# kan-bayashi/ParallelWaveGAN

Hardware: AMD Instinct MI355X
Metric: HiFi-GAN V1 22.05 kHz generator inference RTF^-1 (audio samples/s) (higher is better)
Workload: dtype f32; 1 GPU; HiFi-GAN V1 generator fwd, LJSpeech 22.05 kHz, B16 x 800 mel frames per GPU, fp32, random init; global_batch=16, parallelism=replicas x1

## Files before the change

include/pwg_kernels.h:

```cpp
#ifndef PWG_KERNELS_H_
#define PWG_KERNELS_H_

#include <stddef.h>
#include <stdint.h>

#ifdef __cplusplus
extern "C" {
#endif

typedef enum pwg_status {
  PWG_OK = 0,
  PWG_ERR_BAD_SHAPE = -1,
  PWG_ERR_UNSUPPORTED = -2,
  PWG_ERR_LAUNCH = -3,
  PWG_ERR_NULL = -4,
  PWG_ERR_WORKSPACE = -5
} pwg_status;

const char* pwg_last_error(void);
int pwg_abi_version(void);
int pwg_target_arch(void);

int pwg_prof_enable(int on);
int pwg_prof_reset(void);
int pwg_prof_num_kernels(void);
int pwg_prof_get(int32_t idx, char* name, size_t name_cap, double* total_ms, int64_t* launches,
                 double* flops, double* bytes);

float pwg_set_concurrency_hint(float fill_scale);

int pwg_debug_poison_lds(int on);

enum { PWG_ACT_NONE = 0, PWG_ACT_LEAKY_RELU = 1, PWG_ACT_TANH = 2, PWG_ACT_RELU = 3 };
enum { PWG_PAD_ZERO = 0, PWG_PAD_REFLECT = 1, PWG_PAD_REPLICATE = 2 };

typedef struct pwg_conv1d_desc {
  int32_t batch;
  int32_t c_in;
  int32_t c_out;
  int32_t t_in;
  int32_t t_out;
  int32_t width;
  int32_t kernel;
  int32_t stride;
  int32_t dilation;
  int32_t pad_left;
  int32_t groups;
  int32_t transposed;
  int32_t pad_mode;
  int32_t pre_act;
  float pre_slope;
  int32_t post_act;
  float post_slope;
  float out_mul;
  float out_div;
} pwg_conv1d_desc;

size_t pwg_conv1d_packed_weight_floats(const pwg_conv1d_desc* d);

int pwg_conv1d_pack_weight(const pwg_conv1d_desc* d, const float* w, const float* scale,
                           float* w_packed, void* stream);

size_t pwg_conv1d_forward_workspace_floats(const pwg_conv1d_desc* d);
int pwg_conv1d_forward(const pwg_conv1d_desc* d, const float* x, const float* w_packed,
                       const float* bias, const float* add1, const float* add2, float* y,
                       float* workspace, size_t workspace_floats, void* stream);

size_t pwg_conv1d_packed_weight_bwd_floats(const pwg_conv1d_desc* d);
int pwg_conv1d_pack_weight_bwd(const pwg_conv1d_desc* d, const float* w, const float* scale,
                               float* w_packed_bwd, void* stream);
typedef struct pwg_bank_item {
  const float* w;
  const float* g;
  float* scale;
  float* fwd;
  float* bwd;
  pwg_conv1d_desc desc;
} pwg_bank_item;
size_t pwg_weight_bank_table_bytes(int32_t n_items);
int pwg_weight_bank_build(const pwg_bank_item* items, int32_t n_items, void* table_host, size_t table_bytes,
                          int32_t* info);
int pwg_weight_bank_prepare(const void* table_dev, const int32_t* info, int32_t with_bwd, void* stream);

size_t pwg_conv1d_backward_data_workspace_floats(const pwg_conv1d_desc* d);
int pwg_conv1d_backward_data(const pwg_conv1d_desc* d, const float* dy, const float* w_packed_bwd,
                             const float* x, const float* accum, float* dx, float* workspace,
                             size_t workspace_floats, void* stream);
size_t pwg_conv1d_backward_weight_workspace_floats(const pwg_conv1d_desc* d);
int pwg_conv1d_backward_weight(const pwg_conv1d_desc* d, const float* x, const float* dy, float* dw,
                               float* db, float* workspace, size_t workspace_floats, void* stream);

size_t pwg_conv1d_backward_weight_wn_workspace_floats(const pwg_conv1d_desc* d);
int pwg_conv1d_backward_weight_wn(const pwg_conv1d_desc* d, const float* x, const float* dy, const float* v,
                                  const float* g, float* dv, float* dg, float* db, float* workspace,
                                  size_t workspace_floats, void* stream);

int pwg_conv1d_num_tile_configs(void);
int pwg_conv1d_forward_cfg(const pwg_conv1d_desc* d, const float* x, const float* w_packed,
                           const float* bias, const float* add1, const float* add2, float* y,
                           int32_t tile_config, int32_t use_dma, void* stream);

int pwg_conv1d_bf16_supported(const pwg_conv1d_desc* d);
size_t pwg_conv1d_bf16_packed_weight_bytes(const pwg_conv1d_desc* d);
int pwg_conv1d_bf16_pack_weight(const pwg_conv1d_desc* d, const float* w, const float* scale, void* w_packed,
                                void* stream);
int pwg_conv1d_bf16_forward(const pwg_conv1d_desc* d, const float* x, const void* w_packed, const float* bias,
                            const float* add1, const float* add2, float* y, float* workspace, size_t workspace_floats,
                            void* stream);
int pwg_conv1d_bf16_forward_cfg(const pwg_conv1d_desc* d, const float* x, const void* w_packed, const float* bias,
                                const float* add1, const float* add2, float* y, int32_t mfma_shape, void* stream);

int pwg_conv1d_split_supported(const pwg_conv1d_desc* d);
size_t pwg_conv1d_split_packed_weight_bytes(const pwg_conv1d_desc* d);
int pwg_conv1d_split_pack_weight(const pwg_conv1d_desc* d, const float* w, const float* scale, void* w_packed,
                                 void* stream);
int pwg_conv1d_split_forward(const pwg_conv1d_desc* d, const float* x, const void* w_packed, const float* bias,
                             const float* add1, const float* add2, float* y, float* workspace, size_t workspace_floats,
                             void* stream);
int pwg_conv1d_split_forward_cfg(const pwg_conv1d_desc* d, const float* x, const void* w_packed, const float* bias,
                                 const float* add1, const float* add2, float* y, int32_t mfma_shape, int32_t tile_mode,
                                 void* stream);
int pwg_conv1d_split_step_form(const pwg_conv1d_desc* d);
int pwg_conv1d_split_forward_step(const pwg_conv1d_desc* d, const float* x, const void* w_packed, const float* bias,
                                  const float* add1, const float* add2, float* y, int32_t mfma_shape, int32_t tile_mode,
                                  int32_t step_form, void* stream);
int pwg_conv1d_split_window_form(const pwg_conv1d_desc* d);
int pwg_conv1d_split_forward_window(const pwg_conv1d_desc* d, const float* x, const void* w_packed, const float* bias,
                                    const float* add1, const float* add2, float* y, int32_t mfma_shape,
                                    int32_t tile_mode, int32_t step_form, int32_t window_form, void* stream);

int pwg_convtr1d_split_supported(const pwg_conv1d_desc* d);
size_t pwg_convtr1d_split_packed_weight_bytes(const pwg_conv1d_desc* d);
int pwg_convtr1d_split_pack_weight(const pwg_conv1d_desc* d, const float* w, const float* scale, void* w_packed,
                                   void* stream);
int pwg_convtr1d_split_forward(const pwg_conv1d_desc* d, const float* x, const void* w_packed, const float* bias,
                               const float* add1, const float* add2, float* y, float* workspace,
                               size_t workspace_floats, void* stream);
int pwg_convtr1d_split_forward_cfg(const pwg_conv1d_desc* d, const float* x, const void* w_packed, const float* bias,
                                   const float* add1, const float* add2, float* y, int32_t mfma_shape,
                                   int32_t tile_mode, void* stream);

int pwg_conv1d_stream_supported(const pwg_conv1d_desc* d);
size_t pwg_conv1d_stream_hist_floats(const pwg_conv1d_desc* d);
int pwg_conv1d_stream_forward(const pwg_conv1d_desc* d, const float* x, const float* hist_in, float* hist_out,
                              const float* w_packed, const float* bias, const float* add1, const float* add2, float* y,
                              void* stream);

int pwg_conv1d_stream_bf16_supported(const pwg_conv1d_desc* d);
int pwg_conv1d_stream_bf16_forward(const pwg_conv1d_desc* d, const float* x, const float* hist_in, float* hist_out,
                                   const void* w_packed_bf16, const float* bias, const float* add1,
                                   const float* add2, float* y, void* stream);

int pwg_conv1d_stream_delayed_supported(const pwg_conv1d_desc* d, int32_t delay1, int32_t delay2);
int pwg_conv1d_stream_delayed_forward(const pwg_conv1d_desc* d, const float* x, const float* hist_in, float* hist_out,
                                      const float* w_packed, const float* bias, const float* add1,
                                      const float* add1_hist_in, float* add1_hist_out, int32_t delay1, const float* add2,
                                      const float* add2_hist_in, float* add2_hist_out, int32_t delay2, int32_t valid_lo,
                                      int32_t valid_hi, float* y, void* stream);

int pwg_conv1d_stream_bf16_delayed_supported(const pwg_conv1d_desc* d, int32_t delay1, int32_t delay2);
int pwg_conv1d_stream_bf16_delayed_forward(const pwg_conv1d_desc* d, const float* x, const float* hist_in,
                                           float* hist_out, const void* w_packed_bf16, const float* bias,
                                           const float* add1, const float* add1_hist_in, float* add1_hist_out,
                                           int32_t delay1, const float* add2, const float* add2_hist_in,
                                           float* add2_hist_out, int32_t delay2, int32_t valid_lo, int32_t valid_hi,
                                           float* y, void* stream);

int pwg_conv1d_stream_slots_forward(const pwg_conv1d_desc* d, const float* x, const float* hist_in, float* hist_out,
                                    const float* w_packed, const float* bias, const float* add1,
                                    const float* add1_hist_in, float* add1_hist_out, int32_t delay1, const float* add2,
                                    const float* add2_hist_in, float* add2_hist_out, int32_t delay2, const int32_t* slots,
                                    int32_t rate, int32_t delay, float* y, void* stream);
int pwg_conv1d_stream_slots_forward_bf16(const pwg_conv1d_desc* d, const float* x, const float* hist_in, float* hist_out,
                                         const void* w_packed_bf16, const float* bias, const float* add1,
                                         const float* add1_hist_in, float* add1_hist_out, int32_t delay1,
                                         const float* add2, const float* add2_hist_in, float* add2_hist_out,
                                         int32_t delay2, const int32_t* slots, int32_t rate, int32_t delay, float* y,
                                         void* stream);

int pwg_conv1d_stream_mirrored_supported(const pwg_conv1d_desc* d);
int pwg_conv1d_stream_mirrored_forward(const pwg_conv1d_desc* d, const float* x, const float* hist_in, float* hist_out,
                                       const float* w_packed, const float* bias, float* y, int32_t in_lo, int32_t in_hi,
                                       int32_t valid_lo, int32_t valid_hi, void* stream);

int pwg_conv1d_stream_plan(const pwg_conv1d_desc* d, int32_t* out);

int pwg_conv1d_plan(const pwg_conv1d_desc* d, int32_t has_addends, int32_t* out);
int pwg_debug_conv_tile_of_workgroup(int32_t grid_x, int32_t grid_y, int32_t grid_z, int32_t row_blocks,
                                     int32_t ksplit, int32_t item_major, int32_t workgroup, int32_t* out);

int pwg_conv1d_backward_weight_plan(const pwg_conv1d_desc* d, int32_t weight_norm, int32_t has_bias, int32_t* out);

typedef struct pwg_resunit_desc {
  int32_t batch;
  int32_t channels;
  int32_t t;
  int32_t kernel;
  int32_t dilation;
  int32_t has_conv2;
  float slope1;
  float slope2;
  float out_div;
} pwg_resunit_desc;
int pwg_resunit_supported(const pwg_resunit_desc* d);
int pwg_resunit_profitable(const pwg_resunit_desc* d);
size_t pwg_resunit_packed_weight_floats(int32_t channels, int32_t kernel);
int pwg_resunit_pack_weight(int32_t channels, int32_t kernel, const float* w, const float* scale,
                            float* w_packed, void* stream);
int pwg_resunit_forward(const pwg_resunit_desc* d, const float* x, const float* w1_packed, const float* b1,
                        const float* w2_packed, const float* b2, const float* add2, float* y, void* stream);

int pwg_resunit_split_supported(const pwg_resunit_desc* d);
int pwg_resunit_split_forward(const pwg_resunit_desc* d, const float* x, const void* w1_split, const float* b1,
                              const void* w2_split, const float* b2, const float* add2, float* y, void* stream);
int pwg_resunit_split_forward_cfg(const pwg_resunit_desc* d, const float* x, const void* w1_split, const float* b1,
                                  const void* w2_split, const float* b2, const float* add2, float* y, int32_t mfma_shape,
                                  void* stream);
int pwg_resunit_split_ragged_supported(const pwg_resunit_desc* d, int32_t rate);
int pwg_resunit_split_forward_ragged(const pwg_resunit_desc* d, const float* x, const void* w1_split, const float* b1,
                                     const void* w2_split, const float* b2, const float* add2, float* y,
                                     int32_t mfma_shape, const int32_t* frames, int32_t rate, void* stream);
int pwg_resblock_split_supported(const pwg_resunit_desc* d, int32_t n_units, const int32_t* dilations);
int pwg_resblock_split_frame(const pwg_resunit_desc* d, int32_t n_units, const int32_t* dilations, int32_t* out);
int pwg_resblock_split_forward_cfg(const pwg_resunit_desc* d, int32_t n_units, const int32_t* dilations,
                                   const float* slopes1, const float* slopes2, const float* x,
                                   const void* const* w1_split, const float* const* b1, const void* const* w2_split,
                                   const float* const* b2, const float* add2, float* y, int32_t mfma_shape, void* stream);

int pwg_resstack_supported(int32_t channels, int32_t t, int32_t dilation);
size_t pwg_resstack_packed_weight_floats(int32_t channels);
int pwg_resstack_pack_weight(int32_t channels, const float* w1, const float* scale1, const float* w2,
                             const float* scale2, const float* ws, const float* scale_s, float* w_packed, void* stream);
int pwg_resstack_forward(int32_t batch, int32_t channels, int32_t t, int32_t dilation, float slope, const float* x,
                         const float* w_packed, const float* b1, const float* b2, const float* bs, float* y, float* h,
                         void* stream);
int pwg_resstack_ragged_supported(int32_t channels, int32_t t, int32_t dilation, int32_t rate);
int pwg_resstack_forward_ragged(int32_t batch, int32_t channels, int32_t t, int32_t dilation, float slope, const float* x,
                                const float* w_packed, const float* b1, const float* b2, const float* bs, float* y,
                                const int32_t* frames, int32_t rate, void* stream);
int pwg_resstack_pack_weight_bwd(int32_t channels, const float* w1, const float* scale1, const float* w2,
                                 const float* scale2, const float* ws, const float* scale_s, float* w_packed,
                                 void* stream);
int pwg_resstack_backward_data(int32_t batch, int32_t channels, int32_t t, int32_t dilation, float slope,
                               const float* dy, const float* h, const float* x, const float* w_packed_bwd, float* dh,
                               float* dxp, void* stream);

typedef struct pwg_wavenet_desc {
  int32_t batch;
  int32_t t;
  int32_t residual_channels;
  int32_t gate_channels;
  int32_t skip_channels;
  int32_t aux_channels;
  int32_t kernel;
  int32_t dilation;
  int32_t causal;
  float out_mul;
  float skip_mul;
} pwg_wavenet_desc;
int pwg_wavenet_layer_supported(const pwg_wavenet_desc* d);
size_t pwg_wavenet_packed_weight_floats(const pwg_wavenet_desc* d);
int pwg_wavenet_pack_weights(const pwg_wavenet_desc* d, const float* w_dil, const float* scale_dil, const float* w_aux,
                             const float* scale_aux, const float* w_skip, const float* scale_skip, const float* w_out,
                             const float* scale_out, float* packed, void* stream);
int pwg_wavenet_layer_forward(const pwg_wavenet_desc* d, const float* x, const float* c, const float* skips,
                              const float* packed, const float* b_dil, const float* b_skip, const float* b_out,
                              float* x_out, float* skips_out, float* z_out, float* g_out, void* stream);
int pwg_wavenet_stream_supported(const pwg_wavenet_desc* d);
size_t pwg_wavenet_stream_hist_floats(const pwg_wavenet_desc* d);
int pwg_wavenet_stream_forward(const pwg_wavenet_desc* d, const float* x, const float* c, const float* skips,
                               const float* hist_in, float* hist_out, const float* packed, const float* b_dil,
                               const float* b_skip, const float* b_out, float* x_out, float* skips_out, void* stream);
int pwg_wavenet_stream_delayed_supported(const pwg_wavenet_desc* d, int32_t c_delay);
size_t pwg_wavenet_stream_delayed_hist_floats(const pwg_wavenet_desc* d);
int pwg_wavenet_stream_delayed_forward(const pwg_wavenet_desc* d, const float* x, const float* c, const float* c_line,
                                       int32_t c_cols, int32_t c_delay, const float* skips, const float* skip_line_in,
                                       float* skip_line_out, const float* hist_in, float* hist_out, const float* packed,
                                       const float* b_dil, const float* b_skip, const float* b_out, int32_t valid_lo,
                                       int32_t valid_hi, float* x_out, float* skips_out, void* stream);
int pwg_wavenet_stream_slots_forward(const pwg_wavenet_desc* d, const float* x, const float* c, const float* c_line,
                                     int32_t c_cols, int32_t c_delay, const float* skips, const float* skip_line_in,
                                     float* skip_line_out, const float* hist_in, float* hist_out, const float* packed,
                                     const float* b_dil, const float* b_skip, const float* b_out, const int32_t* slots,
                                     int32_t rate, int32_t delay, float* x_out, float* skips_out, void* stream);
int pwg_wavenet_stream_slots_forward_bf16(const pwg_wavenet_desc* d, const float* x, const float* c, const float* c_line,
                                          int32_t c_cols, int32_t c_delay, const float* skips, const float* skip_line_in,
                                          float* skip_line_out, const float* hist_in, float* hist_out, const void* packed,
                                          const float* b_dil, const float* b_skip, const float* b_out,
                                          const int32_t* slots, int32_t rate, int32_t delay, float* x_out,
                                          float* skips_out, void* stream);
int pwg_wavenet_bf16_supported(const pwg_wavenet_desc* d);
size_t pwg_wavenet_bf16_packed_weight_bytes(const pwg_wavenet_desc* d);
int pwg_wavenet_bf16_pack_weights(const pwg_wavenet_desc* d, const float* w_dil, const float* scale_dil,
                                  const float* w_aux, const float* scale_aux, const float* w_skip, const float* scale_skip,
                                  const float* w_out, const float* scale_out, void* packed, void* stream);
int pwg_wavenet_bf16_layer_forward(const pwg_wavenet_desc* d, const float* x, const float* c, const float* skips,
                                   const void* packed, const float* b_dil, const float* b_skip, const float* b_out,
                                   float* x_out, float* skips_out, float* z_out, float* g_out, void* stream);
int pwg_wavenet_bf16_layer_forward_cfg(const pwg_wavenet_desc* d, const float* x, const float* c, const float* skips,
                                       const void* packed, const float* b_dil, const float* b_skip, const float* b_out,
                                       float* x_out, float* skips_out, float* z_out, float* g_out, int32_t mfma_shape,
                                       void* stream);
int pwg_wavenet_layer_ragged_supported(const pwg_wavenet_desc* d, int32_t rate);
int pwg_wavenet_layer_forward_ragged(const pwg_wavenet_desc* d, const float* x, const float* c, const float* skips,
                                     const float* packed, const float* b_dil, const float* b_skip, const float* b_out,
                                     float* x_out, float* skips_out, const int32_t* frames, int32_t rate, void* stream);
int pwg_wavenet_bf16_layer_forward_ragged(const pwg_wavenet_desc* d, const float* x, const float* c, const float* skips,
                                          const void* packed, const float* b_dil, const float* b_skip,
                                          const float* b_out, float* x_out, float* skips_out, int32_t mfma_shape,
                                          const int32_t* frames, int32_t rate, void* stream);
int pwg_wavenet_stream_bf16_supported(const pwg_wavenet_desc* d);
int pwg_wavenet_stream_bf16_forward(const pwg_wavenet_desc* d, const float* x, const float* c, const float* skips,
                                    const float* hist_in, float* hist_out, const void* packed, const float* b_dil,
                                    const float* b_skip, const float* b_out, float* x_out, float* skips_out, float* z_out,
                                    float* g_out, void* stream);
int pwg_wavenet_stream_bf16_delayed_supported(const pwg_wavenet_desc* d, int32_t c_delay);
int pwg_wavenet_stream_bf16_delayed_forward(const pwg_wavenet_desc* d, const float* x, const float* c, const float* c_line,
                                            int32_t c_cols, int32_t c_delay, const float* skips, const float* skip_line_in,
                                            float* skip_line_out, const float* hist_in, float* hist_out, const void* packed,
                                            const float* b_dil, const float* b_skip, const float* b_out, int32_t valid_lo,
                                            int32_t valid_hi, float* x_out, float* skips_out, float* z_out, float* g_out,
                                            void* stream);
size_t pwg_wavenet_packed_weight_bwd_floats(const pwg_wavenet_desc* d);
int pwg_wavenet_pack_weights_bwd(const pwg_wavenet_desc* d, const float* w_dil, const float* scale_dil, const float* w_aux,
                                 const float* scale_aux, const float* w_skip, const float* scale_skip, const float* w_out,
                                 const float* scale_out, float* packed, void* stream);
int pwg_wavenet_gate_backward(const pwg_wavenet_desc* d, const float* z, const float* dx_out, const float* ds_out,
                              const float* packed_bwd, float* dz, float* go, void* stream);
int pwg_wavenet_data_backward(const pwg_wavenet_desc* d, const float* dz, const float* go, const float* packed_bwd,
                              const float* dc_accum, float* dx, float* dc, void* stream);
typedef struct pwg_wavenet_param_grad {
  const float* v;
  const float* g;
  float* dw;
  float* dg;
  float* db;
} pwg_wavenet_param_grad;
size_t pwg_wavenet_weight_backward_workspace_floats(const pwg_wavenet_desc* d);
int pwg_wavenet_weight_backward(const pwg_wavenet_desc* d, const float* dz, const float* x, const float* c, const float* gs,
                                const float* go, const float* g, const pwg_wavenet_param_grad* grads, float* workspace,
                                size_t workspace_floats, void* stream);
int pwg_wavenet_weight_backward_plan(const pwg_wavenet_desc* d, int32_t out[4]);

int pwg_weight_norm_scale(const float* v, const float* g, float* scale, int32_t n0,
                          int32_t inner, void* stream);
int pwg_scale_rows(const float* v, const float* scale, float* w, int32_t n0, int32_t inner,
                   void* stream);

int pwg_act_backward(const float* dy, const float* y, float* dx, int64_t n, int32_t act, float slope,
                     float scale, void* stream);
int pwg_add3_div(const float* a, const float* b, const float* c, float* y, int64_t n, float div, void* stream);
int pwg_weight_norm_backward(const float* dw, const float* v, const float* g, float* dv, float* dg,
                             int32_t n0, int32_t inner, void* stream);
int pwg_spectral_norm_forward(const float* w_orig, float* u, float* v, float* sigma, float* w, float* tmp,
                              int32_t rows, int32_t cols, int32_t do_iter, float eps, void* stream);
int pwg_spectral_norm_forward_saved(const float* w_orig, float* u, float* v, float* sigma, float* w, float* tmp,
                                    float* u_saved, float* v_saved, int32_t rows, int32_t cols, int32_t do_iter,
                                    float eps, void* stream);
#define PWG_SPECTRAL_NORM_SCRATCH_FLOATS 257
int pwg_spectral_norm_backward(const float* dw, const float* w_orig, const float* u, const float* v,
                               const float* sigma, float* dw_orig, float* scratch, int32_t rows,
                               int32_t cols, void* stream);

int pwg_gate_forward(const float* z, float* out, int32_t batch, int32_t channels, int64_t t, void* stream);
int pwg_gate_backward(const float* z, const float* dout, float* dz, int32_t batch, int32_t channels,
                      int64_t t, void* stream);
#define PWG_STRETCH_CONV_WGRAD_BLOCKS 512
int pwg_stretch_conv_forward(const float* x, const float* w, float* y, int64_t rows, int32_t t_in,
                             int32_t scale, int32_t kernel, int32_t pad_left, int32_t channels,
                             int32_t freq_kernel, int32_t act, float slope, void* stream);
int pwg_stretch_conv_stream(const float* x, const float* hist_in, float* hist_out, const float* w, float* y,
                            int64_t rows, int32_t n, int32_t scale, int32_t freq_kernel, int32_t act, float slope,
                            void* stream);
int pwg_stretch_conv_stream_delayed(const float* x, const float* hist_in, float* hist_out, const float* w, float* y,
                                    int64_t rows, int32_t n, int32_t scale, int32_t freq_kernel, int32_t act, float slope,
                                    int32_t valid_lo, int32_t valid_hi, void* stream);
int pwg_delay_line_forward(const float* x, const float* line_in, float* line_out, float* delayed_out, int64_t rows,
                           int32_t n, int32_t columns, void* stream);
int pwg_stretch_conv_stream_slots(const float* x, const float* hist_in, float* hist_out, const float* w, float* y,
                                  int64_t items, int32_t channels, int32_t n, int32_t scale, int32_t freq_kernel,
                                  int32_t act, float slope, const int32_t* slots, int32_t rate, int32_t delay, void* stream);
int pwg_delay_line_slots_forward(const float* x, const float* line_in, float* line_out, float* delayed_out, int64_t items,
                                 int32_t channels, int32_t n, int32_t columns, const int32_t* slots, void* stream);
int pwg_slot_seed_history(const float* x, float* hist, int64_t items, int32_t channels, int32_t n, int32_t columns,
                          const int32_t* slots, void* stream);
size_t pwg_stretch_conv_backward_workspace_floats(int32_t kernel, int32_t freq_kernel);
int pwg_stretch_conv_backward(const float* dy, const float* x, const float* w, float* dx, float* dw,
                              int64_t rows, int32_t t_in, int32_t scale, int32_t kernel, int32_t pad_left,
                              int32_t channels, int32_t freq_kernel, float* workspace, size_t workspace_floats,
                              void* stream);
int pwg_pqmf_down(const float* x, const float* h, float* y, int32_t batch, int64_t t_in, int64_t n_out,
                  int32_t subbands, int32_t len, int32_t pad, void* stream);
int pwg_pqmf_up(const float* y, const float* g, float* x, int32_t batch, int64_t n_in, int64_t t_out,
                int32_t subbands, int32_t len, int32_t pad, void* stream);

int pwg_pqmf_up_stream_geometry(int32_t subbands, int32_t len, int32_t pad, int32_t* hist_columns,
                                int32_t* delay_columns);
int pwg_pqmf_up_stream(const float* y, const float* hist_in, float* hist_out, const float* g, float* x, int32_t batch,
                       int64_t n, int64_t n_emit, int32_t subbands, int32_t len, int32_t pad, void* stream);

int pwg_instance_norm_forward(const float* x, float* y, float* mean, float* rstd, int64_t rows, int32_t t,
                              float eps, void* stream);
int pwg_instance_norm_backward(const float* dy, const float* y, const float* rstd, float* dx, int64_t rows,
                               int32_t t, void* stream);
int pwg_upsample_nearest_forward(const float* x, const float* add, float* y, int64_t rows, int32_t t_in,
                                 int32_t scale, void* stream);
int pwg_upsample_nearest_backward(const float* dy, float* dx, int64_t rows, int32_t t_in, int32_t scale,
                                  void* stream);
int pwg_tade_modulate_forward(const float* xn, const float* cg, float* y, int32_t batch, int32_t channels,
                              int32_t t_in, int32_t scale, void* stream);
int pwg_tade_modulate_backward(const float* dy, const float* xn, const float* cg, float* dxn, float* dcg,
                               int32_t batch, int32_t channels, int32_t t_in, int32_t scale, void* stream);
int pwg_softmax_gate_forward(const float* z, float* y, int32_t batch, int32_t channels, int64_t t,
                             int32_t use_softmax, void* stream);
int pwg_softmax_gate_backward(const float* z, const float* dy, float* dz, int32_t batch, int32_t channels,
                              int64_t t, int32_t use_softmax, void* stream);

int pwg_copy_channels(float* x, float* y, int32_t batch, int32_t c_src, int32_t c_dst, int32_t c_off,
                      int64_t t, int32_t reverse, void* stream);
int pwg_dropout(const float* x, float* y, int64_t n, float p, uint64_t seed, const uint64_t* seed_dev,
                void* stream);

int pwg_gather_crop(const float* audio, const int64_t* audio_off, const int64_t* audio_len, const float* mel,
                    const int64_t* mel_off, const int32_t* utt, const int32_t* start, float* y, float* c,
                    int32_t batch, int32_t steps, int32_t hop, int32_t frames_ctx, int32_t acw,
                    int32_t channels, void* stream);

int pwg_wave_to_pcm16(const float* x, int16_t* pcm, int64_t n, void* stream);
int pwg_normalize_transpose(const float* x, const float* mean, const float* scale, float* y,
                            int32_t batch, int32_t frames, int32_t channels, void* stream);
int pwg_zero_tail(float* y, const int32_t* frames, int32_t batch, int32_t channels, int64_t t, int32_t rate,
                  void* stream);
int pwg_mirror_tail(float* y, const int32_t* frames, int32_t batch, int32_t channels, int64_t t, int32_t rate,
                    int32_t pad, void* stream);

int pwg_avg_pool1d_forward(const float* x, float* y, int64_t rows, int32_t t_in, int32_t t_out,
                           int32_t kernel, int32_t stride, int32_t pad, int32_t count_include_pad,
                           void* stream);
int pwg_avg_pool1d_backward(const float* dy, float* dx, int64_t rows, int32_t t_in, int32_t t_out,
                            int32_t kernel, int32_t stride, int32_t pad, int32_t count_include_pad,
                            void* stream);
int pwg_pad1d_forward(const float* x, float* y, int64_t rows, int32_t t_in, int32_t pad_left,
                      int32_t pad_right, int32_t mode, void* stream);
int pwg_pad1d_backward(const float* dy, float* dx, int64_t rows, int32_t t_in, int32_t pad_left,
                       int32_t pad_right, int32_t mode, void* stream);

int pwg_frame_fold_forward(const float* x, float* y, int32_t batch, int32_t t, int32_t pad, int32_t hop,
                           int32_t n_cols, void* stream);
int pwg_frame_fold_backward(const float* dy, float* dx, int32_t batch, int32_t t, int32_t pad,
                            int32_t hop, int32_t n_cols, void* stream);
int pwg_stft_mag_forward(const float* spec, float* mag, int32_t batch, int32_t bins, int32_t frames,
                         float eps, void* stream);
int pwg_stft_mag_backward(const float* spec, const float* mag, const float* dmag, float* dspec,
                          int32_t batch, int32_t bins, int32_t frames, float eps, void* stream);
int pwg_log_clamp_forward(const float* x, float* y, int64_t n, float eps, float log_div, void* stream);
int pwg_log_clamp_backward(const float* x, const float* dy, float* dx, int64_t n, float eps, float log_div,
                           void* stream);

size_t pwg_stft_loss_workspace_floats(int32_t batch, int32_t bins, int32_t frames);
int pwg_stft_loss_forward(const float* fx, const float* fy, const float* basis, int32_t batch, int32_t hop,
                          int32_t n_cols, int32_t taps, int32_t bins, int32_t frames, float eps,
                          float* workspace, float* sums, void* stream);
int pwg_stft_loss_backward(const float* fx, const float* fy, const float* basis, int32_t batch, int32_t hop,
                           int32_t n_cols, int32_t taps, int32_t bins, int32_t frames, float eps,
                           const float* sums, const float* g2, float* dspec, void* stream);

int pwg_stft_fft_supported(int32_t n_fft, int32_t win, int32_t hop);
size_t pwg_stft_fft_workspace_floats(int32_t batch, int32_t frames, int32_t n_fft);
int pwg_stft_fft_loss_forward(const float* x, const float* y, const float* window, const float* twiddle, int32_t batch,
                              int32_t t, int32_t n_fft, int32_t hop, int32_t win, float eps, float* workspace,
                              float* sums, void* stream);
int pwg_stft_fft_loss_backward(const float* x, const float* y, const float* window, const float* twiddle, int32_t batch,
                               int32_t t, int32_t n_fft, int32_t hop, int32_t win, float eps, const float* sums,
                               const float* g2, float* dframes, float* dx, void* stream);

int pwg_mel_fft_loss_forward(const float* x, const float* y, const float* window, const float* twiddle, const float* fb,
                             const int32_t* mel_range, const int32_t* bin_range, int32_t batch, int32_t t, int32_t n_fft,
                             int32_t hop, int32_t win, int32_t n_mels, int32_t bins_pad, float eps, float log_div,
                             float* workspace, float* total, void* stream);
int pwg_mel_fft_loss_backward(const float* x, const float* y, const float* window, const float* twiddle, const float* fb,
                              const int32_t* mel_range, const int32_t* bin_range, int32_t batch, int32_t t, int32_t n_fft,
                              int32_t hop, int32_t win, int32_t n_mels, int32_t bins_pad, float eps, float log_div,
                              const float* gout, float* dframes, float* dx, void* stream);

size_t pwg_mel_loss_workspace_floats(int32_t batch, int32_t bins, int32_t frames, int32_t n_mels);
int pwg_mel_loss_forward(const float* fx, const float* fy, const float* basis, const float* mel_t, int32_t batch,
                         int32_t hop, int32_t n_cols, int32_t taps, int32_t bins, int32_t frames, int32_t n_mels,
                         float eps, float log_div, float* workspace, float* mel_x, float* mel_y, float* sum,
                         void* stream);
int pwg_mel_loss_backward(const float* fx, const float* basis, const float* mel_b, const float* mel_x,
                          const float* mel_y, int32_t batch, int32_t hop, int32_t n_cols, int32_t taps,
                          int32_t bins, int32_t frames, int32_t n_mels, float eps, float log_div,
                          const float* gout, float* dspec, void* stream);

enum { PWG_RED_ABS_DIFF = 0, PWG_RED_SQ_DIFF = 1, PWG_RED_SQ = 2, PWG_RED_SQ_DIFF_CONST = 3, PWG_RED_SUM = 4,
       PWG_RED_HINGE_REAL = 5, PWG_RED_HINGE_FAKE = 6 };
int pwg_reduce_forward(const float* a, const float* b, float c, int64_t n, int32_t mode, float scale,
                       float* out, float* workspace, void* stream);
int pwg_reduce_backward(const float* a, const float* b, float c, int64_t n, int32_t mode, float scale,
                        const float* gout, float* da, float* db, void* stream);

#define PWG_RED_MAX_ITEMS 64
typedef struct pwg_red_item {
  const float* a;
  const float* b;
  float* da;
  float* db;
  int64_t n;
  int32_t mode;
  int32_t slot;
  float scale;
  float c;
} pwg_red_item;
size_t pwg_multi_reduce_workspace_floats(const pwg_red_item* items, int32_t n_items);
int pwg_multi_reduce_forward(const pwg_red_item* items, int32_t n_items, int32_t n_slots, float* out,
                             int32_t accumulate, float* workspace, void* stream);
int pwg_multi_reduce_backward(const pwg_red_item* items, int32_t n_items, int32_t n_slots, const float* gout,
                              void* stream);

typedef struct pwg_opt_chunk {
  float* p;
  const float* g;
  float* m;
  float* v;
  float* vmax;
  int32_t n;
  int32_t pad_;
} pwg_opt_chunk;
int pwg_adam_step(const void* chunks, int32_t n_chunks, float lr, float beta1, float beta2, float eps,
                  float weight_decay, int32_t step, float grad_scale, void* stream);
// ... 12 lines not shown
```

parallelwavegan_amd/_lib.py:

```python
import ctypes
import os

_HERE = os.path.dirname(os.path.abspath(__file__))
LIB_PATH = os.environ.get("PWG_KERNEL_LIB") or os.path.join(_HERE, "libpwgkernels.so")

PWG_ACT_NONE, PWG_ACT_LEAKY_RELU, PWG_ACT_TANH, PWG_ACT_RELU = 0, 1, 2, 3
PWG_PAD_ZERO, PWG_PAD_REFLECT, PWG_PAD_REPLICATE = 0, 1, 2
ABI_VERSION = 15
SPECTRAL_NORM_SCRATCH_FLOATS = 257


class ConvDesc(ctypes.Structure):

    _fields_ = [
        ("batch", ctypes.c_int32),
        ("c_in", ctypes.c_int32),
        ("c_out", ctypes.c_int32),
        ("t_in", ctypes.c_int32),
        ("t_out", ctypes.c_int32),
        ("width", ctypes.c_int32),
        ("kernel", ctypes.c_int32),
        ("stride", ctypes.c_int32),
        ("dilation", ctypes.c_int32),
        ("pad_left", ctypes.c_int32),
        ("groups", ctypes.c_int32),
        ("transposed", ctypes.c_int32),
        ("pad_mode", ctypes.c_int32),
        ("pre_act", ctypes.c_int32),
        ("pre_slope", ctypes.c_float),
        ("post_act", ctypes.c_int32),
        ("post_slope", ctypes.c_float),
        ("out_mul", ctypes.c_float),
        ("out_div", ctypes.c_float),
    ]


class BankItem(ctypes.Structure):

    _fields_ = [("w", ctypes.c_void_p), ("g", ctypes.c_void_p), ("scale", ctypes.c_void_p), ("fwd", ctypes.c_void_p),
                ("bwd", ctypes.c_void_p), ("desc", ConvDesc)]


class WaveNetDesc(ctypes.Structure):

    _fields_ = [
        ("batch", ctypes.c_int32),
        ("t", ctypes.c_int32),
        ("residual_channels", ctypes.c_int32),
        ("gate_channels", ctypes.c_int32),
        ("skip_channels", ctypes.c_int32),
        ("aux_channels", ctypes.c_int32),
        ("kernel", ctypes.c_int32),
        ("dilation", ctypes.c_int32),
        ("causal", ctypes.c_int32),
        ("out_mul", ctypes.c_float),
        ("skip_mul", ctypes.c_float),
    ]


class WaveNetParamGrad(ctypes.Structure):

    _fields_ = [("v", ctypes.c_void_p), ("g", ctypes.c_void_p), ("dw", ctypes.c_void_p), ("dg", ctypes.c_void_p),
                ("db", ctypes.c_void_p)]


class ResUnitDesc(ctypes.Structure):

    _fields_ = [
        ("batch", ctypes.c_int32),
        ("channels", ctypes.c_int32),
        ("t", ctypes.c_int32),
        ("kernel", ctypes.c_int32),
        ("dilation", ctypes.c_int32),
        ("has_conv2", ctypes.c_int32),
        ("slope1", ctypes.c_float),
        ("slope2", ctypes.c_float),
        ("out_div", ctypes.c_float),
    ]


class RedItem(ctypes.Structure):

    _fields_ = [
        ("a", ctypes.c_void_p),
        ("b", ctypes.c_void_p),
        ("da", ctypes.c_void_p),
        ("db", ctypes.c_void_p),
        ("n", ctypes.c_int64),
        ("mode", ctypes.c_int32),
        ("slot", ctypes.c_int32),
        ("scale", ctypes.c_float),
        ("c", ctypes.c_float),
    ]


RED_MAX_ITEMS = 64

_lib = None
_vp = ctypes.c_void_p
_i32 = ctypes.c_int32
_i64 = ctypes.c_int64
_f32 = ctypes.c_float

SIGNATURES = {
    "pwg_last_error": (ctypes.c_char_p, []),
    "pwg_abi_version": (ctypes.c_int, []),
    "pwg_target_arch": (ctypes.c_int, []),
    "pwg_debug_poison_lds": (ctypes.c_int, [ctypes.c_int]),
    "pwg_set_concurrency_hint": (ctypes.c_float, [ctypes.c_float]),
    "pwg_prof_enable": (ctypes.c_int, [ctypes.c_int]),
    "pwg_prof_reset": (ctypes.c_int, []),
    "pwg_prof_num_kernels": (ctypes.c_int, []),
    "pwg_prof_get": (ctypes.c_int, [_i32, ctypes.c_char_p, ctypes.c_size_t, ctypes.POINTER(ctypes.c_double),
                                    ctypes.POINTER(ctypes.c_int64), ctypes.POINTER(ctypes.c_double),
                                    ctypes.POINTER(ctypes.c_double)]),
    "pwg_conv1d_packed_weight_floats": (ctypes.c_size_t, [ctypes.POINTER(ConvDesc)]),
    "pwg_conv1d_pack_weight": (ctypes.c_int, [ctypes.POINTER(ConvDesc), _vp, _vp, _vp, _vp]),
    "pwg_conv1d_forward_workspace_floats": (ctypes.c_size_t, [ctypes.POINTER(ConvDesc)]),
    "pwg_conv1d_forward": (ctypes.c_int, [ctypes.POINTER(ConvDesc), _vp, _vp, _vp, _vp, _vp, _vp, _vp, ctypes.c_size_t,
                                          _vp]),
    "pwg_conv1d_bf16_supported": (ctypes.c_int, [ctypes.POINTER(ConvDesc)]),
    "pwg_conv1d_bf16_packed_weight_bytes": (ctypes.c_size_t, [ctypes.POINTER(ConvDesc)]),
    "pwg_conv1d_bf16_pack_weight": (ctypes.c_int, [ctypes.POINTER(ConvDesc), _vp, _vp, _vp, _vp]),
    "pwg_conv1d_bf16_forward": (ctypes.c_int, [ctypes.POINTER(ConvDesc), _vp, _vp, _vp, _vp, _vp, _vp, _vp, ctypes.c_size_t,
                                               _vp]),
    "pwg_conv1d_bf16_forward_cfg": (ctypes.c_int, [ctypes.POINTER(ConvDesc), _vp, _vp, _vp, _vp, _vp, _vp, _i32, _vp]),
    "pwg_conv1d_split_supported": (ctypes.c_int, [ctypes.POINTER(ConvDesc)]),
    "pwg_conv1d_split_packed_weight_bytes": (ctypes.c_size_t, [ctypes.POINTER(ConvDesc)]),
    "pwg_conv1d_split_pack_weight": (ctypes.c_int, [ctypes.POINTER(ConvDesc), _vp, _vp, _vp, _vp]),
    "pwg_conv1d_split_forward": (ctypes.c_int, [ctypes.POINTER(ConvDesc), _vp, _vp, _vp, _vp, _vp, _vp, _vp,
                                                ctypes.c_size_t, _vp]),
    "pwg_conv1d_split_forward_cfg": (ctypes.c_int, [ctypes.POINTER(ConvDesc), _vp, _vp, _vp, _vp, _vp, _vp, _i32, _i32,
                                                    _vp]),
    "pwg_conv1d_split_step_form": (ctypes.c_int, [ctypes.POINTER(ConvDesc)]),
    "pwg_conv1d_split_forward_step": (ctypes.c_int, [ctypes.POINTER(ConvDesc), _vp, _vp, _vp, _vp, _vp, _vp, _i32, _i32,
                                                     _i32, _vp]),
    "pwg_conv1d_split_window_form": (ctypes.c_int, [ctypes.POINTER(ConvDesc)]),
    "pwg_conv1d_split_forward_window": (ctypes.c_int, [ctypes.POINTER(ConvDesc), _vp, _vp, _vp, _vp, _vp, _vp, _i32,
                                                       _i32, _i32, _i32, _vp]),
    "pwg_convtr1d_split_supported": (ctypes.c_int, [ctypes.POINTER(ConvDesc)]),
    "pwg_convtr1d_split_packed_weight_bytes": (ctypes.c_size_t, [ctypes.POINTER(ConvDesc)]),
    "pwg_convtr1d_split_pack_weight": (ctypes.c_int, [ctypes.POINTER(ConvDesc), _vp, _vp, _vp, _vp]),
    "pwg_convtr1d_split_forward": (ctypes.c_int, [ctypes.POINTER(ConvDesc), _vp, _vp, _vp, _vp, _vp, _vp, _vp,
                                                  ctypes.c_size_t, _vp]),
    "pwg_convtr1d_split_forward_cfg": (ctypes.c_int, [ctypes.POINTER(ConvDesc), _vp, _vp, _vp, _vp, _vp, _vp, _i32, _i32,
                                                      _vp]),
    "pwg_conv1d_stream_supported": (ctypes.c_int, [ctypes.POINTER(ConvDesc)]),
    "pwg_conv1d_stream_hist_floats": (ctypes.c_size_t, [ctypes.POINTER(ConvDesc)]),
    "pwg_conv1d_stream_forward": (ctypes.c_int, [ctypes.POINTER(ConvDesc), _vp, _vp, _vp, _vp, _vp, _vp, _vp, _vp, _vp]),
    "pwg_conv1d_stream_plan": (ctypes.c_int, [ctypes.POINTER(ConvDesc), ctypes.POINTER(_i32)]),
    "pwg_conv1d_stream_bf16_supported": (ctypes.c_int, [ctypes.POINTER(ConvDesc)]),
    "pwg_conv1d_stream_bf16_forward": (ctypes.c_int, [ctypes.POINTER(ConvDesc), _vp, _vp, _vp, _vp, _vp, _vp, _vp, _vp,
                                                      _vp]),
    "pwg_conv1d_stream_delayed_supported": (ctypes.c_int, [ctypes.POINTER(ConvDesc), _i32, _i32]),
    "pwg_conv1d_stream_delayed_forward": (ctypes.c_int, [ctypes.POINTER(ConvDesc), _vp, _vp, _vp, _vp, _vp, _vp, _vp, _vp,
                                                         _i32, _vp, _vp, _vp, _i32, _i32, _i32, _vp, _vp]),
    "pwg_conv1d_stream_bf16_delayed_supported": (ctypes.c_int, [ctypes.POINTER(ConvDesc), _i32, _i32]),
    "pwg_conv1d_stream_bf16_delayed_forward": (ctypes.c_int, [ctypes.POINTER(ConvDesc), _vp, _vp, _vp, _vp, _vp, _vp, _vp,
                                                              _vp, _i32, _vp, _vp, _vp, _i32, _i32, _i32, _vp, _vp]),
    "pwg_conv1d_stream_slots_forward": (ctypes.c_int, [ctypes.POINTER(ConvDesc), _vp, _vp, _vp, _vp, _vp, _vp, _vp, _vp,
                                                       _i32, _vp, _vp, _vp, _i32, _vp, _i32, _i32, _vp, _vp]),
    "pwg_conv1d_stream_slots_forward_bf16": (ctypes.c_int, [ctypes.POINTER(ConvDesc), _vp, _vp, _vp, _vp, _vp, _vp, _vp,
                                                            _vp, _i32, _vp, _vp, _vp, _i32, _vp, _i32, _i32, _vp, _vp]),
    "pwg_conv1d_stream_mirrored_supported": (ctypes.c_int, [ctypes.POINTER(ConvDesc)]),
    "pwg_conv1d_stream_mirrored_forward": (ctypes.c_int, [ctypes.POINTER(ConvDesc), _vp, _vp, _vp, _vp, _vp, _vp, _i32,
                                                          _i32, _i32, _i32, _vp]),
    "pwg_conv1d_packed_weight_bwd_floats": (ctypes.c_size_t, [ctypes.POINTER(ConvDesc)]),
    "pwg_conv1d_pack_weight_bwd": (ctypes.c_int, [ctypes.POINTER(ConvDesc), _vp, _vp, _vp, _vp]),
    "pwg_weight_bank_table_bytes": (ctypes.c_size_t, [_i32]),
    "pwg_weight_bank_build": (ctypes.c_int, [ctypes.POINTER(BankItem), _i32, _vp, ctypes.c_size_t,
                                             ctypes.POINTER(ctypes.c_int32)]),
    "pwg_weight_bank_prepare": (ctypes.c_int, [_vp, ctypes.POINTER(ctypes.c_int32), _i32, _vp]),
    "pwg_conv1d_backward_data_workspace_floats": (ctypes.c_size_t, [ctypes.POINTER(ConvDesc)]),
    "pwg_conv1d_backward_data": (ctypes.c_int, [ctypes.POINTER(ConvDesc), _vp, _vp, _vp, _vp, _vp, _vp, ctypes.c_size_t,
                                                _vp]),
    "pwg_conv1d_backward_weight_workspace_floats": (ctypes.c_size_t, [ctypes.POINTER(ConvDesc)]),
    "pwg_conv1d_backward_weight": (ctypes.c_int, [ctypes.POINTER(ConvDesc), _vp, _vp, _vp, _vp, _vp, ctypes.c_size_t, _vp]),
    "pwg_conv1d_backward_weight_wn_workspace_floats": (ctypes.c_size_t, [ctypes.POINTER(ConvDesc)]),
    "pwg_conv1d_backward_weight_wn": (ctypes.c_int, [ctypes.POINTER(ConvDesc), _vp, _vp, _vp, _vp, _vp, _vp, _vp, _vp,
                                                     ctypes.c_size_t, _vp]),
    "pwg_conv1d_num_tile_configs": (ctypes.c_int, []),
    "pwg_conv1d_forward_cfg": (ctypes.c_int, [ctypes.POINTER(ConvDesc), _vp, _vp, _vp, _vp, _vp, _vp, _i32, _i32, _vp]),
    "pwg_conv1d_plan": (ctypes.c_int, [ctypes.POINTER(ConvDesc), _i32, ctypes.POINTER(_i32)]),
    "pwg_conv1d_backward_weight_plan": (ctypes.c_int, [ctypes.POINTER(ConvDesc), _i32, _i32, ctypes.POINTER(_i32)]),
    "pwg_debug_conv_tile_of_workgroup": (ctypes.c_int, [_i32, _i32, _i32, _i32, _i32, _i32, _i32, ctypes.POINTER(_i32)]),
    "pwg_resunit_supported": (ctypes.c_int, [ctypes.POINTER(ResUnitDesc)]),
    "pwg_resunit_profitable": (ctypes.c_int, [ctypes.POINTER(ResUnitDesc)]),
    "pwg_resunit_packed_weight_floats": (ctypes.c_size_t, [_i32, _i32]),
    "pwg_resunit_pack_weight": (ctypes.c_int, [_i32, _i32, _vp, _vp, _vp, _vp]),
    "pwg_resunit_forward": (ctypes.c_int, [ctypes.POINTER(ResUnitDesc), _vp, _vp, _vp, _vp, _vp, _vp, _vp, _vp]),
    "pwg_resunit_split_supported": (ctypes.c_int, [ctypes.POINTER(ResUnitDesc)]),
    "pwg_resunit_split_forward": (ctypes.c_int, [ctypes.POINTER(ResUnitDesc), _vp, _vp, _vp, _vp, _vp, _vp, _vp, _vp]),
    "pwg_resunit_split_forward_cfg": (ctypes.c_int, [ctypes.POINTER(ResUnitDesc), _vp, _vp, _vp, _vp, _vp, _vp, _vp, _i32,
                                                     _vp]),
    "pwg_resunit_split_ragged_supported": (ctypes.c_int, [ctypes.POINTER(ResUnitDesc), _i32]),
    "pwg_resunit_split_forward_ragged": (ctypes.c_int, [ctypes.POINTER(ResUnitDesc), _vp, _vp, _vp, _vp, _vp, _vp, _vp,
                                                        _i32, _vp, _i32, _vp]),
    "pwg_resblock_split_supported": (ctypes.c_int, [ctypes.POINTER(ResUnitDesc), _i32, ctypes.POINTER(_i32)]),
    "pwg_resblock_split_frame": (ctypes.c_int, [ctypes.POINTER(ResUnitDesc), _i32, ctypes.POINTER(_i32),
                                                ctypes.POINTER(_i32)]),
    "pwg_resblock_split_forward_cfg": (ctypes.c_int, [ctypes.POINTER(ResUnitDesc), _i32, ctypes.POINTER(_i32),
                                                      ctypes.POINTER(ctypes.c_float), ctypes.POINTER(ctypes.c_float), _vp,
                                                      ctypes.POINTER(_vp), ctypes.POINTER(_vp), ctypes.POINTER(_vp),
                                                      ctypes.POINTER(_vp), _vp, _vp, _i32, _vp]),
    "pwg_resstack_supported": (ctypes.c_int, [_i32, _i32, _i32]),
    "pwg_resstack_packed_weight_floats": (ctypes.c_size_t, [_i32]),
    "pwg_resstack_pack_weight": (ctypes.c_int, [_i32, _vp, _vp, _vp, _vp, _vp, _vp, _vp, _vp]),
    "pwg_resstack_forward": (ctypes.c_int, [_i32, _i32, _i32, _i32, ctypes.c_float, _vp, _vp, _vp, _vp, _vp, _vp, _vp, _vp]),
    "pwg_resstack_ragged_supported": (ctypes.c_int, [_i32, _i32, _i32, _i32]),
    "pwg_resstack_forward_ragged": (ctypes.c_int, [_i32, _i32, _i32, _i32, ctypes.c_float, _vp, _vp, _vp, _vp, _vp, _vp, _vp,
                                                   _i32, _vp]),
    "pwg_resstack_pack_weight_bwd": (ctypes.c_int, [_i32, _vp, _vp, _vp, _vp, _vp, _vp, _vp, _vp]),
    "pwg_resstack_backward_data": (ctypes.c_int, [_i32, _i32, _i32, _i32, ctypes.c_float, _vp, _vp, _vp, _vp, _vp, _vp, _vp]),
    "pwg_wavenet_layer_supported": (ctypes.c_int, [ctypes.POINTER(WaveNetDesc)]),
    "pwg_wavenet_packed_weight_floats": (ctypes.c_size_t, [ctypes.POINTER(WaveNetDesc)]),
    "pwg_wavenet_pack_weights": (ctypes.c_int, [ctypes.POINTER(WaveNetDesc)] + [_vp] * 10),
    "pwg_wavenet_layer_forward": (ctypes.c_int, [ctypes.POINTER(WaveNetDesc)] + [_vp] * 12),
    "pwg_wavenet_stream_supported": (ctypes.c_int, [ctypes.POINTER(WaveNetDesc)]),
    "pwg_wavenet_stream_hist_floats": (ctypes.c_size_t, [ctypes.POINTER(WaveNetDesc)]),
    "pwg_wavenet_stream_forward": (ctypes.c_int, [ctypes.POINTER(WaveNetDesc)] + [_vp] * 12),
    "pwg_wavenet_stream_delayed_supported": (ctypes.c_int, [ctypes.POINTER(WaveNetDesc), _i32]),
    "pwg_wavenet_stream_delayed_hist_floats": (ctypes.c_size_t, [ctypes.POINTER(WaveNetDesc)]),
    "pwg_wavenet_stream_delayed_forward": (ctypes.c_int, [ctypes.POINTER(WaveNetDesc), _vp, _vp, _vp, _i32, _i32] + [_vp] * 9
                                           + [_i32, _i32, _vp, _vp, _vp]),
    "pwg_wavenet_stream_slots_forward": (ctypes.c_int, [ctypes.POINTER(WaveNetDesc), _vp, _vp, _vp, _i32, _i32] + [_vp] * 9
                                         + [_vp, _i32, _i32, _vp, _vp, _vp]),
    "pwg_wavenet_stream_slots_forward_bf16": (ctypes.c_int, [ctypes.POINTER(WaveNetDesc), _vp, _vp, _vp, _i32, _i32]
                                              + [_vp] * 9 + [_vp, _i32, _i32, _vp, _vp, _vp]),
    "pwg_wavenet_bf16_supported": (ctypes.c_int, [ctypes.POINTER(WaveNetDesc)]),
    "pwg_wavenet_bf16_packed_weight_bytes": (ctypes.c_size_t, [ctypes.POINTER(WaveNetDesc)]),
    "pwg_wavenet_bf16_pack_weights": (ctypes.c_int, [ctypes.POINTER(WaveNetDesc)] + [_vp] * 10),
    "pwg_wavenet_bf16_layer_forward": (ctypes.c_int, [ctypes.POINTER(WaveNetDesc)] + [_vp] * 12),
    "pwg_wavenet_bf16_layer_forward_cfg": (ctypes.c_int, [ctypes.POINTER(WaveNetDesc)] + [_vp] * 11 + [_i32, _vp]),
    "pwg_wavenet_layer_ragged_supported": (ctypes.c_int, [ctypes.POINTER(WaveNetDesc), _i32]),
    "pwg_wavenet_layer_forward_ragged": (ctypes.c_int, [ctypes.POINTER(WaveNetDesc)] + [_vp] * 10 + [_i32, _vp]),
    "pwg_wavenet_bf16_layer_forward_ragged": (ctypes.c_int, [ctypes.POINTER(WaveNetDesc)] + [_vp] * 9
                                              + [_i32, _vp, _i32, _vp]),
    "pwg_wavenet_stream_bf16_supported": (ctypes.c_int, [ctypes.POINTER(WaveNetDesc)]),
    "pwg_wavenet_stream_bf16_forward": (ctypes.c_int, [ctypes.POINTER(WaveNetDesc)] + [_vp] * 14),
    "pwg_wavenet_stream_bf16_delayed_supported": (ctypes.c_int, [ctypes.POINTER(WaveNetDesc), _i32]),
    "pwg_wavenet_stream_bf16_delayed_forward": (ctypes.c_int, [ctypes.POINTER(WaveNetDesc), _vp, _vp, _vp, _i32, _i32]
                                                + [_vp] * 9 + [_i32, _i32, _vp, _vp, _vp, _vp, _vp]),
    "pwg_wavenet_packed_weight_bwd_floats": (ctypes.c_size_t, [ctypes.POINTER(WaveNetDesc)]),
    "pwg_wavenet_pack_weights_bwd": (ctypes.c_int, [ctypes.POINTER(WaveNetDesc)] + [_vp] * 10),
    "pwg_wavenet_gate_backward": (ctypes.c_int, [ctypes.POINTER(WaveNetDesc)] + [_vp] * 7),
    "pwg_wavenet_data_backward": (ctypes.c_int, [ctypes.POINTER(WaveNetDesc)] + [_vp] * 7),
    "pwg_wavenet_weight_backward_workspace_floats": (ctypes.c_size_t, [ctypes.POINTER(WaveNetDesc)]),
    "pwg_wavenet_weight_backward_plan": (ctypes.c_int, [ctypes.POINTER(WaveNetDesc), ctypes.POINTER(_i32)]),
    "pwg_wavenet_weight_backward": (ctypes.c_int, [ctypes.POINTER(WaveNetDesc)] + [_vp] * 6
                                    + [ctypes.POINTER(WaveNetParamGrad), _vp, ctypes.c_size_t, _vp]),
    "pwg_act_backward": (ctypes.c_int, [_vp, _vp, _vp, _i64, _i32, _f32, _f32, _vp]),
    "pwg_add3_div": (ctypes.c_int, [_vp, _vp, _vp, _vp, _i64, _f32, _vp]),
    "pwg_wave_to_pcm16": (ctypes.c_int, [_vp, _vp, _i64, _vp]),
    "pwg_copy_channels": (ctypes.c_int, [_vp, _vp, _i32, _i32, _i32, _i32, _i64, _i32, _vp]),
    "pwg_dropout": (ctypes.c_int, [_vp, _vp, _i64, _f32, ctypes.c_uint64, _vp, _vp]),
    "pwg_instance_norm_forward": (ctypes.c_int, [_vp, _vp, _vp, _vp, _i64, _i32, _f32, _vp]),
    "pwg_instance_norm_backward": (ctypes.c_int, [_vp, _vp, _vp, _vp, _i64, _i32, _vp]),
    "pwg_upsample_nearest_forward": (ctypes.c_int, [_vp, _vp, _vp, _i64, _i32, _i32, _vp]),
    "pwg_upsample_nearest_backward": (ctypes.c_int, [_vp, _vp, _i64, _i32, _i32, _vp]),
    "pwg_tade_modulate_forward": (ctypes.c_int, [_vp, _vp, _vp, _i32, _i32, _i32, _i32, _vp]),
    "pwg_tade_modulate_backward": (ctypes.c_int, [_vp, _vp, _vp, _vp, _vp, _i32, _i32, _i32, _i32, _vp]),
    "pwg_softmax_gate_forward": (ctypes.c_int, [_vp, _vp, _i32, _i32, _i64, _i32, _vp]),
    "pwg_softmax_gate_backward": (ctypes.c_int, [_vp, _vp, _vp, _i32, _i32, _i64, _i32, _vp]),
    "pwg_gather_crop": (ctypes.c_int, [_vp, _vp, _vp, _vp, _vp, _vp, _vp, _vp, _vp, _i32, _i32, _i32, _i32, _i32, _i32,
                                       _vp]),
    "pwg_normalize_transpose": (ctypes.c_int, [_vp, _vp, _vp, _vp, _i32, _i32, _i32, _vp]),
    "pwg_zero_tail": (ctypes.c_int, [_vp, _vp, _i32, _i32, _i64, _i32, _vp]),
    "pwg_mirror_tail": (ctypes.c_int, [_vp, _vp, _i32, _i32, _i64, _i32, _i32, _vp]),
    "pwg_weight_norm_backward": (ctypes.c_int, [_vp, _vp, _vp, _vp, _vp, _i32, _i32, _vp]),
    "pwg_spectral_norm_forward": (ctypes.c_int, [_vp, _vp, _vp, _vp, _vp, _vp, _i32, _i32, _i32, _f32, _vp]),
    "pwg_spectral_norm_forward_saved": (ctypes.c_int, [_vp, _vp, _vp, _vp, _vp, _vp, _vp, _vp, _i32, _i32, _i32, _f32, _vp]),
    "pwg_spectral_norm_backward": (ctypes.c_int, [_vp, _vp, _vp, _vp, _vp, _vp, _vp, _i32, _i32, _vp]),
    "pwg_gate_forward": (ctypes.c_int, [_vp, _vp, _i32, _i32, _i64, _vp]),
    "pwg_gate_backward": (ctypes.c_int, [_vp, _vp, _vp, _i32, _i32, _i64, _vp]),
    "pwg_stretch_conv_forward": (ctypes.c_int, [_vp, _vp, _vp, _i64, _i32, _i32, _i32, _i32, _i32, _i32, _i32, _f32, _vp]),
    "pwg_stretch_conv_stream": (ctypes.c_int, [_vp, _vp, _vp, _vp, _vp, _i64, _i32, _i32, _i32, _i32, _f32, _vp]),
    "pwg_stretch_conv_stream_delayed": (ctypes.c_int, [_vp, _vp, _vp, _vp, _vp, _i64, _i32, _i32, _i32, _i32, _f32, _i32, _i32,
                                                       _vp]),
    "pwg_delay_line_forward": (ctypes.c_int, [_vp, _vp, _vp, _vp, _i64, _i32, _i32, _vp]),
    "pwg_stretch_conv_stream_slots": (ctypes.c_int, [_vp, _vp, _vp, _vp, _vp, _i64, _i32, _i32, _i32, _i32, _i32, _f32, _vp,
                                                     _i32, _i32, _vp]),
    "pwg_delay_line_slots_forward": (ctypes.c_int, [_vp, _vp, _vp, _vp, _i64, _i32, _i32, _i32, _vp, _vp]),
    "pwg_slot_seed_history": (ctypes.c_int, [_vp, _vp, _i64, _i32, _i32, _i32, _vp, _vp]),
    "pwg_stretch_conv_backward_workspace_floats": (ctypes.c_size_t, [_i32, _i32]),
    "pwg_stretch_conv_backward": (ctypes.c_int, [_vp, _vp, _vp, _vp, _vp, _i64, _i32, _i32, _i32, _i32, _i32, _i32, _vp,
                                                 ctypes.c_size_t, _vp]),
    "pwg_pqmf_down": (ctypes.c_int, [_vp, _vp, _vp, _i32, _i64, _i64, _i32, _i32, _i32, _vp]),
    "pwg_pqmf_up": (ctypes.c_int, [_vp, _vp, _vp, _i32, _i64, _i64, _i32, _i32, _i32, _vp]),
    "pwg_pqmf_up_stream_geometry": (ctypes.c_int, [_i32, _i32, _i32, ctypes.POINTER(_i32), ctypes.POINTER(_i32)]),
    "pwg_pqmf_up_stream": (ctypes.c_int, [_vp, _vp, _vp, _vp, _vp, _i32, _i64, _i64, _i32, _i32, _i32, _vp]),
    "pwg_avg_pool1d_forward": (ctypes.c_int, [_vp, _vp, _i64, _i32, _i32, _i32, _i32, _i32, _i32, _vp]),
    "pwg_avg_pool1d_backward": (ctypes.c_int, [_vp, _vp, _i64, _i32, _i32, _i32, _i32, _i32, _i32, _vp]),
    "pwg_pad1d_forward": (ctypes.c_int, [_vp, _vp, _i64, _i32, _i32, _i32, _i32, _vp]),
    "pwg_pad1d_backward": (ctypes.c_int, [_vp, _vp, _i64, _i32, _i32, _i32, _i32, _vp]),
    "pwg_frame_fold_forward": (ctypes.c_int, [_vp, _vp, _i32, _i32, _i32, _i32, _i32, _vp]),
    "pwg_frame_fold_backward": (ctypes.c_int, [_vp, _vp, _i32, _i32, _i32, _i32, _i32, _vp]),
    "pwg_stft_mag_forward": (ctypes.c_int, [_vp, _vp, _i32, _i32, _i32, _f32, _vp]),
    "pwg_stft_mag_backward": (ctypes.c_int, [_vp, _vp, _vp, _vp, _i32, _i32, _i32, _f32, _vp]),
    "pwg_stft_loss_workspace_floats": (ctypes.c_size_t, [_i32, _i32, _i32]),
    "pwg_stft_loss_forward": (ctypes.c_int, [_vp, _vp, _vp, _i32, _i32, _i32, _i32, _i32, _i32, _f32, _vp, _vp, _vp]),
    "pwg_stft_loss_backward": (ctypes.c_int, [_vp, _vp, _vp, _i32, _i32, _i32, _i32, _i32, _i32, _f32, _vp, _vp, _vp,
                                              _vp]),
    "pwg_stft_fft_supported": (ctypes.c_int, [_i32, _i32, _i32]),
    "pwg_stft_fft_workspace_floats": (ctypes.c_size_t, [_i32, _i32, _i32]),
    "pwg_stft_fft_loss_forward": (ctypes.c_int, [_vp, _vp, _vp, _vp, _i32, _i32, _i32, _i32, _i32, _f32, _vp, _vp, _vp]),
    "pwg_stft_fft_loss_backward": (ctypes.c_int, [_vp, _vp, _vp, _vp, _i32, _i32, _i32, _i32, _i32, _f32, _vp, _vp, _vp,
                                                  _vp, _vp]),
    "pwg_mel_fft_loss_forward": (ctypes.c_int, [_vp] * 7 + [_i32] * 7 + [_f32, _f32, _vp, _vp, _vp]),
    "pwg_mel_fft_loss_backward": (ctypes.c_int, [_vp] * 7 + [_i32] * 7 + [_f32, _f32, _vp, _vp, _vp, _vp]),
    "pwg_mel_loss_workspace_floats": (ctypes.c_size_t, [_i32, _i32, _i32, _i32]),
    "pwg_mel_loss_forward": (ctypes.c_int, [_vp, _vp, _vp, _vp, _i32, _i32, _i32, _i32, _i32, _i32, _i32, _f32, _f32, _vp,
                                            _vp, _vp, _vp, _vp]),
    "pwg_mel_loss_backward": (ctypes.c_int, [_vp, _vp, _vp, _vp, _vp, _i32, _i32, _i32, _i32, _i32, _i32, _i32, _f32, _f32,
                                             _vp, _vp, _vp]),
    "pwg_log_clamp_forward": (ctypes.c_int, [_vp, _vp, _i64, _f32, _f32, _vp]),
    "pwg_log_clamp_backward": (ctypes.c_int, [_vp, _vp, _vp, _i64, _f32, _f32, _vp]),
    "pwg_reduce_forward": (ctypes.c_int, [_vp, _vp, _f32, _i64, _i32, _f32, _vp, _vp, _vp]),
    "pwg_reduce_backward": (ctypes.c_int, [_vp, _vp, _f32, _i64, _i32, _f32, _vp, _vp, _vp, _vp]),
    "pwg_multi_reduce_workspace_floats": (ctypes.c_size_t, [ctypes.POINTER(RedItem), _i32]),
    "pwg_multi_reduce_forward": (ctypes.c_int, [ctypes.POINTER(RedItem), _i32, _i32, _vp, _i32, _vp, _vp]),
    "pwg_multi_reduce_backward": (ctypes.c_int, [ctypes.POINTER(RedItem), _i32, _i32, _vp, _vp]),
    "pwg_adam_step": (ctypes.c_int, [_vp, _i32, _f32, _f32, _f32, _f32, _f32, _i32, _f32, _vp]),
    "pwg_radam_step": (ctypes.c_int, [_vp, _i32, _f32, _f32, _f32, _f32, _f32, _i32, _f32, _vp]),
    "pwg_adam_step_dev": (ctypes.c_int, [_vp, _i32, _vp, _vp]),
    "pwg_radam_step_dev": (ctypes.c_int, [_vp, _i32, _vp, _vp]),
    "pwg_clip_grad_norm": (ctypes.c_int, [_vp, _i32, _f32, _vp, _vp, _vp]),
    "pwg_weight_norm_scale": (ctypes.c_int, [_vp, _vp, _vp, _i32, _i32, _vp]),
    "pwg_scale_rows": (ctypes.c_int, [_vp, _vp, _vp, _i32, _i32, _vp]),
}


def lib():
    global _lib
    if _lib is None:
        if not os.path.exists(LIB_PATH):
            raise RuntimeError(
                f"{LIB_PATH} not found: build it with `python -m parallelwavegan_amd.csrc.build` "
                "(hipcc --offload-arch=gfx950). This package has no fallback compute path."
            )
        import torch

        l = ctypes.CDLL(LIB_PATH)
        for name, (res, args) in SIGNATURES.items():
            fn = getattr(l, name)
            fn.restype = res
            fn.argtypes = args
        if l.pwg_abi_version() != ABI_VERSION:
            raise RuntimeError(
                f"libpwgkernels.so ABI {l.pwg_abi_version()} != expected {ABI_VERSION}; rebuild it"
            )
        _lib = l
    return _lib


def check(rc, what=""):
    if rc != 0:
        msg = lib().pwg_last_error().decode(errors="replace")
        raise RuntimeError(f"pwg kernel call failed ({what}, status {rc}): {msg}")
```

parallelwavegan_amd/csrc/mfma_conv.h:

```cpp
#pragma once
#include "common.h"

#include "bf16_mfma.h"

#include <stdint.h>

namespace pwg {

constexpr int KC = 32;
constexpr int kConvRow = KC + 8;
constexpr size_t kConvMaxLds = 64 * 1024;
constexpr int kConvFillWorkgroups = 256;

static inline int plane_rows(int nt, int halo) { return round_up(nt + halo + 3, 4); }
static inline size_t conv_lds_bytes(int parts, int nt, int halo) {
  return (size_t)parts * plane_rows(nt, halo) * kConvRow * sizeof(__bf16);
}

constexpr int conv_row_tile(int m) { return m <= 32 ? 32 : (m <= 64 ? 64 : 128); }
constexpr int image_m_pad(int m) { return (m + conv_row_tile(m) - 1) / conv_row_tile(m) * conv_row_tile(m); }
constexpr int image_chunks(int c_in) { return (c_in + KC - 1) / KC; }

struct MfmaConvGeom {
  int taps, dil, x_off;
  int m, m_pad, mt;
  int phases, out_off;
  int nq;
  int cin_chunks;
  int nt;
  bool half_only;
};

static inline int mfma_conv_geometry(const char* name, int parts, bool allow_transposed, const pwg_conv1d_desc* d,
                                     MfmaConvGeom* g) {
  PWG_REQUIRE(d != nullptr, PWG_ERR_NULL, "%s: NULL descriptor", name);
  PWG_REQUIRE(d->batch > 0 && d->c_in > 0 && d->c_out > 0 && d->t_in > 0 && d->t_out > 0 && d->kernel > 0 &&
                  d->stride > 0 && d->dilation > 0 && d->groups > 0 && d->width > 0 && d->pad_left >= 0,
              PWG_ERR_BAD_SHAPE, "%s: non-positive size in descriptor", name);
  PWG_REQUIRE(d->groups == 1, PWG_ERR_UNSUPPORTED, "%s: groups = %d (only groups == 1)", name, d->groups);
  PWG_REQUIRE(d->width == 1, PWG_ERR_UNSUPPORTED, "%s: width = %d (only width == 1)", name, d->width);
  PWG_REQUIRE(d->pad_mode == PWG_PAD_ZERO, PWG_ERR_UNSUPPORTED, "%s: only zero padding (pad_mode = %d)", name, d->pad_mode);
  if (!allow_transposed) {
    PWG_REQUIRE(!d->transposed, PWG_ERR_UNSUPPORTED, "%s: transposed convolutions are not covered", name);
    PWG_REQUIRE(d->stride == 1, PWG_ERR_UNSUPPORTED, "%s: stride = %d (only stride 1)", name, d->stride);
  }
  PWG_REQUIRE(d->pre_act == PWG_ACT_NONE || d->pre_act == PWG_ACT_LEAKY_RELU || d->pre_act == PWG_ACT_RELU,
              PWG_ERR_UNSUPPORTED, "%s: pre_act = %d", name, d->pre_act);
  PWG_REQUIRE(d->batch <= 65535, PWG_ERR_UNSUPPORTED, "%s: batch = %d (> 65535)", name, d->batch);
  if (d->transposed) {
    PWG_REQUIRE(d->kernel == 2 * d->stride && d->dilation == 1, PWG_ERR_UNSUPPORTED,
                "%s: transposed convolution with kernel = %d, stride = %d (only kernel == 2 * stride)", name, d->kernel,
                d->stride);
    *g = MfmaConvGeom{2, 1, -1, d->c_out * d->stride, 0, 0, d->stride, d->pad_left,
                      ceil_div(d->t_out + d->pad_left, d->stride)};
  } else {
    PWG_REQUIRE(d->stride == 1, PWG_ERR_UNSUPPORTED, "%s: stride = %d (only stride 1)", name, d->stride);
    *g = MfmaConvGeom{d->kernel, d->dilation, -d->pad_left, d->c_out, 0, 0, 1, 0, d->t_out};
  }
  g->mt = conv_row_tile(g->m);
  g->nt = g->m <= 32 ? 256 : 128;
  g->m_pad = image_m_pad(g->m);
  g->cin_chunks = image_chunks(d->c_in);
  PWG_REQUIRE(parts == 1 || (long)(g->taps - 1) * g->dil < (1 << 20), PWG_ERR_UNSUPPORTED, "%s: receptive field too long",
              name);
  const int halo = (g->taps - 1) * g->dil;
  g->half_only = parts > 1 && conv_lds_bytes(parts, g->nt, halo) > kConvMaxLds;
  const size_t lds = conv_lds_bytes(parts, g->half_only ? g->nt / 2 : g->nt, halo);
  PWG_REQUIRE(lds <= kConvMaxLds, PWG_ERR_UNSUPPORTED, "%s: receptive field (%d taps, dilation %d) needs %zu B of LDS", name,
              g->taps, g->dil, lds);
  PWG_REQUIRE(ceil_div(g->m_pad, g->mt) <= 65535, PWG_ERR_UNSUPPORTED, "%s: too many row blocks", name);
  return PWG_OK;
}

constexpr long image_elems(int taps, int cin_chunks, int m_pad) { return (long)taps * cin_chunks * KC * m_pad; }
static inline long image_elems(const MfmaConvGeom& g) { return image_elems(g.taps, g.cin_chunks, g.m_pad); }

struct ImageIndex {
  int tap, ci, row;
};
__device__ __forceinline__ ImageIndex image_decode(long i, int cin_pad, int m_pad) {
  const int j = (int)(i & 7);
  long rest = i >> 3;
  const int row = (int)(rest % m_pad);
  rest /= m_pad;
  const int oct = (int)(rest % (cin_pad / 8));
  return ImageIndex{(int)(rest / (cin_pad / 8)), oct * 8 + j, row};
}

__device__ __forceinline__ const bf16x8* image_rows(const bf16x8* w, int cin_chunks, int m_pad, int tap, int chunk, int oct) {
  return w + ((size_t)(tap * cin_chunks + chunk) * (KC / 8) + oct) * m_pad;
}

__device__ __forceinline__ void split3(float v, __bf16& hi, __bf16& mid, __bf16& lo) {
  hi = (__bf16)v;
  const float r = v - (float)hi;
  mid = (__bf16)r;
  lo = (__bf16)(r - (float)mid);
}

template <int N>
__device__ __forceinline__ void split3_store(const float (&v)[N], __bf16* dst, int plane) {
  typedef __bf16 vec_t __attribute__((ext_vector_type(N)));
  vec_t vh, vm, vl;
#pragma unroll
  for (int j = 0; j < N; ++j) {
    __bf16 hi, mid, lo;
    split3(v[j], hi, mid, lo);
    vh[j] = hi;
    vm[j] = mid;
    vl[j] = lo;
  }
  *reinterpret_cast<vec_t*>(dst) = vh;
  *reinterpret_cast<vec_t*>(dst + plane) = vm;
  *reinterpret_cast<vec_t*>(dst + 2 * plane) = vl;
}

constexpr int kSplitWeightPart[6] = {2, 0, 1, 1, 0, 0};
constexpr int kSplitInputPart[6] = {0, 2, 1, 0, 1, 0};
template <int TILE, int TN, bool XFIRST>
__device__ __forceinline__ void split_product(int p, const bf16x8 (&wf)[3], const bf16x8 (&bfr)[3][TN],
                                              typename Mfma<TILE>::acc_t (&acc)[TN]) {
#pragma unroll
  for (int ni = 0; ni < TN; ++ni)
    acc[ni] = XFIRST ? Mfma<TILE>::run(bfr[kSplitInputPart[p]][ni], wf[kSplitWeightPart[p]], acc[ni])
                     : Mfma<TILE>::run(wf[kSplitWeightPart[p]], bfr[kSplitInputPart[p]][ni], acc[ni]);
}

template <int TILE, int TN, int ROW>
__device__ __forceinline__ void split_plane_fragments(bf16x8 (&bfr)[3][TN], const __bf16* xs, int col, int off, int plane) {
#pragma unroll
  for (int ni = 0; ni < TN; ++ni) {
    const __bf16* src = xs + (col + ni * TILE) * ROW + off;
#pragma unroll
    for (int p = 0; p < 3; ++p) bfr[p][ni] = *reinterpret_cast<const bf16x8*>(src + p * plane);
  }
}

template <int TILE, int TM, int TN, int ROW, bool XFIRST>
__device__ __forceinline__ void split_step(const bf16x8* __restrict__ wp, long part_stride, const __bf16* xs, int col,
                                           int off, int plane, typename Mfma<TILE>::acc_t (&acc)[TM][TN]) {
  bf16x8 af[TM][3], bfr[3][TN];
#pragma unroll
  for (int p = 0; p < 3; ++p)
#pragma unroll
    for (int mi = 0; mi < TM; ++mi) af[mi][p] = wp[p * part_stride + mi * TILE];
  split_plane_fragments<TILE, TN, ROW>(bfr, xs, col, off, plane);
#pragma unroll
  for (int p = 0; p < 6; ++p)
#pragma unroll
    for (int mi = 0; mi < TM; ++mi) split_product<TILE, TN, XFIRST>(p, af[mi], bfr, acc[mi]);
}

struct SplitStepId {
  int chunk, tap, ks;
};
__host__ __device__ __forceinline__ constexpr SplitStepId split_step_successor(SplitStepId s, int chunks, int taps,
                                                                               int ksteps) {
  if (s.ks + 1 < ksteps) return SplitStepId{s.chunk, s.tap, s.ks + 1};
  if (s.tap + 1 < taps) return SplitStepId{s.chunk, s.tap + 1, 0};
  if (s.chunk + 1 < chunks) return SplitStepId{s.chunk + 1, 0, 0};
  return s;
}
constexpr bool split_step_is(SplitStepId s, int chunk, int tap, int ks) {
  return s.chunk == chunk && s.tap == tap && s.ks == ks;
}
static_assert(split_step_is(split_step_successor({0, 0, 0}, 2, 3, 2), 0, 0, 1), "k-step advances first");
static_assert(split_step_is(split_step_successor({0, 0, 1}, 2, 3, 2), 0, 1, 0), "then the tap");
static_assert(split_step_is(split_step_successor({0, 2, 1}, 2, 3, 2), 1, 0, 0), "last step of an inner chunk");
static_assert(split_step_is(split_step_successor({1, 2, 1}, 2, 3, 2), 1, 2, 1), "last step of the last chunk: clamped");
static_assert(split_step_is(split_step_successor({0, 0, 0}, 2, 3, 1), 0, 1, 0), "KSTEPS = 1: every step is a tap");
static_assert(split_step_is(split_step_successor({0, 2, 0}, 2, 3, 1), 1, 0, 0), "KSTEPS = 1: chunk crossing");
static_assert(split_step_is(split_step_successor({1, 2, 0}, 2, 3, 1), 1, 2, 0), "KSTEPS = 1: clamped");
static_assert(split_step_is(split_step_successor({0, 0, 0}, 1, 1, 1), 0, 0, 0), "one step in total: clamped at once");
static_assert(split_step_is(split_step_successor({0, 0, 0}, 3, 1, 1), 1, 0, 0), "k = 1: a chunk crossing every step");

constexpr bool split_image_addressable(long elems_per_part) { return elems_per_part * (long)sizeof(__bf16) < (1L << 32); }
template <int TILE>
__device__ __forceinline__ unsigned split_step_rows(int cin_chunks, int m_pad, SplitStepId s, int h) {
  return (unsigned)(((s.tap * cin_chunks + s.chunk) * (KC / 8) + s.ks * (64 / TILE) + h) * m_pad);
}
template <int TILE>
__device__ __forceinline__ int split_step_off(SplitStepId s, int h) {
  return (s.ks * (64 / TILE) + h) * 8;
}

__device__ __forceinline__ bf16x8 split_part_request(const bf16x8* __restrict__ w, long part_stride, unsigned row, int part) {
  return *reinterpret_cast<const bf16x8*>(reinterpret_cast<const char*>(w + part * part_stride) +
                                          (size_t)(row * (unsigned)sizeof(bf16x8)));
}
__device__ __forceinline__ void split_step_request(bf16x8 (&wf)[3], const bf16x8* __restrict__ w, long part_stride,
                                                   unsigned row) {
#pragma unroll
  for (int p = 0; p < 3; ++p) wf[p] = split_part_request(w, part_stride, row, p);
}

template <int TILE, int TM, int TN, int ROW, bool XFIRST>
__device__ __forceinline__ void split_step_streamed(bf16x8 (&wf)[3], const bf16x8* __restrict__ w, long part_stride,
                                                    unsigned row, unsigned row_next, const __bf16* xs, int col, int off,
                                                    int plane, typename Mfma<TILE>::acc_t (&acc)[TM][TN]) {
  bf16x8 bfr[3][TN];
  split_plane_fragments<TILE, TN, ROW>(bfr, xs, col, off, plane);
  static_assert(kSplitWeightPart[0] == 2 && kSplitWeightPart[1] != 2 && kSplitWeightPart[2] != 2 &&
                    kSplitWeightPart[3] != 2 && kSplitWeightPart[4] != 2 && kSplitWeightPart[5] != 2,
                "lo is read by the first product only");
#pragma unroll
  for (int mi = 0; mi < TM; ++mi) {
    const unsigned rn = mi + 1 < TM ? row + (mi + 1) * TILE : row_next;
    bf16x8 nx[3];
    nx[0] = split_part_request(w, part_stride, rn, 0);
    nx[1] = split_part_request(w, part_stride, rn, 1);
    __builtin_amdgcn_sched_barrier(0);
#pragma unroll
    for (int p = 0; p < 6; ++p) {
      split_product<TILE, TN, XFIRST>(p, wf, bfr, acc[mi]);
      if (p == 0) {
        __builtin_amdgcn_sched_barrier(0);
        nx[2] = split_part_request(w, part_stride, rn, 2);
        __builtin_amdgcn_sched_barrier(0);
      }
    }
#pragma unroll
    for (int p = 0; p < 3; ++p) wf[p] = nx[p];
    __builtin_amdgcn_sched_barrier(0);
  }
}

template <int PARTS>
static __global__ __launch_bounds__(256) void mfma_conv_pack_kernel(const float* __restrict__ w,
                                                                    const float* __restrict__ scale,
                                                                    __bf16* __restrict__ wp, int c_in, int c_out, int kernel,
                                                                    int taps, int cin_pad, int m, int m_pad, int phases,
                                                                    int transposed) {
  const long total = (long)taps * cin_pad * m_pad;
  for (long i = blockIdx.x * 256L + threadIdx.x; i < total; i += (long)gridDim.x * 256L) {
    const ImageIndex e = image_decode(i, cin_pad, m_pad);
    float v = 0.f;
    if (e.ci < c_in && e.row < m) {
      if (transposed) {
        const int co = e.row / phases, ph = e.row - co * phases;
        const int kk = e.tap == 0 ? ph + phases : ph;
        v = w[((long)e.ci * c_out + co) * kernel + kk];
        if (scale) v *= scale[e.ci];
      } else {
        v = w[((long)e.row * c_in + e.ci) * kernel + e.tap];
        if (scale) v *= scale[e.row];
      }
    }
    if (PARTS == 1) {
      wp[i] = (__bf16)v;
    } else {
      __bf16 hi, mid, lo;
      split3(v, hi, mid, lo);
      wp[i] = hi;
      wp[total + i] = mid;
      wp[2 * total + i] = lo;
    }
  }
}

template <int PARTS>
static inline void mfma_conv_pack(const pwg_conv1d_desc* d, const MfmaConvGeom& g, const float* w, const float* scale,
                                  void* w_packed, hipStream_t stream) {
  int blocks = (int)((image_elems(g) + 255) / 256);
  if (blocks > 4096) blocks = 4096;
  hipLaunchKernelGGL(mfma_conv_pack_kernel<PARTS>, dim3(blocks), dim3(256), 0, stream, w, scale,
                     static_cast<__bf16*>(w_packed), d->c_in, d->c_out, d->kernel, g.taps, g.cin_chunks * KC, g.m, g.m_pad,
                     g.phases, d->transposed);
}

constexpr int window_items(int nt) { return nt >= 128 ? nt / 128 : 1; }

struct MfmaConvPlan {
  bool small, vec;
  int mt, nt;
  int plane;
  dim3 grid;
  size_t lds;
  double flops, bytes;
};

static inline MfmaConvPlan mfma_conv_plan(const pwg_conv1d_desc* d, const MfmaConvGeom& g, int parts, int tile_mode,
                                          const float* x, const float* add1, const float* add2) {
  MfmaConvPlan p;
  const int halo = (g.taps - 1) * g.dil;
  const bool few = (long)ceil_div(g.nq, g.nt) * (g.m_pad / g.mt) * d->batch < kConvFillWorkgroups;
  p.small = g.half_only || (tile_mode == 0 ? few : tile_mode == 2);
  p.mt = p.small ? (g.mt > 32 ? 64 : 32) : g.mt;
  p.nt = p.small ? g.nt / 2 : g.nt;
  p.plane = plane_rows(p.nt, halo) * kConvRow;
  p.grid = dim3(ceil_div(g.nq, p.nt), g.m_pad / p.mt, d->batch);
  p.lds = conv_lds_bytes(parts, p.nt, halo);
  p.vec = d->t_in % 4 == 0 && (reinterpret_cast<uintptr_t>(x) & 15u) == 0 &&
          p.nt + halo + 3 <= window_items(p.nt) * 256;
  const double out_elems = (double)d->batch * d->c_out * d->t_out;
  const double in_elems = (double)d->batch * d->c_in * d->t_in;
  p.flops = 2.0 * (double)d->batch * g.m * g.nq * g.taps * d->c_in;
  p.bytes = 4.0 * (in_elems + out_elems * (1 + (add1 ? 1 : 0) + (add2 ? 1 : 0))) + 2.0 * parts * (double)image_elems(g);
  return p;
}

template <template <int, int, int, int> class K, int TILE, class Args>
static inline auto mfma_conv_tile_kernel(const MfmaConvPlan& p) -> void (*)(Args) {
  if (p.small && p.mt == 32) return K<TILE, 1, 1, 1>::fn;
  if (p.small) return K<TILE, 1, 1, 2>::fn;
  if (p.mt == 32) return K<TILE, 1, 2, 1>::fn;
  if (p.mt == 64) return K<TILE, 1, 2, 2>::fn;
  return K<TILE, 2, 2, 2>::fn;
}
template <template <int, int, int, int> class K, class Args>
static inline void mfma_conv_launch(const MfmaConvPlan& p, int mfma_shape, const Args& a, hipStream_t stream) {
  void (*kern)(Args) = mfma_shape == 32 ? mfma_conv_tile_kernel<K, 32, Args>(p) : mfma_conv_tile_kernel<K, 16, Args>(p);
  hipLaunchKernelGGL(kern, p.grid, dim3(256), p.lds, stream, a);
}

struct MfmaConvArgs {
  const float* x;
  const bf16x8* w;
  const float* bias;
  const float* add1;
  const float* add2;
  float* y;
  int c_in, c_out, t_in, t_out;
  int m, m_pad, cin_chunks, taps, dil, x_off, nq;
  int post_act;
  float post_slope, out_mul, out_div;
};

static inline void mfma_conv_fill_args(MfmaConvArgs* a, const pwg_conv1d_desc* d, const MfmaConvGeom& g, const float* x,
                                       const void* w_packed, const float* bias, const float* add1, const float* add2,
                                       float* y) {
  *a = MfmaConvArgs{x, static_cast<const bf16x8*>(w_packed), bias, add1, add2, y, d->c_in, d->c_out, d->t_in, d->t_out,
                    g.m, g.m_pad, g.cin_chunks, g.taps, g.dil, g.x_off, g.nq, d->post_act, d->post_slope, d->out_mul,
                    d->out_div};
}

static inline int mfma_conv_check_forward(const char* name, const pwg_conv1d_desc* d, const void* x, const void* w_packed,
                                          const void* y, int mfma_shape, int tile_mode) {
  PWG_REQUIRE(x && w_packed && y, PWG_ERR_NULL, "%s: NULL pointer", name);
  PWG_REQUIRE((reinterpret_cast<uintptr_t>(w_packed) & 15u) == 0, PWG_ERR_BAD_SHAPE,
              "%s: the weight image must be 16-B aligned", name);
  PWG_REQUIRE(mfma_shape == 16 || mfma_shape == 32, PWG_ERR_BAD_SHAPE, "%s: mfma_shape = %d (16 or 32)", name, mfma_shape);
  PWG_REQUIRE(tile_mode >= 0 && tile_mode <= 2, PWG_ERR_BAD_SHAPE, "%s: tile_mode = %d (0, 1 or 2)", name, tile_mode);
  PWG_REQUIRE(d->post_act >= PWG_ACT_NONE && d->post_act <= PWG_ACT_RELU, PWG_ERR_BAD_SHAPE, "%s: post_act = %d", name,
              d->post_act);
  return PWG_OK;
}

struct MfmaConvTile {
  int tid, lane, wave, wave_m, wave_n;
  int r, h;
  int q0, m0, b;
  int base;
  int sh;
  int wcols;
  const float* xb;
};
template <int TILE, int MT, int NT, int WAVES_M, bool VEC>
__device__ __forceinline__ MfmaConvTile mfma_conv_tile(const MfmaConvArgs& a) {
  MfmaConvTile c;
  c.tid = threadIdx.x, c.lane = c.tid & 63, c.wave = c.tid >> 6;
  c.wave_m = c.wave % WAVES_M, c.wave_n = c.wave / WAVES_M;
  c.r = c.lane & (TILE - 1), c.h = c.lane / TILE;
  c.q0 = blockIdx.x * NT, c.m0 = blockIdx.y * MT, c.b = blockIdx.z;
  const int start = c.q0 + a.x_off;
  c.base = VEC ? (start & ~3) : start;
  c.sh = start - c.base;
  c.wcols = NT + (a.taps - 1) * a.dil + c.sh;
  c.xb = a.x + (size_t)c.b * a.c_in * a.t_in;
  return c;
}

}
```

parallelwavegan_amd/csrc/resunit_split.hip:

```cpp
#include "mfma_conv.h"

#include <stdlib.h>

#include <type_traits>

namespace pwg {
namespace {

constexpr size_t kRuSplitMaxLds = 80 * 1024;

struct RuSplitArgs {
  const float* x;
  const bf16x8* w1;
  const float* b1;
  const bf16x8* w2;
  const float* b2;
  const float* add2;
  float* y;
  int T, k, d1;
  int bn_out;
  int hla;
  int sh;
  int p2;
  int rows;
  int plane;
  long part_stride;
  float slope1, slope2, out_div;
};

struct RuSplitRaggedArgs : RuSplitArgs {
  const int* frames;
  int rate;
};
template <bool RAGGED>
using RuSplitArgsOf = typename std::conditional<RAGGED, RuSplitRaggedArgs, RuSplitArgs>::type;

template <int C>
struct RuSplitCfg {
  static constexpr int MB = C / KC;
  static constexpr int WAVES_N = 4 / MB;
  static constexpr int H = WAVES_N * 64;
  static constexpr int ROW = C + 8;
  static constexpr int OCTS = C / 8;
  static constexpr int CHUNKS = image_chunks(C), M_PAD = image_m_pad(C);
};

template <int C, bool CHECKED, typename Behind>
__device__ __forceinline__ void ru_stage_window(const RuSplitArgs& a, const float* __restrict__ xb, int base, __bf16* xs,
                                                int tid, Behind&& behind) {
  constexpr int OCTS = RuSplitCfg<C>::OCTS, ROW = RuSplitCfg<C>::ROW;
  const int nitems = (a.rows >> 2) * OCTS;
  f32x4 st[2][8];
#pragma unroll
  for (int it = 0; it < 2; ++it) {
    const int idx = tid + it * 256, oct = idx % OCTS, grp = idx / OCTS;
    const int t = base + grp * 4;
    const float* __restrict__ src = xb + (size_t)(oct * 8) * a.T + t;
    const bool in = idx < nitems && (!CHECKED || (t >= 0 && t < a.T));
#pragma unroll
    for (int j = 0; j < 8; ++j) {
      f32x4 v = {0.f, 0.f, 0.f, 0.f};
      if (in) v = *reinterpret_cast<const f32x4*>(src + (size_t)j * a.T);
      st[it][j] = v;
    }
  }
  behind();
#pragma unroll
  for (int it = 0; it < 2; ++it) {
    const int idx = tid + it * 256, oct = idx % OCTS, grp = idx / OCTS;
    if (idx < nitems) {
#pragma unroll
      for (int e = 0; e < 4; ++e) {
        float v[8];
#pragma unroll
        for (int j = 0; j < 8; ++j) {
          const float s = st[it][j][e];
          v[j] = s > 0.f ? s : s * a.slope1;
        }
        split3_store<8>(v, xs + (grp * 4 + e) * ROW + oct * 8, a.plane);
        __builtin_amdgcn_sched_barrier(0);
      }
    }
  }
}

template <int C, int TILE>
__device__ __forceinline__ void ru_request(bf16x8 (&wf)[3], const bf16x8* __restrict__ w, long part_stride, unsigned wrow,
                                           int h) {
  using Cfg = RuSplitCfg<C>;
  split_step_request(wf, w, part_stride, wrow + split_step_rows<TILE>(Cfg::CHUNKS, Cfg::M_PAD, SplitStepId{0, 0, 0}, h));
}
template <int C, int TILE, bool XFIRST>
__device__ __forceinline__ void ru_contract(bf16x8 (&wf)[3], const bf16x8* __restrict__ w, long part_stride, unsigned wrow,
                                            const __bf16* bl, int plane, int tap_step, int taps, int h,
                                            typename Mfma<TILE>::acc_t (&acc)[32 / TILE][64 / TILE]) {
  using Cfg = RuSplitCfg<C>;
  constexpr int HL = 64 / TILE, KSTEPS = KC / (8 * HL), TM = 32 / TILE, TN = 64 / TILE;
  SplitStepId step{0, 0, 0};
#pragma unroll 1
  for (int s = 0; s < Cfg::CHUNKS * taps * KSTEPS; ++s) {
    const SplitStepId next = split_step_successor(step, Cfg::CHUNKS, taps, KSTEPS);
    split_step_streamed<TILE, TM, TN, Cfg::ROW, XFIRST>(
        wf, w, part_stride, wrow + split_step_rows<TILE>(Cfg::CHUNKS, Cfg::M_PAD, step, h),
        wrow + split_step_rows<TILE>(Cfg::CHUNKS, Cfg::M_PAD, next, h), bl, step.tap * tap_step,
        step.chunk * KC + split_step_off<TILE>(step, h), plane, acc);
    step = next;
  }
}

template <int TILE>
__device__ __forceinline__ int ru_out_slot(int wave_n, int h, int n) {
  constexpr int HL = 64 / TILE, NG = TILE * TILE / 256;
  return wave_n * 64 + (n / NG) * TILE + 4 * h + 4 * HL * (n % NG);
}

template <int C, int TILE, bool RAGGED>
__global__ __launch_bounds__(256, 2) void resunit_split_kernel(RuSplitArgsOf<RAGGED> a) {
  using Cfg = RuSplitCfg<C>;
  constexpr int WAVES_N = Cfg::WAVES_N, ROW = Cfg::ROW, H = Cfg::H;
  constexpr int HL = 64 / TILE, TM = 32 / TILE, TN = 64 / TILE, NREG = TILE * TILE / 64, NG = NREG / 4;
  typedef typename Mfma<TILE>::acc_t acc_t;
  extern __shared__ __attribute__((aligned(16))) unsigned char smem[];
  __bf16* xs = reinterpret_cast<__bf16*>(smem);

  const int tid = threadIdx.x, lane = tid & 63;
  const int wave = __builtin_amdgcn_readfirstlane(tid >> 6);
  const int wave_m = wave / WAVES_N, wave_n = wave % WAVES_N;
  const int r = lane & (TILE - 1), h = lane / TILE;
  const int b = blockIdx.y;
  const int t0 = blockIdx.x * a.bn_out;
  const int base = t0 - a.hla;
  const int T = a.T;
  const bool pair = a.w2 != nullptr;
  const float* __restrict__ xb = a.x + (size_t)b * C * T;
  int Tv = T;
  if constexpr (RAGGED) {
    const long end = (long)a.frames[b] * a.rate;
    Tv = end < 0 ? 0 : end < T ? (int)end : T;
    if (t0 >= Tv) {
      const int quads = (T - t0 < a.bn_out ? T - t0 : a.bn_out) >> 2;
      for (int i = tid; i < C * quads; i += 256)
        *reinterpret_cast<f32x4*>(a.y + ((size_t)b * C + i / quads) * T + t0 + 4 * (i % quads)) = f32x4{0.f, 0.f, 0.f, 0.f};
      return;
    }
  }

  const unsigned wrow = wave_m * 32 + r;
  bf16x8 wf[3];
  ru_request<C, TILE>(wf, a.w1, a.part_stride, wrow, h);

  constexpr int NV = TN * NG;
  const bool has2 = a.add2 != nullptr;
  f32x4 res[TM][NV], ad2[TM][NV];
  auto request_values = [&](const float* __restrict__ src, f32x4 (&dst)[TM][NV]) {
    __builtin_amdgcn_sched_barrier(0);
#pragma unroll
    for (int mi = 0; mi < TM; ++mi) {
      const float* __restrict__ rowp = src + ((size_t)b * C + wave_m * 32 + mi * TILE + r) * T;
#pragma unroll
      for (int n = 0; n < NV; ++n) {
        const int slot = ru_out_slot<TILE>(wave_n, h, n);
        const bool ok = slot < a.bn_out && t0 + slot < T;
        dst[mi][n] = *reinterpret_cast<const f32x4*>(rowp + (ok ? t0 + slot : t0));
      }
    }
    __builtin_amdgcn_sched_barrier(0);
  };
#pragma unroll
  for (int mi = 0; mi < TM; ++mi)
#pragma unroll
    for (int n = 0; n < NV; ++n) ad2[mi][n] = f32x4{0.f, 0.f, 0.f, 0.f};
  const float* __restrict__ bias_p = pair ? a.b2 : a.b1;
  const bool has_b1 = a.b1 != nullptr, has_bias = bias_p != nullptr;
  f32x4 bias_h[TM][NG];
  float bias_y[TM];
#pragma unroll
  for (int mi = 0; mi < TM; ++mi) {
    bias_y[mi] = 0.f;
#pragma unroll
    for (int g = 0; g < NG; ++g) bias_h[mi][g] = f32x4{0.f, 0.f, 0.f, 0.f};
  }
  auto behind_window = [&] {
    request_values(a.x, res);
    if (!pair && has2) request_values(a.add2, ad2);
#pragma unroll
    for (int mi = 0; mi < TM; ++mi) {
      if (has_bias) bias_y[mi] = bias_p[wave_m * 32 + mi * TILE + r];
      if (pair && has_b1) {
#pragma unroll
        for (int g = 0; g < NG; ++g)
#pragma unroll
          for (int e = 0; e < 4; ++e) bias_h[mi][g][e] = a.b1[wave_m * 32 + mi * TILE + 4 * h + 4 * HL * g + e];
      }
    }
    __builtin_amdgcn_sched_barrier(0);
  };
  if (base >= 0 && base + a.rows <= T)
    ru_stage_window<C, false>(a, xb, base, xs, tid, behind_window);
  else
    ru_stage_window<C, true>(a, xb, base, xs, tid, behind_window);

  acc_t acc[TM][TN];
#pragma unroll
  for (int mi = 0; mi < TM; ++mi)
#pragma unroll
    for (int ni = 0; ni < TN; ++ni)
#pragma unroll
      for (int i = 0; i < NREG; ++i) acc[mi][ni][i] = 0.f;
  __syncthreads();

  if (pair) {
    ru_contract<C, TILE, false>(wf, a.w1, a.part_stride, wrow, xs + (wave_n * 64 + r + a.sh) * ROW, a.plane, a.d1, a.k,
                                h, acc);
    ru_request<C, TILE>(wf, a.w2, a.part_stride, wrow, h);
    if (has2) request_values(a.add2, ad2);
    __syncthreads();
#pragma unroll
    for (int mi = 0; mi < TM; ++mi)
#pragma unroll
      for (int g = 0; g < NG; ++g) {
        const int c = wave_m * 32 + mi * TILE + 4 * h + 4 * HL * g;
        const f32x4 bias = bias_h[mi][g];
#pragma unroll
        for (int ni = 0; ni < TN; ++ni) {
          const int m = wave_n * 64 + ni * TILE + r;
          const int th = t0 - a.p2 + m;
          const bool inside = th >= 0 && th < Tv;
          float v[4];
#pragma unroll
          for (int e = 0; e < 4; ++e) {
            v[e] = acc[mi][ni][4 * g + e];
            if (has_b1) v[e] += bias[e];
            v[e] = v[e] > 0.f ? v[e] : v[e] * a.slope2;
            v[e] = inside ? v[e] : 0.f;
            acc[mi][ni][4 * g + e] = 0.f;
          }
          split3_store<4>(v, xs + m * ROW + c, a.plane);
        }
      }
    for (int i = tid; i < (a.k - 1) * Cfg::OCTS; i += 256) {
      bf16x8 z;
#pragma unroll
      for (int j = 0; j < 8; ++j) z[j] = (__bf16)0.f;
      __bf16* dst = xs + (H + i / Cfg::OCTS) * ROW + (i % Cfg::OCTS) * 8;
      *reinterpret_cast<bf16x8*>(dst) = z;
      *reinterpret_cast<bf16x8*>(dst + a.plane) = z;
      *reinterpret_cast<bf16x8*>(dst + 2 * a.plane) = z;
    }
    __syncthreads();
    ru_contract<C, TILE, true>(wf, a.w2, a.part_stride, wrow, xs + (wave_n * 64 + r) * ROW, a.plane, 1, a.k, h,
                               acc);
  } else {
    ru_contract<C, TILE, true>(wf, a.w1, a.part_stride, wrow, xs + (wave_n * 64 + r + a.sh) * ROW, a.plane, a.d1, a.k,
                               h, acc);
  }

#pragma unroll
  for (int mi = 0; mi < TM; ++mi) {
    const int c = wave_m * 32 + mi * TILE + r;
    const size_t row = ((size_t)b * C + c) * T;
    int t[NV];
    bool ok[NV];
#pragma unroll
    for (int n = 0; n < NV; ++n) {
      const int slot = ru_out_slot<TILE>(wave_n, h, n);
      ok[n] = slot < a.bn_out && t0 + slot < T;
      t[n] = ok[n] ? t0 + slot : t0;
    }
    const f32x4(&t1)[NV] = res[mi];
    const f32x4(&t2)[NV] = ad2[mi];
    f32x4 v[NV];
    const float bias = bias_y[mi];
#pragma unroll
    for (int n = 0; n < NV; ++n)
#pragma unroll
      for (int e = 0; e < 4; ++e) v[n][e] = acc[mi][n / NG][(n % NG) * 4 + e];
    if (has_bias) {
#pragma unroll
      for (int n = 0; n < NV; ++n) v[n] += bias;
    }
#pragma unroll
    for (int n = 0; n < NV; ++n) v[n] += t1[n];
    if (has2) {
#pragma unroll
      for (int n = 0; n < NV; ++n) v[n] += t2[n];
    }
    if (a.out_div != 1.0f) {
#pragma unroll
      for (int n = 0; n < NV; ++n) v[n] = v[n] / a.out_div;
    }
    if constexpr (RAGGED) {
#pragma unroll
      for (int n = 0; n < NV; ++n)
        if (t[n] >= Tv) v[n] = f32x4{0.f, 0.f, 0.f, 0.f};
    }
#pragma unroll
    for (int n = 0; n < NV; ++n)
      if (ok[n]) *reinterpret_cast<f32x4*>(a.y + row + t[n]) = v[n];
  }
}

struct RuSplitGeom {
  int hla, sh, p2, bn_out, rows, tiles;
  size_t lds;
};

static int ru_split_geometry(const pwg_resunit_desc* d, RuSplitGeom* g) {
  PWG_REQUIRE(d != nullptr, PWG_ERR_NULL, "resunit_split: NULL descriptor");
  const int C = d->channels;
  PWG_REQUIRE(C == 32 || C == 64, PWG_ERR_UNSUPPORTED, "resunit_split: channels = %d (only 32 and 64)", C);
  PWG_REQUIRE(d->kernel >= 1 && (d->kernel & 1) == 1, PWG_ERR_UNSUPPORTED, "resunit_split: kernel = %d (only odd sizes)",
              d->kernel);
  PWG_REQUIRE(d->dilation >= 1, PWG_ERR_UNSUPPORTED, "resunit_split: dilation = %d", d->dilation);
  PWG_REQUIRE(d->batch >= 1 && d->batch <= 65535, PWG_ERR_UNSUPPORTED, "resunit_split: batch = %d (1 .. 65535)", d->batch);
  PWG_REQUIRE(d->t >= 4 && (d->t & 3) == 0, PWG_ERR_UNSUPPORTED, "resunit_split: t = %d (a positive multiple of 4)", d->t);
  PWG_REQUIRE(d->slope1 > 0.f && d->slope1 < 1.f, PWG_ERR_UNSUPPORTED, "resunit_split: slope1 = %g (0 < slope < 1)",
              (double)d->slope1);
  PWG_REQUIRE(!d->has_conv2 || (d->slope2 > 0.f && d->slope2 < 1.f), PWG_ERR_UNSUPPORTED,
              "resunit_split: slope2 = %g (0 < slope < 1)", (double)d->slope2);
  const int k = d->kernel, H = C == 32 ? RuSplitCfg<32>::H : RuSplitCfg<64>::H;
  PWG_REQUIRE((long)(k - 1) * d->dilation < (1 << 20), PWG_ERR_UNSUPPORTED, "resunit_split: receptive field too long");
  g->p2 = d->has_conv2 ? (k - 1) / 2 : 0;
  const int hl = (k - 1) / 2 * d->dilation + g->p2;
  g->hla = round_up(hl, 4);
  g->sh = g->hla - hl;
  g->bn_out = d->has_conv2 ? ((H - (k - 1)) & ~3) : H;
  PWG_REQUIRE(g->bn_out >= 64, PWG_ERR_UNSUPPORTED, "resunit_split: kernel = %d leaves %d outputs per tile", k, g->bn_out);
  g->rows = round_up(H + (k - 1) * d->dilation + g->sh, 4);
  g->lds = (size_t)3 * g->rows * (C + 8) * sizeof(__bf16);
  PWG_REQUIRE(g->lds <= kRuSplitMaxLds && (g->rows / 4) * (C / 8) <= 512, PWG_ERR_UNSUPPORTED,
              "resunit_split: the window (kernel %d, dilation %d) needs %zu B of LDS", k, d->dilation, g->lds);
  g->tiles = ceil_div(d->t, g->bn_out);
  return PWG_OK;
}

template <bool RAGGED>
static int ru_split_forward(const pwg_resunit_desc* d, const float* x, const void* w1, const float* b1, const void* w2,
                            const float* b2, const float* add2, float* y, int mfma_shape, hipStream_t stream,
                            const int32_t* frames = nullptr, int rate = 0) {
  RuSplitGeom g;
  const int rc = ru_split_geometry(d, &g);
  if (rc != PWG_OK) return rc;
  PWG_REQUIRE(x && w1 && y, PWG_ERR_NULL, "resunit_split_forward: NULL pointer");
  PWG_REQUIRE(x != y, PWG_ERR_BAD_SHAPE, "resunit_split_forward: y must not alias x (tiles read their neighbours' halo)");
  PWG_REQUIRE((d->has_conv2 != 0) == (w2 != nullptr), PWG_ERR_BAD_SHAPE,
              "resunit_split_forward: has_conv2 = %d but w2_packed is %s", d->has_conv2, w2 ? "given" : "NULL");
  auto al16 = [](const void* p) { return (reinterpret_cast<uintptr_t>(p) & 15u) == 0; };
  PWG_REQUIRE(al16(x) && al16(y) && al16(add2), PWG_ERR_BAD_SHAPE,
              "resunit_split_forward: x / y / add2 must be 16-B aligned");
  PWG_REQUIRE(al16(w1) && al16(w2), PWG_ERR_BAD_SHAPE, "resunit_split_forward: the weight images must be 16-B aligned");
  PWG_REQUIRE(mfma_shape == 16 || mfma_shape == 32, PWG_ERR_BAD_SHAPE, "resunit_split_forward: mfma_shape = %d (16 or 32)",
              mfma_shape);
  const int C = d->channels;
  RuSplitArgsOf<RAGGED> a;
  a.x = x;
  a.w1 = static_cast<const bf16x8*>(w1);
  a.b1 = b1;
  a.w2 = static_cast<const bf16x8*>(w2);
  a.b2 = b2;
  a.add2 = add2;
  a.y = y;
  a.T = d->t, a.k = d->kernel, a.d1 = d->dilation;
  a.bn_out = g.bn_out, a.hla = g.hla, a.sh = g.sh, a.p2 = g.p2, a.rows = g.rows;
  a.plane = g.rows * (C + 8);
  a.part_stride = image_elems(d->kernel, image_chunks(C), image_m_pad(C)) / 8;
  PWG_REQUIRE(split_image_addressable(a.part_stride * 8), PWG_ERR_UNSUPPORTED, "resunit_split_forward: weight image too large");
  a.slope1 = d->slope1, a.slope2 = d->slope2, a.out_div = d->out_div;
  if constexpr (RAGGED) a.frames = frames, a.rate = rate;
  void (*kern)(RuSplitArgsOf<RAGGED>) =
      C == 32 ? (mfma_shape == 32 ? resunit_split_kernel<32, 32, RAGGED> : resunit_split_kernel<32, 16, RAGGED>)
              : (mfma_shape == 32 ? resunit_split_kernel<64, 32, RAGGED> : resunit_split_kernel<64, 16, RAGGED>);
  if (g.lds > kConvMaxLds && !lds_limit_is_set(reinterpret_cast<const void*>(kern), g.lds)) {
    hipError_t e = hipFuncSetAttribute(reinterpret_cast<const void*>(kern), hipFuncAttributeMaxDynamicSharedMemorySize,
                                       (int)g.lds);
    PWG_REQUIRE(e == hipSuccess, PWG_ERR_LAUNCH, "resunit_split_forward: cannot raise LDS limit to %zu: %s", g.lds,
                hipGetErrorString(e));
  }
  const double elems = (double)d->batch * C * d->t;
  const double flops = 2.0 * elems * C * d->kernel * (d->has_conv2 ? 2 : 1);
  const double bytes = 4.0 * (elems * (2 + (add2 != nullptr)) + (d->has_conv2 ? 2 : 1) * (double)C * C * d->kernel);
  maybe_poison_lds(stream);
  {
    ProfScope prof(stream,
                   RAGGED ? prof_shape_name("resunit_split_ragged_kernel",
                                            "resunit_split_ragged_kernel B%d C%d T%d k%d d%d pair%d", d->batch, C, d->t,
                                            d->kernel, d->dilation, d->has_conv2)
                          : prof_shape_name("resunit_split_kernel", "resunit_split_kernel B%d C%d T%d k%d d%d pair%d",
                                            d->batch, C, d->t, d->kernel, d->dilation, d->has_conv2),
                   flops, bytes);
    hipLaunchKernelGGL(kern, dim3(g.tiles, d->batch), dim3(256), g.lds, stream, a);
  }
  PWG_CHECK_LAUNCH("resunit_split_forward");
  return PWG_OK;
}

constexpr int kDefaultMfmaShape = 16;

static int ru_split_ragged_rate(int rate) {
  PWG_REQUIRE(rate > 0 && (rate & 3) == 0, PWG_ERR_UNSUPPORTED,
              "resunit_split_ragged: rate = %d (a positive multiple of 4: an item ends between two values of four samples)",
              rate);
  return PWG_OK;
}

constexpr int kRbMaxUnits = 3;

struct RbSplitArgs {
  RuSplitArgs u;
  const bf16x8* w1[kRbMaxUnits];
  const bf16x8* w2[kRbMaxUnits];
  const float* b1[kRbMaxUnits];
  const float* b2[kRbMaxUnits];
  int d[kRbMaxUnits];
  float slope1[kRbMaxUnits], slope2[kRbMaxUnits];
  int n_units;
  int margin;
  int edge;
};

template <int C, int TILE>
__global__ __launch_bounds__(256, 2) void resblock_split_kernel(RbSplitArgs a) {
  using Cfg = RuSplitCfg<C>;
  constexpr int WAVES_N = Cfg::WAVES_N, ROW = Cfg::ROW, H = Cfg::H;
  constexpr int HL = 64 / TILE, TM = 32 / TILE, TN = 64 / TILE, NREG = TILE * TILE / 64, NG = NREG / 4;
  typedef typename Mfma<TILE>::acc_t acc_t;
  extern __shared__ __attribute__((aligned(16))) unsigned char smem[];
  __bf16* xs = reinterpret_cast<__bf16*>(smem);

  const int tid = threadIdx.x, lane = tid & 63;
  const int wave = __builtin_amdgcn_readfirstlane(tid >> 6);
  const int wave_m = wave / WAVES_N, wave_n = wave % WAVES_N;
  const int r = lane & (TILE - 1), h = lane / TILE;
  const int b = blockIdx.y;
  const int t0 = blockIdx.x * a.u.bn_out;
  const int f0 = t0 - a.edge;
  const int T = a.u.T, k = a.u.k, p = (k - 1) / 2, plane = a.u.plane, margin = a.margin;
  const long part_stride = a.u.part_stride;
  const float* __restrict__ xb = a.u.x + (size_t)b * C * T;
  __bf16* fr = xs + margin * ROW;

  const unsigned wrow = wave_m * 32 + r;
  bf16x8 wf[3];
  ru_request<C, TILE>(wf, a.w1[0], part_stride, wrow, h);

  for (int i = tid; i < 2 * margin * Cfg::OCTS; i += 256) {
    bf16x8 z;
#pragma unroll
    for (int j = 0; j < 8; ++j) z[j] = (__bf16)0.f;
    const int row = i / Cfg::OCTS;
    __bf16* dst = xs + (row < margin ? row : H + row) * ROW + (i % Cfg::OCTS) * 8;
    *reinterpret_cast<bf16x8*>(dst) = z;
    *reinterpret_cast<bf16x8*>(dst + plane) = z;
    *reinterpret_cast<bf16x8*>(dst + 2 * plane) = z;
  }

  constexpr int NV = TN * NG;
  const bool has2 = a.u.add2 != nullptr;
  f32x4 res[TM][NV], ad2[TM][NV];
  auto request_values = [&](const float* __restrict__ src, f32x4 (&dst)[TM][NV], bool stored_only) {
    __builtin_amdgcn_sched_barrier(0);
#pragma unroll
    for (int mi = 0; mi < TM; ++mi) {
      const float* __restrict__ rowp = src + ((size_t)b * C + wave_m * 32 + mi * TILE + r) * T;
#pragma unroll
      for (int n = 0; n < NV; ++n) {
        const int slot = ru_out_slot<TILE>(wave_n, h, n), t = f0 + slot;
        const bool ok = t >= 0 && t < T && (!stored_only || (slot >= a.edge && slot < a.edge + a.u.bn_out));
        dst[mi][n] = *reinterpret_cast<const f32x4*>(rowp + (ok ? t : t0));
      }
    }
    __builtin_amdgcn_sched_barrier(0);
  };
#pragma unroll
  for (int mi = 0; mi < TM; ++mi)
#pragma unroll
    for (int n = 0; n < NV; ++n) ad2[mi][n] = f32x4{0.f, 0.f, 0.f, 0.f};
  auto behind_window = [&] { request_values(a.u.x, res, false); };
  if (f0 >= 0 && f0 + H <= T)
    ru_stage_window<C, false>(a.u, xb, f0, fr, tid, behind_window);
  else
    ru_stage_window<C, true>(a.u, xb, f0, fr, tid, behind_window);

  acc_t acc[TM][TN];
#pragma unroll
  for (int mi = 0; mi < TM; ++mi)
#pragma unroll
    for (int ni = 0; ni < TN; ++ni)
#pragma unroll
      for (int i = 0; i < NREG; ++i) acc[mi][ni][i] = 0.f;

#pragma unroll 1
  for (int u = 0; u < a.n_units; ++u) {
    const bool last = u + 1 == a.n_units;
    const int d1 = a.d[u];
    const float* __restrict__ b1p = a.b1[u];
    const float* __restrict__ b2p = a.b2[u];
    const bool has_b1 = b1p != nullptr, has_b2 = b2p != nullptr;
    f32x4 bias_h[TM][NG];
    float bias_y[TM];
#pragma unroll
    for (int mi = 0; mi < TM; ++mi) {
      bias_y[mi] = has_b2 ? b2p[wave_m * 32 + mi * TILE + r] : 0.f;
#pragma unroll
      for (int g = 0; g < NG; ++g)
#pragma unroll
        for (int e = 0; e < 4; ++e)
          bias_h[mi][g][e] = has_b1 ? b1p[wave_m * 32 + mi * TILE + 4 * h + 4 * HL * g + e] : 0.f;
    }
    __syncthreads();

    ru_contract<C, TILE, false>(wf, a.w1[u], part_stride, wrow, fr + (wave_n * 64 + r - p * d1) * ROW, plane, d1, k, h,
                                acc);
    ru_request<C, TILE>(wf, a.w2[u], part_stride, wrow, h);
    if (last && has2) request_values(a.u.add2, ad2, true);
    __syncthreads();
#pragma unroll
    for (int mi = 0; mi < TM; ++mi)
#pragma unroll
      for (int g = 0; g < NG; ++g) {
        const int c = wave_m * 32 + mi * TILE + 4 * h + 4 * HL * g;
        const f32x4 bias = bias_h[mi][g];
#pragma unroll
        for (int ni = 0; ni < TN; ++ni) {
          const int m = wave_n * 64 + ni * TILE + r;
          const int th = f0 + m;
          const bool inside = th >= 0 && th < T;
          float v[4];
#pragma unroll
          for (int e = 0; e < 4; ++e) {
            v[e] = acc[mi][ni][4 * g + e];
            if (has_b1) v[e] += bias[e];
            v[e] = v[e] > 0.f ? v[e] : v[e] * a.slope2[u];
            v[e] = inside ? v[e] : 0.f;
            acc[mi][ni][4 * g + e] = 0.f;
          }
          split3_store<4>(v, fr + m * ROW + c, plane);
        }
      }
    __syncthreads();
    ru_contract<C, TILE, true>(wf, a.w2[u], part_stride, wrow, fr + (wave_n * 64 + r - p) * ROW, plane, 1, k, h, acc);
    if (last) break;

    ru_request<C, TILE>(wf, a.w1[u + 1], part_stride, wrow, h);
    const float slope = a.slope1[u + 1];
    __syncthreads();
#pragma unroll
    for (int mi = 0; mi < TM; ++mi) {
      const int c = wave_m * 32 + mi * TILE + r;
      const float bias = bias_y[mi];
#pragma unroll
      for (int n = 0; n < NV; ++n) {
        const int slot = ru_out_slot<TILE>(wave_n, h, n), t = f0 + slot;
        const bool inside = t >= 0 && t < T;
        f32x4 v;
#pragma unroll
        for (int e = 0; e < 4; ++e) {
          v[e] = acc[mi][n / NG][(n % NG) * 4 + e];
          acc[mi][n / NG][(n % NG) * 4 + e] = 0.f;
        }
        if (has_b2) v += bias;
        v += res[mi][n];
        if (!inside) v = f32x4{0.f, 0.f, 0.f, 0.f};
        res[mi][n] = v;
#pragma unroll
        for (int e = 0; e < 4; ++e) {
          const float s = v[e] > 0.f ? v[e] : v[e] * slope;
          __bf16 hi, mid, lo;
          split3(s, hi, mid, lo);
          __bf16* dst = fr + (slot + e) * ROW + c;
          dst[0] = hi;
          dst[plane] = mid;
          dst[2 * plane] = lo;
        }
      }
    }
  }

  const float* __restrict__ b2l = a.b2[a.n_units - 1];
#pragma unroll
  for (int mi = 0; mi < TM; ++mi) {
    const int c = wave_m * 32 + mi * TILE + r;
    const size_t row = ((size_t)b * C + c) * T;
    f32x4 v[NV];
#pragma unroll
    for (int n = 0; n < NV; ++n)
#pragma unroll
      for (int e = 0; e < 4; ++e) v[n][e] = acc[mi][n / NG][(n % NG) * 4 + e];
    if (b2l != nullptr) {
      const float bias = b2l[c];
#pragma unroll
      for (int n = 0; n < NV; ++n) v[n] += bias;
    }
#pragma unroll
    for (int n = 0; n < NV; ++n) v[n] += res[mi][n];
    if (has2) {
#pragma unroll
      for (int n = 0; n < NV; ++n) v[n] += ad2[mi][n];
    }
    if (a.u.out_div != 1.0f) {
#pragma unroll
      for (int n = 0; n < NV; ++n) v[n] = v[n] / a.u.out_div;
    }
#pragma unroll
    for (int n = 0; n < NV; ++n) {
      const int slot = ru_out_slot<TILE>(wave_n, h, n), t = f0 + slot;
      if (slot >= a.edge && slot < a.edge + a.u.bn_out && t < T) *reinterpret_cast<f32x4*>(a.u.y + row + t) = v[n];
    }
  }
}

struct RbSplitGeom {
  int H, edge, margin, bn_out, rows, tiles;
  size_t lds;
};

static int rb_split_geometry(const pwg_resunit_desc* d, int n_units, const int32_t* dilations, RbSplitGeom* g) {
  PWG_REQUIRE(d != nullptr && dilations != nullptr, PWG_ERR_NULL, "resblock_split: NULL descriptor or dilations");
  PWG_REQUIRE(n_units >= 1 && n_units <= kRbMaxUnits, PWG_ERR_UNSUPPORTED, "resblock_split: n_units = %d (1 .. %d)",
              n_units, kRbMaxUnits);
  PWG_REQUIRE(d->has_conv2, PWG_ERR_UNSUPPORTED, "resblock_split: single-convolution units are not chained");
  int dmax = 1, sum = 0;
  for (int u = 0; u < n_units; ++u) {
    pwg_resunit_desc du = *d;
    du.dilation = dilations[u];
    RuSplitGeom gu;
    const int rc = ru_split_geometry(&du, &gu);
    if (rc != PWG_OK) return rc;
    dmax = dilations[u] > dmax ? dilations[u] : dmax;
    sum += (d->kernel - 1) / 2 * (dilations[u] + 1);
  }
  const int C = d->channels;
  g->H = C == 32 ? RuSplitCfg<32>::H : RuSplitCfg<64>::H;
  g->edge = round_up(sum, 4);
  g->margin = (d->kernel - 1) / 2 * dmax;
  g->bn_out = g->H - 2 * g->edge;
  PWG_REQUIRE(g->bn_out >= g->H / 2, PWG_ERR_UNSUPPORTED,
              "resblock_split: kernel = %d over %d units leaves %d outputs per frame of %d columns", d->kernel, n_units,
              g->bn_out, g->H);
  g->rows = g->H + 2 * g->margin;
  g->lds = (size_t)3 * g->rows * (C + 8) * sizeof(__bf16);
  PWG_REQUIRE(g->lds <= kRuSplitMaxLds, PWG_ERR_UNSUPPORTED, "resblock_split: the planes (kernel %d) need %zu B of LDS",
              d->kernel, g->lds);
  g->tiles = ceil_div(d->t, g->bn_out);
  return PWG_OK;
}

}
}

using namespace pwg;

extern "C" int pwg_resblock_split_supported(const pwg_resunit_desc* d, int32_t n_units, const int32_t* dilations) {
  RbSplitGeom g;
  return rb_split_geometry(d, n_units, dilations, &g) == PWG_OK ? 1 : 0;
}

extern "C" int pwg_resblock_split_frame(const pwg_resunit_desc* d, int32_t n_units, const int32_t* dilations,
                                        int32_t* out) {
  RbSplitGeom g;
  const int rc = rb_split_geometry(d, n_units, dilations, &g);
  if (rc != PWG_OK) return rc;
  PWG_REQUIRE(out != nullptr, PWG_ERR_NULL, "resblock_split_frame: NULL out");
  out[0] = g.H, out[1] = g.bn_out, out[2] = g.edge, out[3] = g.margin, out[4] = (int32_t)g.lds, out[5] = g.tiles;
  return PWG_OK;
}

extern "C" int pwg_resblock_split_forward_cfg(const pwg_resunit_desc* d, int32_t n_units, const int32_t* dilations,
                                              const float* slopes1, const float* slopes2, const float* x,
                                              const void* const* w1_split, const float* const* b1,
                                              const void* const* w2_split, const float* const* b2, const float* add2,
                                              float* y, int32_t mfma_shape, void* stream_) {
  hipStream_t stream = (hipStream_t)stream_;
  RbSplitGeom g;
  const int rc = rb_split_geometry(d, n_units, dilations, &g);
  if (rc != PWG_OK) return rc;
  PWG_REQUIRE(x && y && w1_split && w2_split && b1 && b2 && slopes1 && slopes2, PWG_ERR_NULL,
              "resblock_split_forward: NULL pointer");
  PWG_REQUIRE(x != y, PWG_ERR_BAD_SHAPE, "resblock_split_forward: y must not alias x (frames read their neighbours' columns)");
  auto al16 = [](const void* p) { return (reinterpret_cast<uintptr_t>(p) & 15u) == 0; };
  PWG_REQUIRE(al16(x) && al16(y) && al16(add2), PWG_ERR_BAD_SHAPE,
              "resblock_split_forward: x / y / add2 must be 16-B aligned");
  PWG_REQUIRE(mfma_shape == 16 || mfma_shape == 32, PWG_ERR_BAD_SHAPE, "resblock_split_forward: mfma_shape = %d (16 or 32)",
              mfma_shape);
  const int C = d->channels;
  RbSplitArgs a = {};
  for (int u = 0; u < n_units; ++u) {
    PWG_REQUIRE(w1_split[u] && w2_split[u], PWG_ERR_NULL, "resblock_split_forward: NULL weight image of unit %d", u);
    PWG_REQUIRE(al16(w1_split[u]) && al16(w2_split[u]), PWG_ERR_BAD_SHAPE,
                "resblock_split_forward: the weight images must be 16-B aligned");
    PWG_REQUIRE(slopes1[u] > 0.f && slopes1[u] < 1.f && slopes2[u] > 0.f && slopes2[u] < 1.f, PWG_ERR_UNSUPPORTED,
                "resblock_split_forward: slopes of unit %d = %g, %g (0 < slope < 1)", u, (double)slopes1[u],
                (double)slopes2[u]);
    a.w1[u] = static_cast<const bf16x8*>(w1_split[u]);
    a.w2[u] = static_cast<const bf16x8*>(w2_split[u]);
    a.b1[u] = b1[u], a.b2[u] = b2[u];
    a.d[u] = dilations[u];
    a.slope1[u] = slopes1[u], a.slope2[u] = slopes2[u];
  }
  a.n_units = n_units, a.margin = g.margin, a.edge = g.edge;
  a.u.x = x, a.u.add2 = add2, a.u.y = y;
  a.u.T = d->t, a.u.k = d->kernel, a.u.d1 = dilations[0];
  a.u.bn_out = g.bn_out, a.u.rows = g.H;
  a.u.plane = g.rows * (C + 8);
  a.u.part_stride = image_elems(d->kernel, image_chunks(C), image_m_pad(C)) / 8;
  PWG_REQUIRE(split_image_addressable(a.u.part_stride * 8), PWG_ERR_UNSUPPORTED,
              "resblock_split_forward: weight image too large");
  a.u.slope1 = slopes1[0], a.u.slope2 = slopes2[0], a.u.out_div = d->out_div;
  void (*kern)(RbSplitArgs) = C == 32 ? (mfma_shape == 32 ? resblock_split_kernel<32, 32> : resblock_split_kernel<32, 16>)
                                      : (mfma_shape == 32 ? resblock_split_kernel<64, 32> : resblock_split_kernel<64, 16>);
  if (g.lds > kConvMaxLds && !lds_limit_is_set(reinterpret_cast<const void*>(kern), g.lds)) {
    hipError_t e = hipFuncSetAttribute(reinterpret_cast<const void*>(kern), hipFuncAttributeMaxDynamicSharedMemorySize,
                                       (int)g.lds);
    PWG_REQUIRE(e == hipSuccess, PWG_ERR_LAUNCH, "resblock_split_forward: cannot raise LDS limit to %zu: %s", g.lds,
                hipGetErrorString(e));
  }
  const double elems = (double)d->batch * C * d->t;
  const double flops = 2.0 * elems * C * d->kernel * 2 * n_units;
  const double bytes = 4.0 * (elems * (2 * n_units + (add2 != nullptr)) + 2.0 * n_units * C * C * d->kernel);
  maybe_poison_lds(stream);
  {
    ProfScope prof(stream,
                   prof_shape_name("resblock_split_kernel", "resblock_split_kernel B%d C%d T%d k%d n%d", d->batch, C, d->t,
                                   d->kernel, n_units),
                   flops, bytes);
    hipLaunchKernelGGL(kern, dim3(g.tiles, d->batch), dim3(256), g.lds, stream, a);
  }
  PWG_CHECK_LAUNCH("resblock_split_forward");
  return PWG_OK;
}

extern "C" int pwg_resunit_split_supported(const pwg_resunit_desc* d) {
  RuSplitGeom g;
  return ru_split_geometry(d, &g) == PWG_OK ? 1 : 0;
}

extern "C" int pwg_resunit_split_forward(const pwg_resunit_desc* d, const float* x, const void* w1_split, const float* b1,
                                         const void* w2_split, const float* b2, const float* add2, float* y,
                                         void* stream) {
  return ru_split_forward<false>(d, x, w1_split, b1, w2_split, b2, add2, y, kDefaultMfmaShape, (hipStream_t)stream);
}

extern "C" int pwg_resunit_split_forward_cfg(const pwg_resunit_desc* d, const float* x, const void* w1_split,
                                             const float* b1, const void* w2_split, const float* b2, const float* add2,
                                             float* y, int32_t mfma_shape, void* stream) {
  return ru_split_forward<false>(d, x, w1_split, b1, w2_split, b2, add2, y, mfma_shape, (hipStream_t)stream);
}

extern "C" int pwg_resunit_split_ragged_supported(const pwg_resunit_desc* d, int32_t rate) {
  RuSplitGeom g;
  return ru_split_geometry(d, &g) == PWG_OK && ru_split_ragged_rate(rate) == PWG_OK ? 1 : 0;
}

extern "C" int pwg_resunit_split_forward_ragged(const pwg_resunit_desc* d, const float* x, const void* w1_split,
                                                const float* b1, const void* w2_split, const float* b2,
                                                const float* add2, float* y, int32_t mfma_shape, const int32_t* frames,
                                                int32_t rate, void* stream) {
  PWG_REQUIRE(frames != nullptr, PWG_ERR_NULL, "resunit_split_forward_ragged: NULL frames table");
  PWG_REQUIRE((reinterpret_cast<uintptr_t>(frames) & 3u) == 0, PWG_ERR_BAD_SHAPE,
              "resunit_split_forward_ragged: the frames table must be 4-B aligned");
  const int rc = ru_split_ragged_rate(rate);
  if (rc != PWG_OK) return rc;
  return ru_split_forward<true>(d, x, w1_split, b1, w2_split, b2, add2, y, mfma_shape, (hipStream_t)stream, frames, rate);
}
```

parallelwavegan_amd/ops.py:

```python
import ctypes

import torch

from . import _lib
from ._lib import ConvDesc, ResUnitDesc, WaveNetDesc

ACT = {None: _lib.PWG_ACT_NONE, "none": _lib.PWG_ACT_NONE, "leaky_relu": _lib.PWG_ACT_LEAKY_RELU,
       "tanh": _lib.PWG_ACT_TANH, "relu": _lib.PWG_ACT_RELU}
PAD = {"zero": _lib.PWG_PAD_ZERO, "reflect": _lib.PWG_PAD_REFLECT, "replicate": _lib.PWG_PAD_REPLICATE}


PARAM_EPOCH = [0]


def bump_param_epoch():
    PARAM_EPOCH[0] += 1


def cache_epoch():
    return PARAM_EPOCH[0]


def param_epoch(p):
    return getattr(p, "_pwg_epoch", 0)
# ... 134 lines not shown
    assert x.numel() == desc.batch * desc.c_in * desc.t_in * desc.width, (tuple(x.shape), desc.batch, desc.c_in, desc.t_in)
    assert out.numel() == desc.batch * desc.c_out * desc.t_out * desc.width
    ws, ws_n = _workspace(_lib.lib().pwg_conv1d_forward_workspace_floats(ctypes.byref(desc)), x.device)
    _lib.check(_lib.lib().pwg_conv1d_forward(ctypes.byref(desc), _ptr(x), _ptr(w_packed), _ptr(bias), _ptr(add1),
                                             _ptr(add2), _ptr(out), _ptr(ws), ws_n, _stream()), "conv1d_forward")
    return out


def conv1d_bf16_supported(desc):
    return bool(_lib.lib().pwg_conv1d_bf16_supported(ctypes.byref(desc)))


def _zero_padded(desc):
    if desc.pad_mode == PAD["zero"]:
        return desc
    desc = ConvDesc.from_buffer_copy(desc)
    desc.pad_mode = PAD["zero"]
    return desc


def _pack_weight_mfma(kind, desc, w, scale, op="conv1d"):
    _require_device(w, scale)
    n = getattr(_lib.lib(), f"pwg_{op}_{kind}_packed_weight_bytes")(ctypes.byref(desc))
    if n == 0:
        _lib.check(-1, f"{op}_{kind}_packed_weight_bytes")
    out = torch.empty(n, device=w.device, dtype=torch.uint8)
    pack = getattr(_lib.lib(), f"pwg_{op}_{kind}_pack_weight")
    _lib.check(pack(ctypes.byref(desc), _ptr(w), _ptr(scale), _ptr(out), _stream()), f"{op}_{kind}_pack_weight")
    return out


def _conv1d_forward_mfma(kind, desc, image_desc, x, w_packed, bias, add1, add2, out, cfg, op="conv1d", entry="cfg"):
    name = f"{op}_forward_{kind}"
    _require_device(x, bias, add1, add2, out)
    if not w_packed.is_cuda or w_packed.dtype != torch.uint8:
        raise RuntimeError(f"{name}: w_packed must be the device image of pack_weight_{kind}")
    if out is None:
        out = torch.empty((desc.batch, desc.c_out, desc.t_out), device=x.device, dtype=torch.float32)
    assert x.numel() == desc.batch * desc.c_in * desc.t_in, (tuple(x.shape), desc.batch, desc.c_in, desc.t_in)
    assert out.numel() == desc.batch * desc.c_out * desc.t_out
    image_bytes = getattr(_lib.lib(), f"pwg_{op}_{kind}_packed_weight_bytes")(ctypes.byref(image_desc))
    if image_bytes == 0:
        _lib.check(-1, f"{op}_{kind}_packed_weight_bytes")
    assert w_packed.numel() == image_bytes, f"{name}: w_packed is not this layer's {kind} image"
    for t in (add1, add2):
        assert t is None or t.numel() == out.numel()
    args = (ctypes.byref(desc), _ptr(x), _ptr(w_packed), _ptr(bias), _ptr(add1), _ptr(add2), _ptr(out))
    if cfg is None:
        rc = getattr(_lib.lib(), f"pwg_{op}_{kind}_forward")(*args, None, 0, _stream())
    else:
        rc = getattr(_lib.lib(), f"pwg_{op}_{kind}_forward_{entry}")(*args, *cfg, _stream())
    _lib.check(rc, name)
    return out


def pack_weight_bf16(desc, w, scale=None):
    return _pack_weight_mfma("bf16", _zero_padded(desc), w, scale)


def conv1d_forward_bf16(desc, x, w_packed, bias=None, add1=None, add2=None, out=None, mfma_shape=None):
    return _conv1d_forward_mfma("bf16", desc, _zero_padded(desc), x, w_packed, bias, add1, add2, out,
                                None if mfma_shape is None else (int(mfma_shape),))


def conv1d_split_supported(desc):
    return bool(_lib.lib().pwg_conv1d_split_supported(ctypes.byref(desc)))


def pack_weight_split(desc, w, scale=None):
    return _pack_weight_mfma("split", desc, w, scale)


STEP_FORMS = {1: "resident", 2: "streamed"}


def conv1d_split_step_form(desc):
    form = _lib.lib().pwg_conv1d_split_step_form(ctypes.byref(desc))
    if form == 0:
        _lib.check(-1, "conv1d_split_step_form")
    return STEP_FORMS[form]


WINDOW_FORMS = {1: "staged", 2: "prefetched"}


def conv1d_split_window_form(desc):
    form = _lib.lib().pwg_conv1d_split_window_form(ctypes.byref(desc))
    if form == 0:
        _lib.check(-1, "conv1d_split_window_form")
    return WINDOW_FORMS[form]


def conv1d_forward_split(desc, x, w_packed, bias=None, add1=None, add2=None, out=None, mfma_shape=None, tile_mode=0,
                         step_form=0, window_form=0):
    if window_form:
        cfg = (int(mfma_shape or 16), int(tile_mode), int(step_form), int(window_form))
        return _conv1d_forward_mfma("split", desc, desc, x, w_packed, bias, add1, add2, out, cfg, entry="window")
    if step_form:
        cfg = (int(mfma_shape or 16), int(tile_mode), int(step_form))
        return _conv1d_forward_mfma("split", desc, desc, x, w_packed, bias, add1, add2, out, cfg, entry="step")
    cfg = None if mfma_shape is None and not tile_mode else (int(mfma_shape or 16), int(tile_mode))
    return _conv1d_forward_mfma("split", desc, desc, x, w_packed, bias, add1, add2, out, cfg)


def convtr1d_split_supported(desc):
    return bool(_lib.lib().pwg_convtr1d_split_supported(ctypes.byref(desc)))


def pack_weight_split_transposed(desc, w, scale=None):
    return _pack_weight_mfma("split", desc, w, scale, op="convtr1d")


def conv1d_forward_split_transposed(desc, x, w_packed, bias=None, add1=None, add2=None, out=None, mfma_shape=None,
                                    tile_mode=0):
    cfg = None if mfma_shape is None and not tile_mode else (int(mfma_shape or 16), int(tile_mode))
    return _conv1d_forward_mfma("split", desc, desc, x, w_packed, bias, add1, add2, out, cfg, op="convtr1d")


def conv1d_stream_supported(desc):
    return bool(_lib.lib().pwg_conv1d_stream_supported(ctypes.byref(desc)))


def conv1d_stream_hist_floats(desc):
    return _lib.lib().pwg_conv1d_stream_hist_floats(ctypes.byref(desc))


def conv1d_stream_plan(desc):
    out = (ctypes.c_int32 * 5)()
    _lib.check(_lib.lib().pwg_conv1d_stream_plan(ctypes.byref(desc), out), "conv1d_stream_plan")
    return dict(tile=(out[0], out[1]), grid=(out[2], out[3], out[4]))


def _conv1d_stream_out(desc, x, hist_in, hist_out, add1, add2, out):
    if out is None:
        out = torch.empty((desc.batch, desc.c_out, desc.t_out), device=x.device, dtype=torch.float32)
    assert x.numel() == desc.batch * desc.c_in * desc.t_in, (tuple(x.shape), desc.batch, desc.c_in, desc.t_in)
    assert out.numel() == desc.batch * desc.c_out * desc.t_out
    n_hist = conv1d_stream_hist_floats(desc)
    for t in (hist_in, hist_out):
        assert t is None or t.numel() == n_hist, (tuple(t.shape), n_hist)
    for t in (add1, add2):
        assert t is None or t.numel() == out.numel()
    return out


def conv1d_stream_forward(desc, x, hist_in, hist_out, w_packed, bias=None, add1=None, add2=None, out=None):
    _require_device(x, hist_in, hist_out, w_packed, bias, add1, add2, out)
    out = _conv1d_stream_out(desc, x, hist_in, hist_out, add1, add2, out)
    _lib.check(_lib.lib().pwg_conv1d_stream_forward(ctypes.byref(desc), _ptr(x), _ptr(hist_in), _ptr(hist_out),
                                                    _ptr(w_packed), _ptr(bias), _ptr(add1), _ptr(add2), _ptr(out),
                                                    _stream()), "conv1d_stream_forward")
    return out


def conv1d_stream_delayed_supported(desc, delay1=0, delay2=0):
    return bool(_lib.lib().pwg_conv1d_stream_delayed_supported(ctypes.byref(desc), int(delay1), int(delay2)))


def conv1d_stream_delayed_forward(desc, x, hist_in, hist_out, w_packed, bias=None, add1=None, add1_hist=(None, None),
                                  delay1=0, add2=None, add2_hist=(None, None), delay2=0, valid=None, out=None):
    _require_device(w_packed)
    return _conv1d_stream_delayed(_lib.lib().pwg_conv1d_stream_delayed_forward, "conv1d_stream_delayed_forward", desc, x, hist_in, hist_out, w_packed, bias, add1,
                                  add1_hist, delay1, add2, add2_hist, delay2, valid, out)


def _conv1d_stream_delayed(entry, name, desc, x, hist_in, hist_out, image, bias, add1, add1_hist, delay1, add2, add2_hist,
                           delay2, valid, out, slots=None):
    flat = (add1_hist[0], add1_hist[1], add2_hist[0], add2_hist[1])
    _require_device(x, hist_in, hist_out, bias, add1, add2, out, *flat)
    out = _conv1d_stream_out(desc, x, hist_in, hist_out, add1, add2, out)
    for delay, (h_in, h_out) in ((delay1, add1_hist), (delay2, add2_hist)):
        for t in (h_in, h_out):
            assert t is None or t.numel() == desc.batch * desc.c_out * delay, (tuple(t.shape), delay)
    if slots is None:
        lo, hi = (0, desc.t_out) if valid is None else valid
        position = (int(lo), int(hi))
    else:
        table, rate, delay = slots
        if table is None or not table.is_cuda or table.dtype != torch.int32 or not table.is_contiguous():
            raise RuntimeError(f"{name}: slots must be a contiguous int32 device tensor (the kernel reads it; there is no "
                               "CPU fallback path)")
        assert tuple(table.shape) == (desc.batch, SLOT_INTS), (tuple(table.shape), desc.batch)
        position = (_ptr(table), int(rate), int(delay))
    _lib.check(entry(
        ctypes.byref(desc), _ptr(x), _ptr(hist_in), _ptr(hist_out), _ptr(image), _ptr(bias),
        _ptr(add1), _ptr(flat[0]), _ptr(flat[1]), int(delay1), _ptr(add2), _ptr(flat[2]), _ptr(flat[3]), int(delay2),
        *position, _ptr(out), _stream()), name)
    return out


SLOT_INTS = 4
SLOT_PAUSED, SLOT_LEFT_KNOWN = 1, 2


def conv1d_stream_slots_forward(desc, x, hist_in, hist_out, w_packed, bias=None, add1=None, add1_hist=(None, None),
                                delay1=0, add2=None, add2_hist=(None, None), delay2=0, slots=None, rate=1, delay=0,
                                out=None):
    _require_device(w_packed)
    return _conv1d_stream_delayed(_lib.lib().pwg_conv1d_stream_slots_forward, "conv1d_stream_slots_forward", desc, x,
                                  hist_in, hist_out, w_packed, bias, add1, add1_hist, delay1, add2, add2_hist, delay2, None,
                                  out, (slots, rate, delay))


def conv1d_stream_slots_forward_bf16(desc, x, hist_in, hist_out, w_packed_bf16, bias=None, add1=None,
                                     add1_hist=(None, None), delay1=0, add2=None, add2_hist=(None, None), delay2=0,
                                     slots=None, rate=1, delay=0, out=None):
    _check_stream_image_bf16("conv1d_stream_slots_forward_bf16", desc, w_packed_bf16)
    return _conv1d_stream_delayed(_lib.lib().pwg_conv1d_stream_slots_forward_bf16, "conv1d_stream_slots_forward_bf16", desc,
                                  x, hist_in, hist_out, w_packed_bf16, bias, add1, add1_hist, delay1, add2, add2_hist,
                                  delay2, None, out, (slots, rate, delay))


def conv1d_stream_mirrored_supported(desc):
    return bool(_lib.lib().pwg_conv1d_stream_mirrored_supported(ctypes.byref(desc)))


_I32_MAX = 2 ** 31 - 1


def conv1d_stream_mirrored_forward(desc, x, hist_in, hist_out, w_packed, bias=None, in_window=(0, None), valid=None,
                                   out=None):
    _require_device(x, hist_in, hist_out, w_packed, bias, out)
    out = _conv1d_stream_out(desc, x, hist_in, hist_out, None, None, out)
    lo, hi = (0, desc.t_out) if valid is None else valid
    in_lo, in_hi = in_window
    clamp = lambda v: max(-_I32_MAX, min(_I32_MAX, int(v)))
    _lib.check(_lib.lib().pwg_conv1d_stream_mirrored_forward(
        ctypes.byref(desc), _ptr(x), _ptr(hist_in), _ptr(hist_out), _ptr(w_packed), _ptr(bias), _ptr(out), clamp(in_lo),
        _I32_MAX if in_hi is None else clamp(in_hi), int(lo), int(hi), _stream()), "conv1d_stream_mirrored_forward")
    return out


def conv1d_stream_bf16_supported(desc):
    return bool(_lib.lib().pwg_conv1d_stream_bf16_supported(ctypes.byref(desc)))


def _check_stream_image_bf16(name, desc, w_packed_bf16):
    if not w_packed_bf16.is_cuda or w_packed_bf16.dtype != torch.uint8:
        raise RuntimeError(f"{name}: w_packed_bf16 must be the device image of pack_weight_bf16")
    assert w_packed_bf16.numel() == _lib.lib().pwg_conv1d_bf16_packed_weight_bytes(ctypes.byref(_zero_padded(desc))), \
        f"{name}: w_packed_bf16 is not this layer's bf16 image"


def conv1d_stream_forward_bf16(desc, x, hist_in, hist_out, w_packed_bf16, bias=None, add1=None, add2=None, out=None):
    _require_device(x, hist_in, hist_out, bias, add1, add2, out)
    _check_stream_image_bf16("conv1d_stream_forward_bf16", desc, w_packed_bf16)
    out = _conv1d_stream_out(desc, x, hist_in, hist_out, add1, add2, out)
    _lib.check(_lib.lib().pwg_conv1d_stream_bf16_forward(ctypes.byref(desc), _ptr(x), _ptr(hist_in), _ptr(hist_out),
                                                         _ptr(w_packed_bf16), _ptr(bias), _ptr(add1), _ptr(add2),
                                                         _ptr(out), _stream()), "conv1d_stream_bf16_forward")
    return out


def conv1d_stream_bf16_delayed_supported(desc, delay1=0, delay2=0):
    return bool(_lib.lib().pwg_conv1d_stream_bf16_delayed_supported(ctypes.byref(desc), int(delay1), int(delay2)))


def conv1d_stream_delayed_forward_bf16(desc, x, hist_in, hist_out, w_packed_bf16, bias=None, add1=None,
                                       add1_hist=(None, None), delay1=0, add2=None, add2_hist=(None, None), delay2=0,
                                       valid=None, out=None):
    _check_stream_image_bf16("conv1d_stream_delayed_forward_bf16", desc, w_packed_bf16)
    return _conv1d_stream_delayed(_lib.lib().pwg_conv1d_stream_bf16_delayed_forward, "conv1d_stream_bf16_delayed_forward",
                                  desc, x, hist_in, hist_out, w_packed_bf16, bias, add1, add1_hist, delay1, add2,
                                  add2_hist, delay2, valid, out)


def make_resunit_desc(batch, channels, t, kernel, dilation, has_conv2=True, slope1=0.1, slope2=0.1, out_div=1.0):
    return ResUnitDesc(int(batch), int(channels), int(t), int(kernel), int(dilation), int(bool(has_conv2)),
                       float(slope1), float(slope2), float(out_div))


def resunit_supported(desc):
    return bool(_lib.lib().pwg_resunit_supported(ctypes.byref(desc)))


def resunit_profitable(desc):
    return bool(_lib.lib().pwg_resunit_profitable(ctypes.byref(desc)))


def resunit_pack_weight(w, scale=None):
    _require_device(w, scale)
    c, k = w.shape[0], w.shape[2]
    assert w.shape[1] == c
    out = torch.empty(_lib.lib().pwg_resunit_packed_weight_floats(c, k), device=w.device, dtype=torch.float32)
    _lib.check(_lib.lib().pwg_resunit_pack_weight(c, k, _ptr(w), _ptr(scale), _ptr(out), _stream()),
               "resunit_pack_weight")
    return out


def resunit_forward(desc, x, w1_packed, b1, w2_packed=None, b2=None, add2=None, out=None):
    _require_device(x, w1_packed, b1, w2_packed, b2, add2, out)
    assert x.numel() == desc.batch * desc.channels * desc.t
    if out is None:
        out = torch.empty_like(x)
    _lib.check(_lib.lib().pwg_resunit_forward(ctypes.byref(desc), _ptr(x), _ptr(w1_packed), _ptr(b1), _ptr(w2_packed),
                                              _ptr(b2), _ptr(add2), _ptr(out), _stream()), "resunit_forward")
    return out


def resunit_split_supported(desc):
    return bool(_lib.lib().pwg_resunit_split_supported(ctypes.byref(desc)))


def resunit_forward_split(desc, x, w1_split, b1, w2_split=None, b2=None, add2=None, out=None, mfma_shape=None):
    _require_device(x, b1, b2, add2, out)
    for w in (w1_split, w2_split):
        if w is not None and (not w.is_cuda or w.dtype != torch.uint8):
            raise RuntimeError("resunit_forward_split: the weights must be device images of pack_weight_split")
    assert x.numel() == desc.batch * desc.channels * desc.t
    image_bytes = 6 * desc.kernel * desc.channels * desc.channels
    for w in (w1_split, w2_split):
        assert w is None or w.numel() == image_bytes, "resunit_forward_split: not this unit's split image"
    assert add2 is None or add2.numel() == x.numel()
    if out is None:
        out = torch.empty_like(x)
    args = (ctypes.byref(desc), _ptr(x), _ptr(w1_split), _ptr(b1), _ptr(w2_split), _ptr(b2), _ptr(add2), _ptr(out))
    if mfma_shape is None:
        rc = _lib.lib().pwg_resunit_split_forward(*args, _stream())
    else:
        rc = _lib.lib().pwg_resunit_split_forward_cfg(*args, int(mfma_shape), _stream())
    _lib.check(rc, "resunit_split_forward")
    return out


def resblock_split_supported(desc, dilations):
    dil = (ctypes.c_int32 * len(dilations))(*[int(v) for v in dilations])
    return bool(_lib.lib().pwg_resblock_split_supported(ctypes.byref(desc), len(dilations), dil))


def resblock_split_frame(desc, dilations):
    dil = (ctypes.c_int32 * len(dilations))(*[int(v) for v in dilations])
    out = (ctypes.c_int32 * 6)()
    _lib.check(_lib.lib().pwg_resblock_split_frame(ctypes.byref(desc), len(dilations), dil, out), "resblock_split_frame")
    return dict(zip(("H", "bn_out", "edge", "margin", "lds", "tiles"), (int(v) for v in out)))


def resblock_forward_split(desc, x, dilations, slopes1, slopes2, w1_split, b1, w2_split, b2, add2=None, out=None,
                           mfma_shape=None):
    n = len(dilations)
    assert len(slopes1) == len(slopes2) == len(w1_split) == len(b1) == len(w2_split) == len(b2) == n
    _require_device(x, add2, out, *b1, *b2)
    image_bytes = 6 * desc.kernel * desc.channels * desc.channels
    for w in (*w1_split, *w2_split):
        if w is None or not w.is_cuda or w.dtype != torch.uint8:
            raise RuntimeError("resblock_forward_split: the weights must be device images of pack_weight_split")
        assert w.numel() == image_bytes, "resblock_forward_split: not this unit's split image"
    assert x.numel() == desc.batch * desc.channels * desc.t
    assert add2 is None or add2.numel() == x.numel()
    if out is None:
        out = torch.empty_like(x)

    def ptrs(ts):
        return (ctypes.c_void_p * n)(*[None if t is None else t.data_ptr() for t in ts])

    _lib.check(_lib.lib().pwg_resblock_split_forward_cfg(
        ctypes.byref(desc), n, (ctypes.c_int32 * n)(*[int(v) for v in dilations]),
        (ctypes.c_float * n)(*[float(v) for v in slopes1]), (ctypes.c_float * n)(*[float(v) for v in slopes2]), _ptr(x),
        ptrs(w1_split), ptrs(b1), ptrs(w2_split), ptrs(b2), _ptr(add2), _ptr(out),
        16 if mfma_shape is None else int(mfma_shape), _stream()), "resblock_split_forward")
    return out


def _require_frames(frames, batch, what):
    if not isinstance(frames, torch.Tensor) or not frames.is_cuda:
        raise RuntimeError(f"{what}: the frames table must be a device tensor; there is no CPU fallback path")
    if frames.dtype != torch.int32 or tuple(frames.shape) != (int(batch),) or not frames.is_contiguous():
        raise RuntimeError(f"{what}: the frames table must be a contiguous int32 tensor of shape ({int(batch)},), got "
                           f"{frames.dtype} {tuple(frames.shape)}")


def zero_tail(y, frames, rate):
    _require_device(y)
    if y.dim() != 3:
        raise RuntimeError(f"zero_tail: expected a (B, C, T) tensor, got {tuple(y.shape)}")
    _require_frames(frames, y.shape[0], "zero_tail")
    _lib.check(_lib.lib().pwg_zero_tail(_ptr(y), _ptr(frames), y.shape[0], y.shape[1], y.shape[2], int(rate), _stream()),
               "zero_tail")
    return y


def mirror_tail(y, frames, rate, pad):
    _require_device(y)
    if y.dim() != 3:
        raise RuntimeError(f"mirror_tail: expected a (B, C, T) tensor, got {tuple(y.shape)}")
    _require_frames(frames, y.shape[0], "mirror_tail")
    _lib.check(_lib.lib().pwg_mirror_tail(_ptr(y), _ptr(frames), y.shape[0], y.shape[1], y.shape[2], int(rate), int(pad),
                                          _stream()), "mirror_tail")
    return y


def resunit_split_ragged_supported(desc, rate):
    return bool(_lib.lib().pwg_resunit_split_ragged_supported(ctypes.byref(desc), int(rate)))


def resunit_forward_split_ragged(desc, x, frames, rate, w1_split, b1, w2_split=None, b2=None, add2=None, out=None,
                                 mfma_shape=16):
    _require_device(x, b1, b2, add2, out)
    for w in (w1_split, w2_split):
        if w is not None and (not w.is_cuda or w.dtype != torch.uint8):
            raise RuntimeError("resunit_forward_split_ragged: the weights must be device images of pack_weight_split")
    _require_frames(frames, desc.batch, "resunit_forward_split_ragged")
    assert x.numel() == desc.batch * desc.channels * desc.t
    image_bytes = 6 * desc.kernel * desc.channels * desc.channels
    for w in (w1_split, w2_split):
        assert w is None or w.numel() == image_bytes, "resunit_forward_split_ragged: not this unit's split image"
    assert add2 is None or add2.numel() == x.numel()
    if out is None:
        out = torch.empty_like(x)
    _lib.check(_lib.lib().pwg_resunit_split_forward_ragged(
        ctypes.byref(desc), _ptr(x), _ptr(w1_split), _ptr(b1), _ptr(w2_split), _ptr(b2), _ptr(add2), _ptr(out),
        int(mfma_shape), _ptr(frames), int(rate), _stream()), "resunit_split_forward_ragged")
    return out


def resstack_supported(channels, t, dilation):
    return bool(_lib.lib().pwg_resstack_supported(int(channels), int(t), int(dilation)))


def resstack_pack_weight(w1, s1, w2, s2, ws, ss):
    _require_device(w1, s1, w2, s2, ws, ss)
    c = w1.shape[0]
    n = _lib.lib().pwg_resstack_packed_weight_floats(c)
    if n == 0:
        _lib.check(-1, "resstack_packed_weight_floats")
    out = torch.empty(n, device=w1.device, dtype=torch.float32)
    _lib.check(_lib.lib().pwg_resstack_pack_weight(c, _ptr(w1), _ptr(s1), _ptr(w2), _ptr(s2), _ptr(ws), _ptr(ss), _ptr(out),
                                                   _stream()), "resstack_pack_weight")
    return out


def resstack_forward(x, w_packed, dilation, slope, b1=None, b2=None, bs=None, save_h=False):
    _require_device(x, w_packed, b1, b2, bs)
    b, c, t = x.shape
    y = torch.empty_like(x)
    h = torch.empty_like(x) if save_h else None
    _lib.check(_lib.lib().pwg_resstack_forward(b, c, t, int(dilation), float(slope), _ptr(x), _ptr(w_packed), _ptr(b1), _ptr(b2),
                                               _ptr(bs), _ptr(y), _ptr(h), _stream()), "resstack_forward")
    return y, h


def resstack_ragged_supported(channels, t, dilation, rate):
    return bool(_lib.lib().pwg_resstack_ragged_supported(int(channels), int(t), int(dilation), int(rate)))


def resstack_forward_ragged(x, frames, rate, w_packed, dilation, slope, b1=None, b2=None, bs=None, out=None):
    _require_device(x, w_packed, b1, b2, bs, out)
    if x.dim() != 3 or not x.is_contiguous():
        raise RuntimeError(f"resstack_forward_ragged: expected a contiguous (B, C, T) tensor, got {tuple(x.shape)}")
    b, c, t = x.shape
    _require_frames(frames, b, "resstack_forward_ragged")
    if out is None:
        out = torch.empty_like(x)
    assert out.shape == x.shape and out.is_contiguous()
    _lib.check(_lib.lib().pwg_resstack_forward_ragged(b, c, t, int(dilation), float(slope), _ptr(x), _ptr(w_packed),
                                                      _ptr(b1), _ptr(b2), _ptr(bs), _ptr(out), _ptr(frames), int(rate),
                                                      _stream()), "resstack_forward_ragged")
    return out


def resstack_pack_weight_bwd(w1, s1, w2, s2, ws, ss):
    _require_device(w1, s1, w2, s2, ws, ss)
    c = w1.shape[0]
    n = _lib.lib().pwg_resstack_packed_weight_floats(c)
    if n == 0:
        _lib.check(-1, "resstack_packed_weight_floats")
    out = torch.empty(n, device=w1.device, dtype=torch.float32)
    _lib.check(_lib.lib().pwg_resstack_pack_weight_bwd(c, _ptr(w1), _ptr(s1), _ptr(w2), _ptr(s2), _ptr(ws), _ptr(ss),
                                                       _ptr(out), _stream()), "resstack_pack_weight_bwd")
    return out


def resstack_backward_data(dy, h, x, w_packed_bwd, dilation, slope):
    _require_device(dy, h, x, w_packed_bwd)
    b, c, t = x.shape
    dh = torch.empty_like(x)
    dxp = torch.empty((b, c, t + 2 * int(dilation)), device=x.device, dtype=torch.float32)
    _lib.check(_lib.lib().pwg_resstack_backward_data(b, c, t, int(dilation), float(slope), _ptr(dy), _ptr(h), _ptr(x),
                                                     _ptr(w_packed_bwd), _ptr(dh), _ptr(dxp), _stream()),
               "resstack_backward_data")
    return dh, dxp


def make_wavenet_desc(batch, t, dilation, residual_channels=64, gate_channels=128, skip_channels=64, aux_channels=80,
                      kernel=3, causal=False, out_mul=1.0, skip_mul=1.0):
    return WaveNetDesc(int(batch), int(t), int(residual_channels), int(gate_channels), int(skip_channels),
                       int(aux_channels), int(kernel), int(dilation), int(bool(causal)), float(out_mul), float(skip_mul))


def wavenet_layer_supported(desc):
    return bool(_lib.lib().pwg_wavenet_layer_supported(ctypes.byref(desc)))


def wavenet_pack_weights(desc, w_dil, s_dil, w_aux, s_aux, w_skip, s_skip, w_out, s_out):
    _require_device(w_dil, s_dil, w_aux, s_aux, w_skip, s_skip, w_out, s_out)
    out = torch.empty(_lib.lib().pwg_wavenet_packed_weight_floats(ctypes.byref(desc)), device=w_dil.device,
                      dtype=torch.float32)
    _lib.check(_lib.lib().pwg_wavenet_pack_weights(ctypes.byref(desc), _ptr(w_dil), _ptr(s_dil), _ptr(w_aux), _ptr(s_aux),
                                                   _ptr(w_skip), _ptr(s_skip), _ptr(w_out), _ptr(s_out), _ptr(out),
                                                   _stream()), "wavenet_pack_weights")
    return out


def wavenet_layer_forward(desc, x, c, skips, packed, b_dil, b_skip, b_out, save=False, skips_out=None):
    _require_device(x, c, skips, packed, b_dil, b_skip, b_out, skips_out)
    x_out = torch.empty_like(x)
    if skips_out is None:
        skips_out = torch.empty_like(x)
    z = torch.empty((x.shape[0], desc.gate_channels, x.shape[2]), device=x.device, dtype=torch.float32) if save else None
    g = torch.empty_like(x) if save else None
    _lib.check(_lib.lib().pwg_wavenet_layer_forward(ctypes.byref(desc), _ptr(x), _ptr(c), _ptr(skips), _ptr(packed),
                                                    _ptr(b_dil), _ptr(b_skip), _ptr(b_out), _ptr(x_out), _ptr(skips_out),
                                                    _ptr(z), _ptr(g), _stream()), "wavenet_layer_forward")
    return x_out, skips_out, z, g


def wavenet_stream_supported(desc):
    return bool(_lib.lib().pwg_wavenet_stream_supported(ctypes.byref(desc)))


def wavenet_stream_hist_floats(desc):
    return _lib.lib().pwg_wavenet_stream_hist_floats(ctypes.byref(desc))


def wavenet_stream_forward(desc, x, c, skips, hist_in, hist_out, packed, b_dil, b_skip, b_out, skips_out=None):
    _require_device(x, c, skips, hist_in, hist_out, packed, b_dil, b_skip, b_out, skips_out)
    assert x.numel() == desc.batch * desc.residual_channels * desc.t, (tuple(x.shape), desc.batch, desc.t)
    assert c.numel() == desc.batch * desc.aux_channels * desc.t, (tuple(c.shape), desc.batch, desc.t)
    n_hist = wavenet_stream_hist_floats(desc)
    for t in (hist_in, hist_out):
        assert t is None or n_hist == 0 or t.numel() == n_hist, (tuple(t.shape), n_hist)
    x_out = torch.empty_like(x)
    if skips_out is None:
        skips_out = torch.empty_like(x)
    for t in (skips, skips_out):
        assert t is None or t.numel() == x.numel()
    _lib.check(_lib.lib().pwg_wavenet_stream_forward(ctypes.byref(desc), _ptr(x), _ptr(c), _ptr(skips), _ptr(hist_in),
                                                     _ptr(hist_out), _ptr(packed), _ptr(b_dil), _ptr(b_skip), _ptr(b_out),
                                                     _ptr(x_out), _ptr(skips_out), _stream()), "wavenet_stream_forward")
    return x_out, skips_out


def stretch_conv_stream(x, hist_in, hist_out, w, scale, freq_kernel=1, act=None, slope=0.0):
    x = x.contiguous()
    w = w.reshape(-1).contiguous()
    _require_device(x, hist_in, hist_out, w)
    b, ch, n = x.shape
    assert w.numel() == (2 * scale + 1) * freq_kernel, (w.numel(), scale, freq_kernel)
    for t in (hist_in, hist_out):
        assert t is None or t.numel() == b * ch * 2, tuple(t.shape)
    y = torch.empty((b, ch, n * scale), device=x.device, dtype=torch.float32)
    _lib.check(_lib.lib().pwg_stretch_conv_stream(_ptr(x), _ptr(hist_in), _ptr(hist_out), _ptr(w), _ptr(y), b * ch, n,
                                                  int(scale), int(freq_kernel), ACT[act], float(slope), _stream()),
               "stretch_conv_stream")
    return y


def wavenet_stream_delayed_supported(desc, c_delay=0):
    return bool(_lib.lib().pwg_wavenet_stream_delayed_supported(ctypes.byref(desc), int(c_delay)))


def wavenet_stream_delayed_hist_floats(desc):
    return _lib.lib().pwg_wavenet_stream_delayed_hist_floats(ctypes.byref(desc))


def wavenet_stream_delayed_forward(desc, x, c, c_line, c_delay, skips, skip_line, hist_in, hist_out, packed, b_dil, b_skip,
                                   b_out, valid=None):
    line_in, line_out = skip_line if skips is not None else (None, None)
    _require_device(x, c, c_line, skips, line_in, line_out, hist_in, hist_out, packed, b_dil, b_skip, b_out)
    assert x.numel() == desc.batch * desc.residual_channels * desc.t, (tuple(x.shape), desc.batch, desc.t)
    assert c.numel() == desc.batch * desc.aux_channels * desc.t, (tuple(c.shape), desc.batch, desc.t)
    n_hist = wavenet_stream_delayed_hist_floats(desc)
    for t in (hist_in, hist_out):
        assert t is None or n_hist == 0 or t.numel() == n_hist, (tuple(t.shape), n_hist)
    for t in (line_in, line_out):
        assert t is None or t.numel() == desc.batch * desc.skip_channels * desc.dilation, tuple(t.shape)
    assert skips is None or skips.numel() == x.numel()
    c_cols = 0
    if c_line is not None:
        assert c_line.is_contiguous() and c_line.numel() % (desc.batch * desc.aux_channels) == 0, tuple(c_line.shape)
        c_cols = c_line.numel() // (desc.batch * desc.aux_channels)
    x_out, skips_out = torch.empty_like(x), torch.empty_like(x)
    lo, hi = (0, desc.t) if valid is None else valid
    _lib.check(_lib.lib().pwg_wavenet_stream_delayed_forward(
        ctypes.byref(desc), _ptr(x), _ptr(c), _ptr(c_line), c_cols, int(c_delay), _ptr(skips), _ptr(line_in), _ptr(line_out),
        _ptr(hist_in), _ptr(hist_out), _ptr(packed), _ptr(b_dil), _ptr(b_skip), _ptr(b_out), int(lo), int(hi), _ptr(x_out),
        _ptr(skips_out), _stream()), "wavenet_stream_delayed_forward")
    return x_out, skips_out


def stretch_conv_stream_delayed(x, hist_in, hist_out, w, scale, freq_kernel=1, act=None, slope=0.0, valid=None):
    x = x.contiguous()
    w = w.reshape(-1).contiguous()
    _require_device(x, hist_in, hist_out, w)
    b, ch, n = x.shape
    assert w.numel() == (2 * scale + 1) * freq_kernel, (w.numel(), scale, freq_kernel)
    for t in (hist_in, hist_out):
        assert t is None or t.numel() == b * ch * 2, tuple(t.shape)
    y = torch.empty((b, ch, n * scale), device=x.device, dtype=torch.float32)
    lo, hi = (0, n * scale) if valid is None else valid
    _lib.check(_lib.lib().pwg_stretch_conv_stream_delayed(_ptr(x), _ptr(hist_in), _ptr(hist_out), _ptr(w), _ptr(y), b * ch, n,
                                                          int(scale), int(freq_kernel), ACT[act], float(slope), int(lo),
                                                          int(hi), _stream()), "stretch_conv_stream_delayed")
    return y


def delay_line_forward(x, line_in, line_out, delayed=False):
    x = x.contiguous()
    _require_device(x, line_in, line_out)
    b, ch, n = x.shape
    L = line_out.shape[-1]
    for t in (line_in, line_out):
        assert t is None or (t.is_contiguous() and tuple(t.shape) == (b, ch, L)), (tuple(t.shape), (b, ch, L))
    out = torch.empty_like(x) if delayed else None
    _lib.check(_lib.lib().pwg_delay_line_forward(_ptr(x), _ptr(line_in), _ptr(line_out), _ptr(out), b * ch, n, L, _stream()),
               "delay_line_forward")
    return out



def _slot_table(name, slots, batch):
    if slots is None or not slots.is_cuda or slots.dtype != torch.int32 or not slots.is_contiguous():
        raise RuntimeError(f"{name}: slots must be a contiguous int32 device tensor (the kernel reads it; there is no CPU "
                           "fallback path)")
    assert tuple(slots.shape) == (batch, SLOT_INTS), (tuple(slots.shape), batch)
    return slots


def wavenet_stream_slots_forward(desc, x, c, c_line, c_delay, skips, skip_line, hist_in, hist_out, packed, b_dil, b_skip,
                                 b_out, slots=None, rate=1, delay=0, precision="fp32"):
    bf16 = precision == "bf16"
    name = "wavenet_stream_slots_forward_bf16" if bf16 else "wavenet_stream_slots_forward"
    line_in, line_out = skip_line if skips is not None else (None, None)
    _require_device(x, c, c_line, skips, line_in, line_out, hist_in, hist_out, b_dil, b_skip, b_out)
    if bf16:
        _bf16_stream_image(name, packed)
    else:
        _require_device(packed)
    _slot_table(name, slots, desc.batch)
    assert x.numel() == desc.batch * desc.residual_channels * desc.t, (tuple(x.shape), desc.batch, desc.t)
    assert c.numel() == desc.batch * desc.aux_channels * desc.t, (tuple(c.shape), desc.batch, desc.t)
    n_hist = wavenet_stream_delayed_hist_floats(desc)
    for t in (hist_in, hist_out):
        assert t is None or n_hist == 0 or t.numel() == n_hist, (tuple(t.shape), n_hist)
    for t in (line_in, line_out):
        assert t is None or t.numel() == desc.batch * desc.skip_channels * desc.dilation, tuple(t.shape)
    assert skips is None or skips.numel() == x.numel()
    c_cols = 0
    if c_line is not None:
        assert c_line.is_contiguous() and c_line.numel() % (desc.batch * desc.aux_channels) == 0, tuple(c_line.shape)
        c_cols = c_line.numel() // (desc.batch * desc.aux_channels)
    x_out, skips_out = torch.empty_like(x), torch.empty_like(x)
    entry = _lib.lib().pwg_wavenet_stream_slots_forward_bf16 if bf16 else _lib.lib().pwg_wavenet_stream_slots_forward
    _lib.check(entry(
        ctypes.byref(desc), _ptr(x), _ptr(c), _ptr(c_line), c_cols, int(c_delay), _ptr(skips), _ptr(line_in), _ptr(line_out),
        _ptr(hist_in), _ptr(hist_out), _ptr(packed), _ptr(b_dil), _ptr(b_skip), _ptr(b_out), _ptr(slots), int(rate),
        int(delay), _ptr(x_out), _ptr(skips_out), _stream()), name)
    return x_out, skips_out


def stretch_conv_stream_slots(x, hist_in, hist_out, w, scale, freq_kernel=1, act=None, slope=0.0, slots=None, rate=1,
                              delay=0):
    x = x.contiguous()
    w = w.reshape(-1).contiguous()
    _require_device(x, hist_in, hist_out, w)
    b, ch, n = x.shape
    _slot_table("stretch_conv_stream_slots", slots, b)
    assert w.numel() == (2 * scale + 1) * freq_kernel, (w.numel(), scale, freq_kernel)
    for t in (hist_in, hist_out):
        assert t is None or (t.is_contiguous() and t.numel() == b * ch * 2), tuple(t.shape)
    y = torch.empty((b, ch, n * scale), device=x.device, dtype=torch.float32)
    _lib.check(_lib.lib().pwg_stretch_conv_stream_slots(_ptr(x), _ptr(hist_in), _ptr(hist_out), _ptr(w), _ptr(y), b, ch, n,
                                                        int(scale), int(freq_kernel), ACT[act], float(slope), _ptr(slots),
                                                        int(rate), int(delay), _stream()), "stretch_conv_stream_slots")
    return y


def delay_line_slots_forward(x, line_in, line_out, slots, delayed=False):
    x = x.contiguous()
    _require_device(x, line_in, line_out)
    b, ch, n = x.shape
    _slot_table("delay_line_slots_forward", slots, b)
    L = line_out.shape[-1]
    for t in (line_in, line_out):
        assert t is None or (t.is_contiguous() and tuple(t.shape) == (b, ch, L)), (tuple(t.shape), (b, ch, L))
    out = torch.empty_like(x) if delayed else None
    _lib.check(_lib.lib().pwg_delay_line_slots_forward(_ptr(x), _ptr(line_in), _ptr(line_out), _ptr(out), b, ch, n, L,
                                                       _ptr(slots), _stream()), "delay_line_slots_forward")
    return out


def slot_seed_history(x, hist, slots):
    x = x.contiguous()
    _require_device(x, hist)
    b, ch, n = x.shape
    _slot_table("slot_seed_history", slots, b)
    assert hist is None or (hist.is_contiguous() and tuple(hist.shape[:2]) == (b, ch)), tuple(hist.shape)
    cols = 1 if hist is None else hist.shape[-1]
    _lib.check(_lib.lib().pwg_slot_seed_history(_ptr(x), _ptr(hist), b, ch, n, cols, _ptr(slots), _stream()),
               "slot_seed_history")
    return hist


def wavenet_bf16_supported(desc):
    return bool(_lib.lib().pwg_wavenet_bf16_supported(ctypes.byref(desc)))


def wavenet_bf16_packed_weight_bytes(desc):
    n = _lib.lib().pwg_wavenet_bf16_packed_weight_bytes(ctypes.byref(desc))
    if n == 0:
        _lib.check(-1, "wavenet_bf16_packed_weight_bytes")
    return n


def wavenet_bf16_pack_weights(desc, w_dil, s_dil, w_aux, s_aux, w_skip, s_skip, w_out, s_out):
# ... 334 lines not shown
```

Measured before the change: 86.42 million samples/s.

## Software-pipeline LDS activation plane loads in split residual-unit MFMA contraction

```diff
diff --git a/include/pwg_kernels.h b/include/pwg_kernels.h
--- a/include/pwg_kernels.h
+++ b/include/pwg_kernels.h
@@ -226,6 +226,19 @@
                                    const float* slopes1, const float* slopes2, const float* x,
                                    const void* const* w1_split, const float* const* b1, const void* const* w2_split,
                                    const float* const* b2, const float* add2, float* y, int32_t mfma_shape, void* stream);
+int pwg_resunit_split_plane_form(const pwg_resunit_desc* d, int32_t n_units);
+int pwg_resunit_split_forward_planes(const pwg_resunit_desc* d, const float* x, const void* w1_split, const float* b1,
+                                     const void* w2_split, const float* b2, const float* add2, float* y,
+                                     int32_t mfma_shape, int32_t plane_form, void* stream);
+int pwg_resunit_split_forward_ragged_planes(const pwg_resunit_desc* d, const float* x, const void* w1_split,
+                                            const float* b1, const void* w2_split, const float* b2, const float* add2,
+                                            float* y, int32_t mfma_shape, int32_t plane_form, const int32_t* frames,
+                                            int32_t rate, void* stream);
+int pwg_resblock_split_forward_planes(const pwg_resunit_desc* d, int32_t n_units, const int32_t* dilations,
+                                      const float* slopes1, const float* slopes2, const float* x,
+                                      const void* const* w1_split, const float* const* b1, const void* const* w2_split,
+                                      const float* const* b2, const float* add2, float* y, int32_t mfma_shape,
+                                      int32_t plane_form, void* stream);
 
 int pwg_resstack_supported(int32_t channels, int32_t t, int32_t dilation);
 size_t pwg_resstack_packed_weight_floats(int32_t channels);
diff --git a/parallelwavegan_amd/_lib.py b/parallelwavegan_amd/_lib.py
--- a/parallelwavegan_amd/_lib.py
+++ b/parallelwavegan_amd/_lib.py
@@ -203,6 +203,16 @@
                                                       ctypes.POINTER(ctypes.c_float), ctypes.POINTER(ctypes.c_float), _vp,
                                                       ctypes.POINTER(_vp), ctypes.POINTER(_vp), ctypes.POINTER(_vp),
                                                       ctypes.POINTER(_vp), _vp, _vp, _i32, _vp]),
+    "pwg_resunit_split_plane_form": (ctypes.c_int, [ctypes.POINTER(ResUnitDesc), _i32]),
+    "pwg_resunit_split_forward_planes": (ctypes.c_int, [ctypes.POINTER(ResUnitDesc), _vp, _vp, _vp, _vp, _vp, _vp, _vp,
+                                                        _i32, _i32, _vp]),
+    "pwg_resunit_split_forward_ragged_planes": (ctypes.c_int, [ctypes.POINTER(ResUnitDesc), _vp, _vp, _vp, _vp, _vp, _vp,
+                                                               _vp, _i32, _i32, _vp, _i32, _vp]),
+    "pwg_resblock_split_forward_planes": (ctypes.c_int, [ctypes.POINTER(ResUnitDesc), _i32, ctypes.POINTER(_i32),
+                                                         ctypes.POINTER(ctypes.c_float), ctypes.POINTER(ctypes.c_float),
+                                                         _vp, ctypes.POINTER(_vp), ctypes.POINTER(_vp),
+                                                         ctypes.POINTER(_vp), ctypes.POINTER(_vp), _vp, _vp, _i32, _i32,
+                                                         _vp]),
     "pwg_resstack_supported": (ctypes.c_int, [_i32, _i32, _i32]),
     "pwg_resstack_packed_weight_floats": (ctypes.c_size_t, [_i32]),
     "pwg_resstack_pack_weight": (ctypes.c_int, [_i32, _vp, _vp, _vp, _vp, _vp, _vp, _vp, _vp]),
diff --git a/parallelwavegan_amd/csrc/mfma_conv.h b/parallelwavegan_amd/csrc/mfma_conv.h
--- a/parallelwavegan_amd/csrc/mfma_conv.h
+++ b/parallelwavegan_amd/csrc/mfma_conv.h
@@ -215,6 +215,56 @@
       split_product<TILE, TN, XFIRST>(p, wf, bfr, acc[mi]);
       if (p == 0) {
         __builtin_amdgcn_sched_barrier(0);
+        nx[2] = split_part_request(w, part_stride, rn, 2);
+        __builtin_amdgcn_sched_barrier(0);
+      }
+    }
+#pragma unroll
+    for (int p = 0; p < 3; ++p) wf[p] = nx[p];
+    __builtin_amdgcn_sched_barrier(0);
+  }
+}
+
+constexpr int kSplitPlaneOrder[3] = {0, 2, 1};
+static_assert(kSplitInputPart[0] == kSplitPlaneOrder[0] && kSplitInputPart[1] == kSplitPlaneOrder[1] &&
+                  kSplitInputPart[2] == kSplitPlaneOrder[2],
+              "the fragments are numbered in the order of their first use");
+template <int TILE, int TN, int ROW>
+__device__ __forceinline__ void split_plane_request(bf16x8 (&bfr)[3][TN], int f, const __bf16* xs, int col, int off,
+                                                    int plane) {
+  const int p = kSplitPlaneOrder[f / TN], ni = f % TN;
+  bfr[p][ni] = *reinterpret_cast<const bf16x8*>(xs + (col + ni * TILE) * ROW + off + p * plane);
+}
+template <int TILE, int TN, int ROW, int NPRE>
+__device__ __forceinline__ void split_planes_request(bf16x8 (&bfr)[3][TN], const __bf16* xs, int col, int off, int plane) {
+#pragma unroll
+  for (int f = 0; f < NPRE; ++f) split_plane_request<TILE, TN, ROW>(bfr, f, xs, col, off, plane);
+}
+template <int TILE, int TM, int TN, int ROW, bool XFIRST, int NPRE>
+__device__ __forceinline__ void split_step_pipelined(bf16x8 (&wf)[3], const bf16x8* __restrict__ w, long part_stride,
+                                                     unsigned row, unsigned row_next, bf16x8 (&cur)[3][TN],
+                                                     bf16x8 (&nxt)[3][TN], const __bf16* xs, int col, int off,
+                                                     int col_next, int off_next, int plane,
+                                                     typename Mfma<TILE>::acc_t (&acc)[TM][TN]) {
+  static_assert(NPRE >= 1 && NPRE <= 3 * TN && 3 * TN <= 6 * TM, "one request per group of TN MFMAs");
+#pragma unroll
+  for (int f = NPRE; f < 3 * TN; ++f) split_plane_request<TILE, TN, ROW>(cur, f, xs, col, off, plane);
+#pragma unroll
+  for (int mi = 0; mi < TM; ++mi) {
+    const unsigned rn = mi + 1 < TM ? row + (mi + 1) * TILE : row_next;
+    bf16x8 nx[3];
+    nx[0] = split_part_request(w, part_stride, rn, 0);
+    nx[1] = split_part_request(w, part_stride, rn, 1);
+    __builtin_amdgcn_sched_barrier(0);
+#pragma unroll
+    for (int p = 0; p < 6; ++p) {
+      if (mi * 6 + p < NPRE) {
+        split_plane_request<TILE, TN, ROW>(nxt, mi * 6 + p, xs, col_next, off_next, plane);
+        __builtin_amdgcn_sched_barrier(0);
+      }
+      split_product<TILE, TN, XFIRST>(p, wf, cur, acc[mi]);
+      __builtin_amdgcn_sched_barrier(0);
+      if (p == 0) {
         nx[2] = split_part_request(w, part_stride, rn, 2);
         __builtin_amdgcn_sched_barrier(0);
       }
diff --git a/parallelwavegan_amd/csrc/resunit_split.hip b/parallelwavegan_amd/csrc/resunit_split.hip
--- a/parallelwavegan_amd/csrc/resunit_split.hip
+++ b/parallelwavegan_amd/csrc/resunit_split.hip
@@ -90,13 +90,33 @@
   using Cfg = RuSplitCfg<C>;
   split_step_request(wf, w, part_stride, wrow + split_step_rows<TILE>(Cfg::CHUNKS, Cfg::M_PAD, SplitStepId{0, 0, 0}, h));
 }
-template <int C, int TILE, bool XFIRST>
+template <int C, int TILE, bool XFIRST, int NPRE>
 __device__ __forceinline__ void ru_contract(bf16x8 (&wf)[3], const bf16x8* __restrict__ w, long part_stride, unsigned wrow,
                                             const __bf16* bl, int plane, int tap_step, int taps, int h,
                                             typename Mfma<TILE>::acc_t (&acc)[32 / TILE][64 / TILE]) {
   using Cfg = RuSplitCfg<C>;
   constexpr int HL = 64 / TILE, KSTEPS = KC / (8 * HL), TM = 32 / TILE, TN = 64 / TILE;
   SplitStepId step{0, 0, 0};
+  if constexpr (NPRE > 0) {
+    bf16x8 pf[2][3][TN];
+    split_planes_request<TILE, TN, Cfg::ROW, NPRE>(pf[0], bl, 0, split_step_off<TILE>(step, h), plane);
+    const int steps = Cfg::CHUNKS * taps * KSTEPS;
+#pragma unroll 1
+    for (int s = 0; s < steps; s += 2) {
+#pragma unroll
+      for (int half = 0; half < 2; ++half) {
+        if (half == 1 && s + 1 >= steps) break;
+        const SplitStepId next = split_step_successor(step, Cfg::CHUNKS, taps, KSTEPS);
+        split_step_pipelined<TILE, TM, TN, Cfg::ROW, XFIRST, NPRE>(
+            wf, w, part_stride, wrow + split_step_rows<TILE>(Cfg::CHUNKS, Cfg::M_PAD, step, h),
+            wrow + split_step_rows<TILE>(Cfg::CHUNKS, Cfg::M_PAD, next, h), pf[half], pf[half ^ 1], bl,
+            step.tap * tap_step, step.chunk * KC + split_step_off<TILE>(step, h), next.tap * tap_step,
+            next.chunk * KC + split_step_off<TILE>(next, h), plane, acc);
+        step = next;
+      }
+    }
+    return;
+  }
 #pragma unroll 1
   for (int s = 0; s < Cfg::CHUNKS * taps * KSTEPS; ++s) {
     const SplitStepId next = split_step_successor(step, Cfg::CHUNKS, taps, KSTEPS);
@@ -114,7 +134,7 @@
   return wave_n * 64 + (n / NG) * TILE + 4 * h + 4 * HL * (n % NG);
 }
 
-template <int C, int TILE, bool RAGGED>
+template <int C, int TILE, bool RAGGED, int NPRE>
 __global__ __launch_bounds__(256, 2) void resunit_split_kernel(RuSplitArgsOf<RAGGED> a) {
   using Cfg = RuSplitCfg<C>;
   constexpr int WAVES_N = Cfg::WAVES_N, ROW = Cfg::ROW, H = Cfg::H;
@@ -210,7 +230,7 @@
   __syncthreads();
 
   if (pair) {
-    ru_contract<C, TILE, false>(wf, a.w1, a.part_stride, wrow, xs + (wave_n * 64 + r + a.sh) * ROW, a.plane, a.d1, a.k,
+    ru_contract<C, TILE, false, NPRE>(wf, a.w1, a.part_stride, wrow, xs + (wave_n * 64 + r + a.sh) * ROW, a.plane, a.d1, a.k,
                                 h, acc);
     ru_request<C, TILE>(wf, a.w2, a.part_stride, wrow, h);
     if (has2) request_values(a.add2, ad2);
@@ -248,10 +268,10 @@
       *reinterpret_cast<bf16x8*>(dst + 2 * a.plane) = z;
     }
     __syncthreads();
-    ru_contract<C, TILE, true>(wf, a.w2, a.part_stride, wrow, xs + (wave_n * 64 + r) * ROW, a.plane, 1, a.k, h,
+    ru_contract<C, TILE, true, NPRE>(wf, a.w2, a.part_stride, wrow, xs + (wave_n * 64 + r) * ROW, a.plane, 1, a.k, h,
                                acc);
   } else {
-    ru_contract<C, TILE, true>(wf, a.w1, a.part_stride, wrow, xs + (wave_n * 64 + r + a.sh) * ROW, a.plane, a.d1, a.k,
+    ru_contract<C, TILE, true, NPRE>(wf, a.w1, a.part_stride, wrow, xs + (wave_n * 64 + r + a.sh) * ROW, a.plane, a.d1, a.k,
                                h, acc);
   }
 
@@ -334,13 +354,38 @@
   return PWG_OK;
 }
 
+constexpr int kPlaneFormPlan = 0, kPlaneFormResident = 1, kPlaneFormPipelined = 2;
+template <int TILE>
+constexpr int ru_planes_ahead() {
+  return 3 * (64 / TILE);
+}
+template <int C, int TILE>
+constexpr int rb_planes_ahead() {
+  return TILE == 16 ? (C == 32 ? 6 : 8) : 3 * (64 / TILE);
+}
+static int ru_split_plane_form(int channels, int kernel, int n_units) {
+  if (n_units == 0) return channels == 64 && kernel >= 7 && kernel <= 11 ? kPlaneFormPipelined : kPlaneFormResident;
+  return channels == 32 && kernel == 3 && n_units == 2 ? kPlaneFormPipelined : kPlaneFormResident;
+}
+static int ru_split_resolve_plane_form(const char* name, int plane_form, int channels, int kernel, int n_units,
+                                       bool* pipelined) {
+  PWG_REQUIRE(plane_form == kPlaneFormPlan || plane_form == kPlaneFormResident || plane_form == kPlaneFormPipelined,
+              PWG_ERR_BAD_SHAPE, "%s: plane_form = %d (0 plan, 1 resident, 2 pipelined)", name, plane_form);
+  *pipelined = (plane_form == kPlaneFormPlan ? ru_split_plane_form(channels, kernel, n_units) : plane_form) ==
+               kPlaneFormPipelined;
+  return PWG_OK;
+}
+
 template <bool RAGGED>
 static int ru_split_forward(const pwg_resunit_desc* d, const float* x, const void* w1, const float* b1, const void* w2,
-                            const float* b2, const float* add2, float* y, int mfma_shape, hipStream_t stream,
-                            const int32_t* frames = nullptr, int rate = 0) {
+                            const float* b2, const float* add2, float* y, int mfma_shape, int plane_form,
+                            hipStream_t stream, const int32_t* frames = nullptr, int rate = 0) {
   RuSplitGeom g;
   const int rc = ru_split_geometry(d, &g);
   if (rc != PWG_OK) return rc;
+  bool ahead = false;
+  const int rcf = ru_split_resolve_plane_form("resunit_split_forward", plane_form, d->channels, d->kernel, 0, &ahead);
+  if (rcf != PWG_OK) return rcf;
   PWG_REQUIRE(x && w1 && y, PWG_ERR_NULL, "resunit_split_forward: NULL pointer");
   PWG_REQUIRE(x != y, PWG_ERR_BAD_SHAPE, "resunit_split_forward: y must not alias x (tiles read their neighbours' halo)");
   PWG_REQUIRE((d->has_conv2 != 0) == (w2 != nullptr), PWG_ERR_BAD_SHAPE,
@@ -367,9 +412,12 @@
   PWG_REQUIRE(split_image_addressable(a.part_stride * 8), PWG_ERR_UNSUPPORTED, "resunit_split_forward: weight image too large");
   a.slope1 = d->slope1, a.slope2 = d->slope2, a.out_div = d->out_div;
   if constexpr (RAGGED) a.frames = frames, a.rate = rate;
+  constexpr int A16 = ru_planes_ahead<16>(), A32 = ru_planes_ahead<32>();
   void (*kern)(RuSplitArgsOf<RAGGED>) =
-      C == 32 ? (mfma_shape == 32 ? resunit_split_kernel<32, 32, RAGGED> : resunit_split_kernel<32, 16, RAGGED>)
-              : (mfma_shape == 32 ? resunit_split_kernel<64, 32, RAGGED> : resunit_split_kernel<64, 16, RAGGED>);
+      ahead ? (C == 32 ? (mfma_shape == 32 ? resunit_split_kernel<32, 32, RAGGED, A32> : resunit_split_kernel<32, 16, RAGGED, A16>)
+                       : (mfma_shape == 32 ? resunit_split_kernel<64, 32, RAGGED, A32> : resunit_split_kernel<64, 16, RAGGED, A16>))
+            : (C == 32 ? (mfma_shape == 32 ? resunit_split_kernel<32, 32, RAGGED, 0> : resunit_split_kernel<32, 16, RAGGED, 0>)
+                       : (mfma_shape == 32 ? resunit_split_kernel<64, 32, RAGGED, 0> : resunit_split_kernel<64, 16, RAGGED, 0>));
   if (g.lds > kConvMaxLds && !lds_limit_is_set(reinterpret_cast<const void*>(kern), g.lds)) {
     hipError_t e = hipFuncSetAttribute(reinterpret_cast<const void*>(kern), hipFuncAttributeMaxDynamicSharedMemorySize,
                                        (int)g.lds);
@@ -418,7 +466,7 @@
   int edge;
 };
 
-template <int C, int TILE>
+template <int C, int TILE, int NPRE>
 __global__ __launch_bounds__(256, 2) void resblock_split_kernel(RbSplitArgs a) {
   using Cfg = RuSplitCfg<C>;
   constexpr int WAVES_N = Cfg::WAVES_N, ROW = Cfg::ROW, H = Cfg::H;
@@ -509,7 +557,7 @@
     }
     __syncthreads();
 
-    ru_contract<C, TILE, false>(wf, a.w1[u], part_stride, wrow, fr + (wave_n * 64 + r - p * d1) * ROW, plane, d1, k, h,
+    ru_contract<C, TILE, false, NPRE>(wf, a.w1[u], part_stride, wrow, fr + (wave_n * 64 + r - p * d1) * ROW, plane, d1, k, h,
                                 acc);
     ru_request<C, TILE>(wf, a.w2[u], part_stride, wrow, h);
     if (last && has2) request_values(a.u.add2, ad2, true);
@@ -538,7 +586,7 @@
         }
       }
     __syncthreads();
-    ru_contract<C, TILE, true>(wf, a.w2[u], part_stride, wrow, fr + (wave_n * 64 + r - p) * ROW, plane, 1, k, h, acc);
+    ru_contract<C, TILE, true, NPRE>(wf, a.w2[u], part_stride, wrow, fr + (wave_n * 64 + r - p) * ROW, plane, 1, k, h, acc);
     if (last) break;
 
     ru_request<C, TILE>(wf, a.w1[u + 1], part_stride, wrow, h);
@@ -665,15 +713,17 @@
   return PWG_OK;
 }
 
-extern "C" int pwg_resblock_split_forward_cfg(const pwg_resunit_desc* d, int32_t n_units, const int32_t* dilations,
-                                              const float* slopes1, const float* slopes2, const float* x,
-                                              const void* const* w1_split, const float* const* b1,
-                                              const void* const* w2_split, const float* const* b2, const float* add2,
-                                              float* y, int32_t mfma_shape, void* stream_) {
+static int rb_split_forward(const pwg_resunit_desc* d, int32_t n_units, const int32_t* dilations, const float* slopes1,
+                            const float* slopes2, const float* x, const void* const* w1_split, const float* const* b1,
+                            const void* const* w2_split, const float* const* b2, const float* add2, float* y,
+                            int32_t mfma_shape, int32_t plane_form, void* stream_) {
   hipStream_t stream = (hipStream_t)stream_;
   RbSplitGeom g;
   const int rc = rb_split_geometry(d, n_units, dilations, &g);
   if (rc != PWG_OK) return rc;
+  bool ahead = false;
+  const int rcf = ru_split_resolve_plane_form("resblock_split_forward", plane_form, d->channels, d->kernel, n_units, &ahead);
+  if (rcf != PWG_OK) return rcf;
   PWG_REQUIRE(x && y && w1_split && w2_split && b1 && b2 && slopes1 && slopes2, PWG_ERR_NULL,
               "resblock_split_forward: NULL pointer");
   PWG_REQUIRE(x != y, PWG_ERR_BAD_SHAPE, "resblock_split_forward: y must not alias x (frames read their neighbours' columns)");
@@ -706,8 +756,13 @@
   PWG_REQUIRE(split_image_addressable(a.u.part_stride * 8), PWG_ERR_UNSUPPORTED,
               "resblock_split_forward: weight image too large");
   a.u.slope1 = slopes1[0], a.u.slope2 = slopes2[0], a.u.out_div = d->out_div;
-  void (*kern)(RbSplitArgs) = C == 32 ? (mfma_shape == 32 ? resblock_split_kernel<32, 32> : resblock_split_kernel<32, 16>)
-                                      : (mfma_shape == 32 ? resblock_split_kernel<64, 32> : resblock_split_kernel<64, 16>);
+  void (*kern)(RbSplitArgs) =
+      ahead ? (C == 32 ? (mfma_shape == 32 ? resblock_split_kernel<32, 32, rb_planes_ahead<32, 32>()>
+                                           : resblock_split_kernel<32, 16, rb_planes_ahead<32, 16>()>)
+                       : (mfma_shape == 32 ? resblock_split_kernel<64, 32, rb_planes_ahead<64, 32>()>
+                                           : resblock_split_kernel<64, 16, rb_planes_ahead<64, 16>()>))
+            : (C == 32 ? (mfma_shape == 32 ? resblock_split_kernel<32, 32, 0> : resblock_split_kernel<32, 16, 0>)
+                       : (mfma_shape == 32 ? resblock_split_kernel<64, 32, 0> : resblock_split_kernel<64, 16, 0>));
   if (g.lds > kConvMaxLds && !lds_limit_is_set(reinterpret_cast<const void*>(kern), g.lds)) {
     hipError_t e = hipFuncSetAttribute(reinterpret_cast<const void*>(kern), hipFuncAttributeMaxDynamicSharedMemorySize,
                                        (int)g.lds);
@@ -729,6 +784,34 @@
   return PWG_OK;
 }
 
+extern "C" int pwg_resblock_split_forward_cfg(const pwg_resunit_desc* d, int32_t n_units, const int32_t* dilations,
+                                              const float* slopes1, const float* slopes2, const float* x,
+                                              const void* const* w1_split, const float* const* b1,
+                                              const void* const* w2_split, const float* const* b2, const float* add2,
+                                              float* y, int32_t mfma_shape, void* stream) {
+  return rb_split_forward(d, n_units, dilations, slopes1, slopes2, x, w1_split, b1, w2_split, b2, add2, y, mfma_shape,
+                          kPlaneFormPlan, stream);
+}
+
+extern "C" int pwg_resblock_split_forward_planes(const pwg_resunit_desc* d, int32_t n_units, const int32_t* dilations,
+                                                 const float* slopes1, const float* slopes2, const float* x,
+                                                 const void* const* w1_split, const float* const* b1,
+                                                 const void* const* w2_split, const float* const* b2, const float* add2,
+                                                 float* y, int32_t mfma_shape, int32_t plane_form, void* stream) {
+  return rb_split_forward(d, n_units, dilations, slopes1, slopes2, x, w1_split, b1, w2_split, b2, add2, y, mfma_shape,
+                          plane_form, stream);
+}
+
+extern "C" int pwg_resunit_split_plane_form(const pwg_resunit_desc* d, int32_t n_units) {
+  RuSplitGeom g;
+  if (ru_split_geometry(d, &g) != PWG_OK) return 0;
+  if (n_units < 0 || n_units > kRbMaxUnits) {
+    set_error("resunit_split_plane_form: n_units = %d (0: the unit, 1 .. %d: the chained block)", n_units, kRbMaxUnits);
+    return 0;
+  }
+  return ru_split_plane_form(d->channels, d->kernel, n_units);
+}
+
 extern "C" int pwg_resunit_split_supported(const pwg_resunit_desc* d) {
   RuSplitGeom g;
   return ru_split_geometry(d, &g) == PWG_OK ? 1 : 0;
@@ -737,13 +820,20 @@
 extern "C" int pwg_resunit_split_forward(const pwg_resunit_desc* d, const float* x, const void* w1_split, const float* b1,
                                          const void* w2_split, const float* b2, const float* add2, float* y,
                                          void* stream) {
-  return ru_split_forward<false>(d, x, w1_split, b1, w2_split, b2, add2, y, kDefaultMfmaShape, (hipStream_t)stream);
+  return ru_split_forward<false>(d, x, w1_split, b1, w2_split, b2, add2, y, kDefaultMfmaShape, kPlaneFormPlan,
+                                 (hipStream_t)stream);
 }
 
 extern "C" int pwg_resunit_split_forward_cfg(const pwg_resunit_desc* d, const float* x, const void* w1_split,
                                              const float* b1, const void* w2_split, const float* b2, const float* add2,
                                              float* y, int32_t mfma_shape, void* stream) {
-  return ru_split_forward<false>(d, x, w1_split, b1, w2_split, b2, add2, y, mfma_shape, (hipStream_t)stream);
+  return ru_split_forward<false>(d, x, w1_split, b1, w2_split, b2, add2, y, mfma_shape, kPlaneFormPlan, (hipStream_t)stream);
+}
+
+extern "C" int pwg_resunit_split_forward_planes(const pwg_resunit_desc* d, const float* x, const void* w1_split,
+                                                const float* b1, const void* w2_split, const float* b2, const float* add2,
+                                                float* y, int32_t mfma_shape, int32_t plane_form, void* stream) {
+  return ru_split_forward<false>(d, x, w1_split, b1, w2_split, b2, add2, y, mfma_shape, plane_form, (hipStream_t)stream);
 }
 
 extern "C" int pwg_resunit_split_ragged_supported(const pwg_resunit_desc* d, int32_t rate) {
@@ -751,14 +841,30 @@
   return ru_split_geometry(d, &g) == PWG_OK && ru_split_ragged_rate(rate) == PWG_OK ? 1 : 0;
 }
 
-extern "C" int pwg_resunit_split_forward_ragged(const pwg_resunit_desc* d, const float* x, const void* w1_split,
-                                                const float* b1, const void* w2_split, const float* b2,
-                                                const float* add2, float* y, int32_t mfma_shape, const int32_t* frames,
-                                                int32_t rate, void* stream) {
+static int ru_split_forward_ragged(const pwg_resunit_desc* d, const float* x, const void* w1_split, const float* b1,
+                                   const void* w2_split, const float* b2, const float* add2, float* y, int32_t mfma_shape,
+                                   int32_t plane_form, const int32_t* frames, int32_t rate, void* stream) {
   PWG_REQUIRE(frames != nullptr, PWG_ERR_NULL, "resunit_split_forward_ragged: NULL frames table");
   PWG_REQUIRE((reinterpret_cast<uintptr_t>(frames) & 3u) == 0, PWG_ERR_BAD_SHAPE,
               "resunit_split_forward_ragged: the frames table must be 4-B aligned");
   const int rc = ru_split_ragged_rate(rate);
   if (rc != PWG_OK) return rc;
-  return ru_split_forward<true>(d, x, w1_split, b1, w2_split, b2, add2, y, mfma_shape, (hipStream_t)stream, frames, rate);
-}
+  return ru_split_forward<true>(d, x, w1_split, b1, w2_split, b2, add2, y, mfma_shape, plane_form, (hipStream_t)stream,
+                                frames, rate);
+}
+
+extern "C" int pwg_resunit_split_forward_ragged(const pwg_resunit_desc* d, const float* x, const void* w1_split,
+                                                const float* b1, const void* w2_split, const float* b2,
+                                                const float* add2, float* y, int32_t mfma_shape, const int32_t* frames,
+                                                int32_t rate, void* stream) {
+  return ru_split_forward_ragged(d, x, w1_split, b1, w2_split, b2, add2, y, mfma_shape, kPlaneFormPlan, frames, rate,
+                                 stream);
+}
+
+extern "C" int pwg_resunit_split_forward_ragged_planes(const pwg_resunit_desc* d, const float* x, const void* w1_split,
+                                                       const float* b1, const void* w2_split, const float* b2,
+                                                       const float* add2, float* y, int32_t mfma_shape,
+                                                       int32_t plane_form, const int32_t* frames, int32_t rate,
+                                                       void* stream) {
+  return ru_split_forward_ragged(d, x, w1_split, b1, w2_split, b2, add2, y, mfma_shape, plane_form, frames, rate, stream);
+}
diff --git a/parallelwavegan_amd/ops.py b/parallelwavegan_amd/ops.py
--- a/parallelwavegan_amd/ops.py
+++ b/parallelwavegan_amd/ops.py
@@ -460,7 +460,15 @@
     return bool(_lib.lib().pwg_resunit_split_supported(ctypes.byref(desc)))
 
 
-def resunit_forward_split(desc, x, w1_split, b1, w2_split=None, b2=None, add2=None, out=None, mfma_shape=None):
+PLANE_FORMS = {None: 0, "plan": 0, "resident": 1, "pipelined": 2}
+
+
+def resunit_split_plane_form(desc, n_units=0):
+    return {1: "resident", 2: "pipelined"}.get(_lib.lib().pwg_resunit_split_plane_form(ctypes.byref(desc), int(n_units)))
+
+
+def resunit_forward_split(desc, x, w1_split, b1, w2_split=None, b2=None, add2=None, out=None, mfma_shape=None,
+                          plane_form=None):
     _require_device(x, b1, b2, add2, out)
     for w in (w1_split, w2_split):
         if w is not None and (not w.is_cuda or w.dtype != torch.uint8):
@@ -473,7 +481,10 @@
     if out is None:
         out = torch.empty_like(x)
     args = (ctypes.byref(desc), _ptr(x), _ptr(w1_split), _ptr(b1), _ptr(w2_split), _ptr(b2), _ptr(add2), _ptr(out))
-    if mfma_shape is None:
+    if plane_form is not None:
+        rc = _lib.lib().pwg_resunit_split_forward_planes(*args, 16 if mfma_shape is None else int(mfma_shape),
+                                                         PLANE_FORMS[plane_form], _stream())
+    elif mfma_shape is None:
         rc = _lib.lib().pwg_resunit_split_forward(*args, _stream())
     else:
         rc = _lib.lib().pwg_resunit_split_forward_cfg(*args, int(mfma_shape), _stream())
@@ -494,7 +505,7 @@
 
 
 def resblock_forward_split(desc, x, dilations, slopes1, slopes2, w1_split, b1, w2_split, b2, add2=None, out=None,
-                           mfma_shape=None):
+                           mfma_shape=None, plane_form=None):
     n = len(dilations)
     assert len(slopes1) == len(slopes2) == len(w1_split) == len(b1) == len(w2_split) == len(b2) == n
     _require_device(x, add2, out, *b1, *b2)
@@ -511,11 +522,15 @@
     def ptrs(ts):
         return (ctypes.c_void_p * n)(*[None if t is None else t.data_ptr() for t in ts])
 
-    _lib.check(_lib.lib().pwg_resblock_split_forward_cfg(
-        ctypes.byref(desc), n, (ctypes.c_int32 * n)(*[int(v) for v in dilations]),
-        (ctypes.c_float * n)(*[float(v) for v in slopes1]), (ctypes.c_float * n)(*[float(v) for v in slopes2]), _ptr(x),
-        ptrs(w1_split), ptrs(b1), ptrs(w2_split), ptrs(b2), _ptr(add2), _ptr(out),
-        16 if mfma_shape is None else int(mfma_shape), _stream()), "resblock_split_forward")
+    args = (ctypes.byref(desc), n, (ctypes.c_int32 * n)(*[int(v) for v in dilations]),
+            (ctypes.c_float * n)(*[float(v) for v in slopes1]), (ctypes.c_float * n)(*[float(v) for v in slopes2]), _ptr(x),
+            ptrs(w1_split), ptrs(b1), ptrs(w2_split), ptrs(b2), _ptr(add2), _ptr(out),
+            16 if mfma_shape is None else int(mfma_shape))
+    if plane_form is not None:
+        rc = _lib.lib().pwg_resblock_split_forward_planes(*args, PLANE_FORMS[plane_form], _stream())
+    else:
+        rc = _lib.lib().pwg_resblock_split_forward_cfg(*args, _stream())
+    _lib.check(rc, "resblock_split_forward")
     return out
 
 
@@ -552,7 +567,7 @@
 
 
 def resunit_forward_split_ragged(desc, x, frames, rate, w1_split, b1, w2_split=None, b2=None, add2=None, out=None,
-                                 mfma_shape=16):
+                                 mfma_shape=16, plane_form=None):
     _require_device(x, b1, b2, add2, out)
     for w in (w1_split, w2_split):
         if w is not None and (not w.is_cuda or w.dtype != torch.uint8):
@@ -565,9 +580,14 @@
     assert add2 is None or add2.numel() == x.numel()
     if out is None:
         out = torch.empty_like(x)
-    _lib.check(_lib.lib().pwg_resunit_split_forward_ragged(
-        ctypes.byref(desc), _ptr(x), _ptr(w1_split), _ptr(b1), _ptr(w2_split), _ptr(b2), _ptr(add2), _ptr(out),
-        int(mfma_shape), _ptr(frames), int(rate), _stream()), "resunit_split_forward_ragged")
+    args = (ctypes.byref(desc), _ptr(x), _ptr(w1_split), _ptr(b1), _ptr(w2_split), _ptr(b2), _ptr(add2), _ptr(out),
+            int(mfma_shape))
+    if plane_form is not None:
+        rc = _lib.lib().pwg_resunit_split_forward_ragged_planes(*args, PLANE_FORMS[plane_form], _ptr(frames), int(rate),
+                                                                _stream())
+    else:
+        rc = _lib.lib().pwg_resunit_split_forward_ragged(*args, _ptr(frames), int(rate), _stream())
+    _lib.check(rc, "resunit_split_forward_ragged")
     return out
 
 
```

After: 86.40 million samples/s. Within noise of the previous version (-0.0%).
